# Many98/Crop2Seg

Measured on AMD Instinct MI355X. Metric: train patches/sec (Tx10x128x128) U-TAE, higher is better.
Workload: dtype f32

## Files before the change

crop2seg_amd/_lib.py:

```python
from __future__ import annotations

import ctypes as C
import os
from typing import Optional

HERE = os.path.dirname(os.path.abspath(__file__))
LIB_PATH = os.environ.get("C2S_LIB", os.path.join(HERE, "libc2s_hip.so"))

c_float_p = C.c_void_p
c_int_p = C.c_void_p

PAD_ZEROS, PAD_REFLECT = 0, 1
SRC_F32, SRC_I16, SRC_U16 = 0, 1, 2
NORM_GROUP, NORM_BATCH = 0, 1


class ConvDesc(C.Structure):
    _fields_ = [(n, C.c_int) for n in (
        "N", "C0", "C1", "Hin", "Win", "Cout", "CoutP", "Hout", "Wout", "OutH", "OutW", "KH", "KW", "S",
        "pad_y", "pad_x", "pad_mode", "osy", "osx", "ooy", "oox", "accumulate", "reflect_adjoint")]


class WgradDesc(C.Structure):
    _fields_ = [(n, C.c_int) for n in (
        "N", "C0", "C1", "Hin", "Win", "Cout", "Hout", "Wout", "KH", "KW", "S", "pad_y", "pad_x", "pad_mode",
        "nslices")]


class NormDesc(C.Structure):
    _fields_ = [("N", C.c_int), ("C", C.c_int), ("HW", C.c_int), ("kind", C.c_int), ("groups", C.c_int),
                ("training", C.c_int), ("eps", C.c_float), ("momentum", C.c_float)]


class LtaeDesc(C.Structure):
    _fields_ = [("B", C.c_int), ("T", C.c_int), ("C", C.c_int), ("HW", C.c_int), ("n_head", C.c_int),
                ("d_model", C.c_int), ("eps", C.c_float), ("dropout_p", C.c_float), ("seed", C.c_uint64),
                ("keep", C.c_void_p), ("seed_dev", C.c_void_p), ("keep_bits", C.c_void_p)]


class AggDesc(C.Structure):
    _fields_ = [(n, C.c_int) for n in ("B", "T", "C", "H", "W", "n_head", "h", "w")]


P = C.c_void_p
I = C.c_int
L = C.c_long
F = C.c_float
SZ = C.c_size_t

SIGNATURES = {
    "c2s_abi_version": (I, []),
    "c2s_last_error": (C.c_char_p, []),
    "c2s_init": (I, [I]),
    "c2s_device_cus": (I, []),
    "c2s_pack_weights": (I, [P, P, I, I, I, I, L, L, C.POINTER(I), P]),
    "c2s_pack_job_bytes": (SZ, []),
    "c2s_pack_job_fill": (I, [P, P, P, I, I, I, I, L, L, I, C.POINTER(I), I]),
    "c2s_pack_job_blocks": (I, [I, I, I, I]),
    "c2s_pack_batch": (I, [P, I, I, P]),
    "c2s_conv_igemm": (I, [C.POINTER(ConvDesc), P, P, P, P, P, P, P]),
    "c2s_conv_igemm_split": (I, [C.POINTER(ConvDesc), I]),
    "c2s_conv_xpair": (I, [C.POINTER(ConvDesc), P, P, P, P, P, P]),
    "c2s_conv3x3_smallcin_supported": (I, [C.POINTER(ConvDesc)]),
    "c2s_conv3x3_smallcin": (I, [C.POINTER(ConvDesc), P, P, P, P, P, P]),
    "c2s_winograd_packed_floats": (SZ, [I, I]),
    "c2s_pack_weights_winograd": (I, [P, P, I, I, I, L, L, C.POINTER(I), P]),
    "c2s_conv3x3_winograd": (I, [C.POINTER(ConvDesc), P, P, P, P, P, P, P]),
    "c2s_winograd16_packed_floats": (SZ, [I, I]),
    "c2s_pack_weights_winograd16": (I, [P, P, I, I, I, L, L, C.POINTER(I), P]),
    "c2s_conv3x3_winograd16_supported": (I, [C.POINTER(ConvDesc)]),
    "c2s_conv3x3_winograd16": (I, [C.POINTER(ConvDesc), P, P, P, P, P, P, P]),
    "c2s_s2wino_packed_floats": (SZ, [I, I]),
    "c2s_pack_weights_s2wino": (I, [P, P, I, I, I, L, L, C.POINTER(I), P]),
    "c2s_conv4x4s2_winograd_supported": (I, [C.POINTER(ConvDesc)]),
    "c2s_conv4x4s2_winograd": (I, [C.POINTER(ConvDesc), P, P, P, P, P, P]),
    "c2s_s2dgrad_packed_floats": (SZ, [I, I]),
    "c2s_pack_weights_s2dgrad": (I, [P, P, I, I, I, L, L, C.POINTER(I), P]),
    "c2s_conv4x4s2_dgrad_winograd_supported": (I, [C.POINTER(ConvDesc)]),
    "c2s_conv4x4s2_dgrad_winograd": (I, [C.POINTER(ConvDesc), P, P, P, P, P]),
    "c2s_conv4x4s2_dgrad_winograd_skip_supported": (I, [C.POINTER(ConvDesc), I, I]),
    "c2s_conv4x4s2_dgrad_winograd_skip": (I, [C.POINTER(ConvDesc), P, P, P, P, P, P, I, I, P]),
    "c2s_bf16x3_packed_elems": (SZ, [I, I]),
    "c2s_pack_weights_bf16x3": (I, [P, P, P, I, I, I, I, L, L, C.POINTER(I), P]),
    "c2s_conv3x3_bf16x3": (I, [C.POINTER(ConvDesc), P, P, P, P, P, P, P, P]),
    "c2s_bf16x3_set_single_product": (None, [I]),
    "c2s_wgrad_workspace_floats": (SZ, [C.POINTER(WgradDesc)]),
    "c2s_conv_wgrad": (I, [C.POINTER(WgradDesc), P, P, P, P, SZ, P, P]),
    "c2s_wgrad_algorithms": (I, [I, I]),
    "c2s_wgrad_path": (I, [C.POINTER(WgradDesc), C.POINTER(I)]),
    "c2s_wgrad_reduce": (I, [C.POINTER(WgradDesc), P, P, L, L, C.POINTER(I), I, P]),
    "c2s_wgrad_reduce_job_bytes": (SZ, []),
    "c2s_wgrad_reduce_job_blocks": (I, [C.POINTER(WgradDesc)]),
    "c2s_wgrad_reduce_job_fill": (I, [P, C.POINTER(WgradDesc), P, P, L, L, C.POINTER(I), I, I]),
    "c2s_wgrad_reduce_batch": (I, [P, I, I, P]),
    "c2s_dwconv_fwd": (I, [P, P, P, P, I, I, I, I, I, I, I, I, P]),
    "c2s_dwconv_dgrad": (I, [P, P, P, P, I, I, I, I, I, I, I, I, I, P]),
    "c2s_dwconv_wgrad": (I, [P, P, P, P, P, I, I, I, I, I, I, I, I, P]),
    "c2s_dwconv_paths": (I, [I, I, I, I, I, I, C.POINTER(I), C.POINTER(I), C.POINTER(I)]),
    "c2s_norm_workspace_floats": (SZ, [C.POINTER(NormDesc)]),
    "c2s_norm_fwd": (I, [C.POINTER(NormDesc), P, P, P, P, P, P, P, P, P, P, I, P, SZ, P, F, P]),
    "c2s_norm_bwd": (I, [C.POINTER(NormDesc), P, P, P, P, P, I, P, P, P, P, P, SZ, P, P]),
    "c2s_norm_bwd_params": (I, [C.POINTER(NormDesc), P, P, P, P, P, P]),
    "c2s_norm_onepass_sync_bytes": (SZ, [C.POINTER(NormDesc), I]),
    "c2s_norm_fwd_onepass": (I, [C.POINTER(NormDesc), P, P, P, P, P, P, P, P, P, P, I, P, F, P, SZ, P]),
    "c2s_norm_bwd_onepass": (I, [C.POINTER(NormDesc), P, P, P, P, P, I, P, P, P, P, P, SZ, P, P, SZ, P]),
    "c2s_se_workspace_floats": (SZ, [I, I, I]),
    "c2s_channel_bias_add": (I, [P, P, P, I, I, I, P]),
    "c2s_se_fwd": (I, [P, P, P, P, P, P, P, P, I, I, I, F, P, SZ, P]),
    "c2s_se_bwd": (I, [P, P, P, P, P, P, P, P, P, P, I, I, P, I, I, I, P, SZ, P]),
    "c2s_frame_flags": (I, [P, P, I, L, F, P]),
    "c2s_ltae_attn_fwd": (I, [C.POINTER(LtaeDesc)] + [P] * 13 + [P]),
    "c2s_positional_table": (I, [P, P, L, C.c_float, P]),
    "c2s_ltae_fold_fwd": (I, [P] * 9 + [I, I, P]),
    "c2s_ltae_fold_bwd": (I, [P] * 16 + [I, I, I, P, SZ, P]),
    "c2s_ltae_fold_bwd_workspace_floats": (SZ, []),
    "c2s_positional_table_ex": (I, [P, P, L, C.c_float, I, P]),
    "c2s_ltae_fold_fwd_ex": (I, [P] * 9 + [I, I, I, I, I, P]),
    "c2s_ltae_fold_bwd_ex": (I, [P] * 16 + [I, I, I, I, I, I, P, SZ, P]),
    "c2s_ltae_fold_bwd_workspace_floats_ex": (SZ, [I, I]),
    "c2s_ltae_pe_table": (I, [I, P, P, F, P, P, P, P, P, I, P]),
    "c2s_ltae_pe_abs_add": (I, [P, P, P, P, P, I, P]),
    "c2s_ltae_pe_abs_bwd": (I, [P, P, P, P, I, P]),
    "c2s_ltae_pe_fwd": (I, [P, P, P, P, P, I, I, I, I, P]),
    "c2s_ltae_pe_gattn": (I, [P, P, P, P, I, I, I, P]),
    "c2s_ltae_pe_bwd": (I, [I] + [P] * 15 + [I, I, I, P]),
    "c2s_ltae_pe_bwd_ex": (I, [I] + [P] * 15 + [I, I, I, I, P]),
    "c2s_ltae_fwd_workspace_floats": (SZ, [C.POINTER(LtaeDesc)]),
    "c2s_ltae_attn_fwd_ws": (I, [C.POINTER(LtaeDesc)] + [P] * 13 + [P, SZ, P]),
    "c2s_ltae_uses_streaming": (I, [C.POINTER(LtaeDesc)]),
    "c2s_ltae_fwd_path": (I, [C.POINTER(LtaeDesc)]),
    "c2s_ltae_attn_optional": (I, [C.POINTER(LtaeDesc)]),
    "c2s_ltae_paths": (I, [C.POINTER(LtaeDesc), I, P, P]),
    "c2s_ltae_bwd_workspace_floats": (SZ, [C.POINTER(LtaeDesc)]),
    "c2s_ltae_attn_bwd": (I, [C.POINTER(LtaeDesc)] + [P] * 22 + [SZ, P]),
    "c2s_dropout_nchw": (I, [P, P, I, I, I, F, C.c_uint64, P, P, P]),
    "c2s_pixel_gn_fwd": (I, [P, P, P, P, P, I, I, I, I, F, P]),
    "c2s_pixel_gn_bwd_workspace_floats": (SZ, [I, I, I]),
    "c2s_pixel_gn_bwd": (I, [P, P, P, P, P, P, P, I, I, I, I, P, SZ, P]),
    "c2s_attn_head_mean": (I, [P, P, I, L, P]),
    "c2s_attn_head_mean_bwd": (I, [P, P, I, L, I, P]),
    "c2s_frame_mean_weights": (I, [P, P, I, I, I, P]),
    "c2s_temporal_aggregate_fwd": (I, [C.POINTER(AggDesc), P, P, P, P, P]),
    "c2s_temporal_aggregate_bwd_workspace_floats": (SZ, [C.POINTER(AggDesc)]),
    "c2s_temporal_aggregate_bwd": (I, [C.POINTER(AggDesc), P, P, P, P, P, I, P, P, SZ, P]),
    "c2s_temporal_aggregate_bwd_skip": (I, [C.POINTER(AggDesc), P, P, P, P, P, I, P, P, P, SZ, P]),
    "c2s_agg_skip_term": (I, [C.POINTER(AggDesc), P, P, P, P, P]),
    "c2s_cross_entropy_workspace_floats": (SZ, [I, I]),
    "c2s_cross_entropy": (I, [P, P, P, P, P, I, I, I, F, C.c_longlong, P, SZ, P]),
    "c2s_metrics_update": (I, [P, P, P, P, P, P, I, I, I, P]),
    "c2s_confusion_add": (I, [P, P, P, L, I, P]),
    "c2s_loss_meter_add": (I, [P, P, P]),
    "c2s_boundary_target": (I, [P, P, I, I, I, P]),
    "c2s_region_relabel": (I, [P, P, I, I, I, I, C.c_longlong, P]),
    "c2s_focal_ce_workspace_floats": (SZ, []),
    "c2s_focal_ce": (I, [P, P, P, P, I, I, I, F, C.c_longlong, I, P, SZ, P]),
    "c2s_focal_ce_ex": (I, [P, P, P, P, P, I, I, I, F, C.c_longlong, I, I, P, SZ, P]),
    "c2s_smooth_ce_workspace_floats": (SZ, []),
    "c2s_smooth_ce": (I, [P, P, P, P, P, P, I, I, I, I, F, C.c_longlong, I, P, SZ, P]),
    "c2s_smooth_ce_ex": (I, [P, P, P, P, P, P, P, I, I, I, I, F, C.c_longlong, I, I, P, SZ, P]),
    "c2s_recall_ce_workspace_floats": (SZ, [I, I]),
    "c2s_recall_ce": (I, [P, P, P, P, P, P, I, I, I, C.c_longlong, I, P, SZ, P]),
    "c2s_parcel_seeds": (I, [P, P, P, P, I, I, I, I, I, I, F, P]),
    "c2s_label_components_workspace_bytes": (SZ, [I, I, I]),
    "c2s_label_components": (I, [P, P, P, I, I, I, I, P, SZ, P, P]),
    "c2s_parcel_vote_workspace_bytes": (SZ, [I, I, I]),
    "c2s_parcel_vote": (I, [P, P, P, P, I, I, I, I, I, F, I, P, SZ, P, P]),
    "c2s_parcel_soft_vote_workspace_bytes": (SZ, [I, I, I]),
    "c2s_parcel_soft_vote": (I, [P, P, P, P, P, P, P, I, I, I, I, I, I, F, I, P, SZ, P, P]),
    "c2s_collate_series": (I, [P, I, P, P, P, P, P, I, I, I, I, I, C.POINTER(I), C.POINTER(F), C.POINTER(F), F, P]),
    "c2s_collate_series_ndvi": (I, [P, I, P, P, P, P, P, I, I, I, I, I, C.POINTER(I), C.POINTER(F), C.POINTER(F), F, I, I, P]),
    "c2s_softmax_stitch": (I, [P, P, P, I, I, I, I, I, I, I, I, P]),
    "c2s_window_count": (I, [I, I, I]),
    "c2s_window_origin": (I, [I, I, I, I]),
    "c2s_cut_windows": (I, [P, P, I, I, I, I, I, I, I, I, I, I, I, C.POINTER(F), P]),
    "c2s_window_frames": (I, [P, I, P, P, P, P, P, I, I, I, I, I, I, I, I, I, I, F, I, P]),
    "c2s_cut_windows_raw": (I, [P, I, P, P, I, I, I, I, I, I, I, I, I, I, I, I, C.POINTER(I), C.POINTER(F), C.POINTER(F),
                                C.POINTER(F), F, I, I, P]),
    "c2s_softmax_blend": (I, [P, P, P, P, P, I, I, I, I, I, I, I, I, I, I, P]),
    "c2s_blend_finish": (I, [P, P, P, I, I, I, P]),
    "c2s_adam_flat": (I, [P, P, P, P, L, F, F, F, F, I, P, F, P]),
    "c2s_grad_sumsq_workspace_doubles": (SZ, []),
    "c2s_grad_sumsq": (I, [P, P, P, I, L, P, SZ, P, P]),
    "c2s_step_decide": (I, [P, F, F, I, P, P, I, P, P]),
    "c2s_adam_slots": (I, [P, P, P, P, P, P, P, I, L, F, F, F, F, P, P]),
    "c2s_restore_if_skipped": (I, [P, P, L, P, P]),
    "c2s_fill": (I, [P, L, F, P]),
    "c2s_add_inplace": (I, [P, P, L, P]),
}

_LIB: Optional[C.CDLL] = None


class C2SError(RuntimeError):
    pass


def lib() -> C.CDLL:
    global _LIB
    if _LIB is None:
        if not os.path.exists(LIB_PATH):
            raise C2SError(
                f"{LIB_PATH} not found: build it with `python -m crop2seg_amd.build` "
                "(or __graft_entry__.build()); crop2seg_amd has no CPU/PyTorch fallback")
        handle = C.CDLL(LIB_PATH)
        for name, (res, args) in SIGNATURES.items():
            fn = getattr(handle, name)
            fn.restype = res
            fn.argtypes = args
        _LIB = handle
    return _LIB


_INITED = set()


def init_device(index: int) -> None:
    if index in _INITED:
        return
    check(lib().c2s_init(index), "c2s_init")
    _INITED.add(index)


def check(rc: int, what: str) -> None:
    if rc != 0:
        msg = lib().c2s_last_error().decode(errors="replace")
        raise C2SError(f"{what} failed (code {rc}): {msg}")
```

crop2seg_amd/backbones/functional.py:

```python
from __future__ import annotations

from dataclasses import dataclass, field
from typing import List, Optional, Sequence, Tuple

import torch

from .. import _lib
from .. import engine as E

Tensor = torch.Tensor


@dataclass
class BackboneSpec:
    model: str = "utae"
    input_dim: int = 10
    encoder_widths: List[int] = field(default_factory=lambda: [64, 64, 64, 128])
    decoder_widths: List[int] = field(default_factory=lambda: [32, 32, 64, 128])
    out_conv: List[int] = field(default_factory=lambda: [32, 20])
    str_conv_k: int = 4
    str_conv_s: int = 2
    str_conv_p: int = 1
    agg_mode: str = "att_group"
    encoder_norm: str = "group"
    n_head: int = 16
    d_model: int = 256
    d_k: int = 4
    pad_value: float = 0.0
    padding_mode: str = "reflect"
    conv_type: str = "2d"
    add_boundary_loss: bool = False
    encoder: bool = False
    return_maps: bool = False
    pe_period: float = 1000.0
    pe_mode: str = "rel"
    num_queries: int = 1
    add_squeeze_excit: bool = False
    use_mbconv: bool = False
    attn_dropout: float = 0.1
    mlp_dropout: float = 0.2


@dataclass
class DropoutState:
    attn_seed: int = 0
    mlp_seed: int = 0
    attn_keep: Optional[Tensor] = None
    mlp_keep: Optional[Tensor] = None
    seed_dev: Optional[Tensor] = None


def _mode(spec: BackboneSpec) -> int:
    return _lib.PAD_REFLECT if spec.padding_mode == "reflect" else _lib.PAD_ZEROS


def _norm_kind(norm: str) -> int:
    if norm not in ("group", "batch", "instance"):
        raise NotImplementedError(f"norm {norm!r}")
    return _lib.NORM_BATCH if norm == "batch" else _lib.NORM_GROUP


def conv_layer(ctx: E.Ctx, srcs: Sequence[Tensor], prefix: str, n_convs: int, norm: str, k: int, s: int, p: int,
               spec: BackboneSpec, valid: Optional[Tensor], residual: Optional[Tensor] = None,
               depthwise_separable: bool = False, need_input_grad: bool = True, add_squeeze: bool = False) -> Tensor:
    mode = _mode(spec)
    x = list(srcs)
    y = None
    for i in range(n_convs):
        cp = f"{prefix}.conv.{3 * i}"
        if depthwise_separable:
            t = E.depthwise_conv2d(ctx, x[0], cp + ".depthwise.weight", k, s, p, mode, valid)
            y = E.conv2d(ctx, [t], cp + ".pointwise.weight", None, 1, 1, 0, _lib.PAD_ZEROS, valid)
            bias = None
        else:
            y = E.conv2d(ctx, x, cp + ".weight", cp + ".bias", k, s, p, mode, valid,
                         need_input_grad=need_input_grad or i > 0)
            bias = cp + ".bias"
        last = i == n_convs - 1
        y = E.norm_act(ctx, y, f"{prefix}.conv.{3 * i + 1}", _norm_kind(norm), y.shape[1] if norm == "instance" else 4, True,
                       residual if last else None, valid, spec.pad_value if valid is not None else 0.0, conv_bias=bias,
                       affine=norm != "instance")
        x = [y]
    if add_squeeze:
        y = E.squeeze_excite(ctx, y, f"{prefix}.conv.{3 * n_convs}", valid, spec.pad_value if valid is not None else 0.0)
    return y


def _norm_groups(norm: str, channels: int) -> int:
    return channels if norm == "instance" else 4


def mbconv(ctx: E.Ctx, srcs: Sequence[Tensor], prefix: str, norm: str, spec: BackboneSpec, valid: Optional[Tensor],
           need_input_grad: bool = True) -> Tensor:
    cin = sum(t.shape[1] for t in srcs)
    res = (prefix + ".0.0.block.0.weight") in ctx.p
    base = prefix + (".0.0.block" if res else ".0.0.0")
    cout = ctx.p[base + ".7.weight"].shape[0]
    assert res == (cin == cout) and (not res or len(srcs) == 1)
    kind = _norm_kind(norm)
    pv = spec.pad_value if valid is not None else 0.0
    aff = norm != "instance"
    o = E.conv2d(ctx, srcs, base + ".0.weight", base + ".0.bias", 1, 1, 0, _lib.PAD_ZEROS, valid, need_input_grad=need_input_grad)
    o = E.norm_act(ctx, o, base + ".1", kind, _norm_groups(norm, o.shape[1]), True, None, valid, pv, conv_bias=base + ".0.bias",
                   affine=aff)
    o = E.depthwise_conv2d(ctx, o, base + ".3.weight", 3, 1, 1, _lib.PAD_REFLECT, valid, bname=base + ".3.bias")
    o = E.norm_act(ctx, o, base + ".4", kind, _norm_groups(norm, o.shape[1]), True, None, valid, pv, conv_bias=base + ".3.bias",
                   affine=aff)
    o = E.squeeze_excite(ctx, o, base + ".6", valid, pv)
    o = E.conv2d(ctx, [o], base + ".7.weight", base + ".7.bias", 1, 1, 0, _lib.PAD_ZEROS, valid)
    return E.norm_act(ctx, o, base + ".8", kind, _norm_groups(norm, o.shape[1]), False, srcs[0] if res else None, valid, pv,
                      conv_bias=base + ".7.bias", affine=aff)


def mbconv_layer(ctx, srcs, prefix, n, norm, spec, valid, need_input_grad=True):
    x = list(srcs)
    for i in range(n):
        x = [mbconv(ctx, x, f"{prefix}.conv.{i}", norm, spec, valid, need_input_grad=need_input_grad or i > 0)]
    return x[0]


def conv_block(ctx, x, prefix, n_convs, norm, spec, valid, need_input_grad=True, depthwise_separable=False, add_squeeze=False):
    if spec.use_mbconv:
        return mbconv_layer(ctx, [x], prefix + ".conv", n_convs, norm, spec, valid, need_input_grad=need_input_grad)
    return conv_layer(ctx, [x], prefix + ".conv", n_convs, norm, 3, 1, 1, spec, valid, need_input_grad=need_input_grad,
                      depthwise_separable=depthwise_separable, add_squeeze=add_squeeze)


def down_conv_block(ctx, x, prefix, norm, spec, valid, depthwise_separable=False, add_squeeze=False):
    o = conv_layer(ctx, [x], prefix + ".down", 1, norm, spec.str_conv_k, spec.str_conv_s, spec.str_conv_p, spec, valid,
                   depthwise_separable=depthwise_separable)
    if spec.use_mbconv:
        o1 = mbconv_layer(ctx, [o], prefix + ".conv1", 1, norm, spec, valid)
        return mbconv_layer(ctx, [o1], prefix + ".conv2", 1, norm, spec, valid)
    o1 = conv_layer(ctx, [o], prefix + ".conv1", 1, norm, 3, 1, 1, spec, valid, depthwise_separable=depthwise_separable)
    o2 = conv_layer(ctx, [o1], prefix + ".conv2", 1, norm, 3, 1, 1, spec, valid, residual=o1,
                    depthwise_separable=depthwise_separable)
    if add_squeeze:
        o2 = E.squeeze_excite(ctx, o2, prefix + ".sae", valid, spec.pad_value if valid is not None else 0.0)
    return o2


def up_conv_block(ctx, x, skip, prefix, spec):
    sk = E.conv2d(ctx, [skip], prefix + ".skip_conv.0.weight", prefix + ".skip_conv.0.bias", 1, 1, 0, _lib.PAD_ZEROS, None)
    sk = E.norm_act(ctx, sk, prefix + ".skip_conv.1", _lib.NORM_BATCH, 1, True, None, None,
                    conv_bias=prefix + ".skip_conv.0.bias")
    assert spec.str_conv_s == 2, "only stride-2 up-convs are built"
    up = E.conv_transpose2d(ctx, x, prefix + ".up.0.weight", prefix + ".up.0.bias", spec.str_conv_k, spec.str_conv_p)
    up = E.norm_act(ctx, up, prefix + ".up.1", _lib.NORM_BATCH, 1, True, None, None, conv_bias=prefix + ".up.0.bias")
    if spec.use_mbconv:
        o1 = mbconv_layer(ctx, [up, sk], prefix + ".conv1", 1, "batch", spec, None)
        return mbconv_layer(ctx, [o1], prefix + ".conv2", 1, "batch", spec, None)
    o1 = conv_layer(ctx, [up, sk], prefix + ".conv1", 1, "batch", 3, 1, 1, spec, None)
    return conv_layer(ctx, [o1], prefix + ".conv2", 1, "batch", 3, 1, 1, spec, None, residual=o1)


def ltae(ctx, x5, dates, valid, prefix, spec: BackboneSpec, drop: DropoutState, with_tail: bool, need_attn: bool = True):
    emb, attn = E.ltae_attention(ctx, x5, dates, valid, prefix, spec.n_head, spec.d_k, spec.d_model, spec.pe_period,
                                 spec.attn_dropout, with_tail, drop.attn_seed, drop.attn_keep, drop.seed_dev,
                                 pe_mode=spec.pe_mode, need_attn=need_attn)
    if not with_tail:
        return None, attn
    o = E.conv2d(ctx, [emb], prefix + ".mlp.0.weight", prefix + ".mlp.0.bias", 1, 1, 0, _lib.PAD_ZEROS, None)
    o = E.norm_act(ctx, o, prefix + ".mlp.2", _lib.NORM_BATCH, 1, True, None, None, conv_bias=prefix + ".mlp.0.bias")
    o = E.dropout_nchw(ctx, o, spec.mlp_dropout, drop.mlp_seed, drop.mlp_keep, drop.seed_dev)
    o = E.pixel_group_norm(ctx, o, prefix + ".out_norm", spec.n_head)
    return o, attn


@dataclass
class BackboneOutput:
    logits: Optional[Tensor]
    att: Tensor
    boundary: Optional[Tensor] = None
    maps: Optional[List[Tensor]] = None
    last: Optional[Tensor] = None


def _decoder_and_head(ctx, out, skips, spec, att):
    n_stages = len(spec.encoder_widths)
    maps = [out]
    for i in range(n_stages - 1):
        out = up_conv_block(ctx, out, skips[i], f"up_blocks.{i}", spec)
        maps.append(out)
    keep_maps = maps if (spec.return_maps or spec.encoder) else None
    if spec.encoder:
        return BackboneOutput(None, att, None, keep_maps, out)
    if spec.use_mbconv:
        logits = mbconv_layer(ctx, [out], "out_conv.conv", len(spec.out_conv), "group", spec, None)
        boundary = mbconv_layer(ctx, [out], "boundary_conv.conv", 2, "group", spec, None) if spec.add_boundary_loss else None
        return BackboneOutput(logits, att, boundary, keep_maps, out)
    logits = conv_layer(ctx, [out], "out_conv.conv", len(spec.out_conv), "batch", 3, 1, 1, spec, None)
    boundary = None
    if spec.add_boundary_loss:
        boundary = conv_layer(ctx, [out], "boundary_conv.conv", 2, "batch", 3, 1, 1, spec, None)
    return BackboneOutput(logits, att, boundary, keep_maps, out)


def _fold(x5: Tensor) -> Tensor:
    B, T = x5.shape[:2]
    return x5.view(B * T, *x5.shape[2:])


def _unfold(x4: Tensor, B: int, T: int) -> Tensor:
    return x4.view(B, T, *x4.shape[1:])


def utae_forward(ctx, spec, x5, dates, drop):
    B, T = x5.shape[:2]
    valid = E.frame_flags(x5, spec.pad_value)
    dws = spec.conv_type == "depthwise_separable"
    se = spec.add_squeeze_excit
    f = conv_block(ctx, _fold(x5), "in_conv", 2, spec.encoder_norm, spec, valid, need_input_grad=False, depthwise_separable=dws,
                   add_squeeze=se)
    fmaps = [f]
    n_stages = len(spec.encoder_widths)
    for i in range(n_stages - 1):
        f = down_conv_block(ctx, f, f"down_blocks.{i}", spec.encoder_norm, spec, valid, depthwise_separable=dws, add_squeeze=se)
        fmaps.append(f)
    if ctx.tape is not None and ctx.early_hook is not None:
        ctx.tape.record(ctx.early_hook)
    out, att = ltae(ctx, _unfold(fmaps[-1], B, T), dates, valid, "temporal_encoder", spec, drop, True)
    skips = [E.temporal_aggregate(ctx, _unfold(fmaps[-(i + 2)], B, T), att, valid, spec.n_head, spec.agg_mode)
             for i in range(n_stages - 1)]
    return _decoder_and_head(ctx, out, skips, spec, att)


def timeunet_forward(ctx, spec, x5, dates, drop):
    B, T = x5.shape[:2]
    valid = E.frame_flags(x5, spec.pad_value)
    dws = spec.conv_type == "depthwise_separable"
    se = spec.add_squeeze_excit
    f0 = conv_block(ctx, _fold(x5), "in_conv", 2, spec.encoder_norm, spec, valid, need_input_grad=False, depthwise_separable=dws,
                    add_squeeze=se)
    if ctx.tape is not None and ctx.early_hook is not None:
        ctx.tape.record(ctx.early_hook)
    out, att = ltae(ctx, _unfold(f0, B, T), dates, valid, "temporal_encoder", spec, drop, True, need_attn=ctx.want_att)
    fmaps = [out]
    n_stages = len(spec.encoder_widths)
    for i in range(n_stages - 1):
        fmaps.append(down_conv_block(ctx, fmaps[-1], f"down_blocks.{i}", spec.encoder_norm, spec, None, depthwise_separable=dws,
                                     add_squeeze=se))
    skips = [fmaps[-(i + 2)] for i in range(n_stages - 1)]
    return _decoder_and_head(ctx, fmaps[-1], skips, spec, att)


def wtae_forward(ctx, spec, x5, dates, drop):
    B, T = x5.shape[:2]
    valid = E.frame_flags(x5, spec.pad_value)
    dws = spec.conv_type == "depthwise_separable"
    se = spec.add_squeeze_excit
    f0 = conv_block(ctx, _fold(x5), "in_conv", 2, spec.encoder_norm, spec, valid, need_input_grad=False, depthwise_separable=dws,
                    add_squeeze=se)
    red = f0
    n_stages = len(spec.encoder_widths)
    for i in range(n_stages - 1):
        red = down_conv_block(ctx, red, f"spatial_reduction.{i}", spec.encoder_norm, spec, valid, depthwise_separable=True,
                              add_squeeze=se)
    if ctx.tape is not None and ctx.early_hook is not None:
        ctx.tape.record(ctx.early_hook)
    _, att = ltae(ctx, _unfold(red, B, T), dates, valid, "temporal_encoder", spec, drop, False)
    fmaps = [E.temporal_aggregate(ctx, _unfold(f0, B, T), att, valid, spec.n_head, spec.agg_mode)]
    for i in range(n_stages - 1):
        fmaps.append(down_conv_block(ctx, fmaps[-1], f"down_blocks.{i}", spec.encoder_norm, spec, None, depthwise_separable=dws,
                                     add_squeeze=se))
    skips = [fmaps[-(i + 2)] for i in range(n_stages - 1)]
    return _decoder_and_head(ctx, fmaps[-1], skips, spec, att)


FORWARDS = {"utae": utae_forward, "timeunet": timeunet_forward, "wtae": wtae_forward}
```

crop2seg_amd/build.py:

```python
from __future__ import annotations

import os
import shutil
import subprocess
import sys
from concurrent.futures import ThreadPoolExecutor

HERE = os.path.dirname(os.path.abspath(__file__))
CSRC = os.path.join(HERE, "csrc")
LIB = os.path.join(HERE, "libc2s_hip.so")
SOURCES = ["pack.hip", "conv_igemm.hip", "conv_bf16x3.hip", "conv_xpair.hip", "conv_first.hip", "conv_winograd.hip", "conv_winograd16.hip", "conv_s2wino.hip", "conv_s2dgrad.hip", "conv_wgrad.hip", "norm.hip", "se.hip", "ltae.hip", "ltae_long.hip", "ltae_pe.hip", "aggregate.hip", "misc.hip", "guard.hip", "metrics.hip", "loss.hip", "parcels.hip", "io.hip"]
FLAGS = ["--offload-arch=gfx950", "-O3", "-fPIC", "-std=c++17", "-Wall", "-Wno-unused-function",
         "-Wno-unused-result", "-Wno-unused-value", "-D__HIP_PLATFORM_AMD__"]


def hipcc() -> str:
    for cand in (os.environ.get("HIPCC"), shutil.which("hipcc"), "/opt/rocm/bin/hipcc"):
        if cand and os.path.exists(cand):
            return cand
    raise RuntimeError("hipcc not found")


def _stale(target: str, deps) -> bool:
    if not os.path.exists(target):
        return True
    t = os.path.getmtime(target)
    return any(os.path.getmtime(d) > t for d in deps)


def build(force: bool = False, verbose: bool = True) -> str:
    cc = hipcc()
    headers = [os.path.join(CSRC, "common.h"), os.path.join(CSRC, "ltae_drop.h"), os.path.join(CSRC, "ltae_long.h"),
               os.path.join(CSRC, "parcels_uf.h"),
               os.path.join(os.path.dirname(HERE), "include", "c2s_hip.h")]
    objs, jobs = [], []
    for s in SOURCES:
        src = os.path.join(CSRC, s)
        obj = os.path.join(CSRC, s.replace(".hip", ".o"))
        objs.append(obj)
        if force or _stale(obj, [src] + headers):
            jobs.append((src, obj))

    def compile_one(job):
        src, obj = job
        cmd = [cc, *FLAGS, "-c", src, "-o", obj]
        r = subprocess.run(cmd, capture_output=True, text=True)
        if r.returncode != 0:
            raise RuntimeError(f"hipcc failed for {src}:\n{r.stdout}\n{r.stderr}")
        if verbose and r.stderr.strip():
            print(r.stderr, file=sys.stderr)
        return obj

    if jobs:
        with ThreadPoolExecutor(max_workers=min(4, len(jobs))) as ex:
            list(ex.map(compile_one, jobs))
    if force or jobs or _stale(LIB, objs):
        r = subprocess.run([cc, "--offload-arch=gfx950", "-shared", "-fPIC", *objs, "-o", LIB],
                           capture_output=True, text=True)
        if r.returncode != 0:
            raise RuntimeError(f"link failed:\n{r.stdout}\n{r.stderr}")
    return LIB


if __name__ == "__main__":
    print(build(force="--force" in sys.argv))
```

crop2seg_amd/csrc/conv_first.hip:

```cpp
#include "common.h"

namespace {

struct FirstParams {
    const float* src;
    const float* wpk;
    const float* bias;
    float* out;
    const int* valid;
    int N, Cin, H, W, Cout, CoutP;
    int tiles_x, tiles_y, ntiles;
};

constexpr int FT_ROWS = 8, FT_COLS = 32;
constexpr int FT_PR = FT_ROWS + 2, FT_PC = FT_COLS + 2;
constexpr int ft_chs() {
    int v = FT_PR * FT_PC;
    while (v % 64 != 32) ++v;
    return v;
}
constexpr int FT_CHS = ft_chs();

template <int NP, bool REFLECT>
__global__ __launch_bounds__(256, 2) void conv_first_kernel(FirstParams p) {
    constexpr int NCH = 2 * NP;
    constexpr int NE = NCH * FT_PR * FT_PC;
    constexpr int EPT = (NE + 255) / 256;
    __shared__ float patch[NCH * FT_CHS];
    const int tid = threadIdx.x, lane = tid & 63, wave = __builtin_amdgcn_readfirstlane(tid >> 6);
    const int px = lane & 31, kk = lane >> 5;
    const int cb = blockIdx.y * 64;

    float wreg[9][NP][2];
#pragma unroll
    for (int t = 0; t < 9; ++t)
#pragma unroll
        for (int s = 0; s < NP; ++s) {
            const int ch = 2 * s + kk;
#pragma unroll
            for (int h = 0; h < 2; ++h) {
                const float v = p.wpk[((size_t)t * p.Cin + (ch < p.Cin ? ch : 0)) * p.CoutP + cb + h * 32 + px];
                wreg[t][s][h] = ch < p.Cin ? v : 0.f;
            }
        }
    __shared__ float bias_s[64];
    if (tid < 64) bias_s[tid] = (p.bias != nullptr && cb + tid < p.Cout) ? p.bias[cb + tid] : 0.f;

    auto load_patch = [&](int tile, float (&v)[EPT]) {
        int tid = threadIdx.x;
        asm volatile("" : "+v"(tid));
        const int n = tile / (p.tiles_x * p.tiles_y);
        const int rem = tile - n * (p.tiles_x * p.tiles_y);
        const int y0 = (rem / p.tiles_x) * FT_ROWS - 1, x0 = (rem % p.tiles_x) * FT_COLS - 1;
        const float* base = p.src + (size_t)n * p.Cin * p.H * p.W;
#pragma unroll
        for (int j = 0; j < EPT; ++j) {
            const int e = tid + 256 * j;
            const int ch = e / (FT_PR * FT_PC), r2 = e - ch * (FT_PR * FT_PC);
            const int row = r2 / FT_PC, col = r2 - row * FT_PC;
            int gy = y0 + row, gx = x0 + col;
            bool ok = e < NE && ch < p.Cin;
            if (REFLECT) {
                gy = reflect_idx(gy, p.H); gx = reflect_idx(gx, p.W);
            } else {
                ok = ok && gy >= 0 && gy < p.H && gx >= 0 && gx < p.W;
                gy = min(max(gy, 0), p.H - 1); gx = min(max(gx, 0), p.W - 1);
            }
            const int chc = min(ch, p.Cin - 1);
            const float t = base[((size_t)chc * p.H + gy) * p.W + gx];
            v[j] = ok ? t : 0.f;
        }
    };
    auto store_patch = [&](const float (&v)[EPT]) {
        int tid = threadIdx.x;
        asm volatile("" : "+v"(tid));
#pragma unroll
        for (int j = 0; j < EPT; ++j) {
            const int e = tid + 256 * j;
            const int ch = e / (FT_PR * FT_PC), r2 = e - ch * (FT_PR * FT_PC);
            if (e < NE) patch[ch * FT_CHS + r2] = v[j];
        }
    };
    auto frame_ok = [&](int tile) {
        return p.valid == nullptr || p.valid[tile / (p.tiles_x * p.tiles_y)] != 0;
    };

    int tile = blockIdx.x;
    float pre[EPT];
    if (tile < p.ntiles && frame_ok(tile)) load_patch(tile, pre);
    for (; tile < p.ntiles; tile += gridDim.x) {
        const bool ok = frame_ok(tile);
        const int nxt = tile + gridDim.x;
        if (ok) {
            __syncthreads();
            store_patch(pre);
            __syncthreads();
        }
        if (nxt < p.ntiles && frame_ok(nxt)) load_patch(nxt, pre);
        if (!ok) continue;
        f32x16 acc[2][2];
#pragma unroll
        for (int r = 0; r < 2; ++r)
#pragma unroll
            for (int h = 0; h < 2; ++h)
#pragma unroll
                for (int i = 0; i < 16; ++i) acc[r][h][i] = 0.f;
        const float* pb = patch + kk * FT_CHS + (2 * wave) * FT_PC + px;
#pragma unroll
        for (int ky = 0; ky < 3; ++ky)
#pragma unroll
            for (int kx = 0; kx < 3; ++kx)
#pragma unroll
                for (int s = 0; s < NP; ++s) {
                    const float b0 = pb[2 * s * FT_CHS + ky * FT_PC + kx];
                    const float b1 = pb[2 * s * FT_CHS + (ky + 1) * FT_PC + kx];
                    acc[0][0] = __builtin_amdgcn_mfma_f32_32x32x2f32(wreg[ky * 3 + kx][s][0], b0, acc[0][0], 0, 0, 0);
                    acc[0][1] = __builtin_amdgcn_mfma_f32_32x32x2f32(wreg[ky * 3 + kx][s][1], b0, acc[0][1], 0, 0, 0);
                    acc[1][0] = __builtin_amdgcn_mfma_f32_32x32x2f32(wreg[ky * 3 + kx][s][0], b1, acc[1][0], 0, 0, 0);
                    acc[1][1] = __builtin_amdgcn_mfma_f32_32x32x2f32(wreg[ky * 3 + kx][s][1], b1, acc[1][1], 0, 0, 0);
                }
        const int n = tile / (p.tiles_x * p.tiles_y);
        const int rem = tile - n * (p.tiles_x * p.tiles_y);
        const int y = (rem / p.tiles_x) * FT_ROWS + 2 * wave, x0 = (rem % p.tiles_x) * FT_COLS;
        const size_t plane = (size_t)p.H * p.W;
        float* ub = p.out + ((size_t)n * p.Cout + cb) * plane + (size_t)y * p.W + x0;
        const unsigned lo = (unsigned)(4 * kk) * (unsigned)plane + (unsigned)px;
#pragma unroll
        for (int h = 0; h < 2; ++h)
#pragma unroll
            for (int i = 0; i < 16; ++i) {
                const int og = h * 32 + (i & 3) + 8 * (i >> 2);
                float* op = ub + (size_t)og * plane;
                const float b = bias_s[og + 4 * kk];
                op[lo] = acc[0][h][i] + b;
                op[lo + p.W] = acc[1][h][i] + b;
            }
    }
}

}

extern "C" int c2s_conv3x3_smallcin_supported(const c2s_conv_desc* d) {
    return d && d->KH == 3 && d->KW == 3 && d->S == 1 && d->pad_y == 1 && d->pad_x == 1 && d->C1 == 0 && d->C0 >= 1 &&
           d->C0 <= 10 && d->Cout % 64 == 0 && d->CoutP == d->Cout && d->Hin % FT_ROWS == 0 && d->Win % FT_COLS == 0 && d->Hout == d->Hin &&
           d->Wout == d->Win && d->OutH == d->Hin && d->OutW == d->Win && d->osy == 1 && d->osx == 1 && d->ooy == 0 &&
           d->oox == 0 && !d->accumulate && !d->reflect_adjoint;
}

extern "C" int c2s_conv3x3_smallcin(const c2s_conv_desc* d, const float* src, const float* wpk, const float* bias,
                                    float* out, const int* valid, void* stream) {
    C2S_REQUIRE(d && src && wpk && out, "conv3x3_smallcin: null pointer");
    C2S_REQUIRE(c2s_conv3x3_smallcin_supported(d),
                "conv3x3_smallcin: needs 3x3/s1/pad1, one source of <= 10 channels, Cout %% 64 == 0, H %% 8 == 0, W %% 32 == 0");
    if (d->pad_mode == C2S_PAD_REFLECT) C2S_REQUIRE(d->Hin >= 2 && d->Win >= 2, "conv3x3_smallcin: reflect needs planes >= 2x2");
    FirstParams p;
    p.src = src; p.wpk = wpk; p.bias = bias; p.out = out; p.valid = valid;
    p.N = d->N; p.Cin = d->C0; p.H = d->Hin; p.W = d->Win; p.Cout = d->Cout; p.CoutP = d->CoutP;
    p.tiles_x = d->Win / FT_COLS; p.tiles_y = d->Hin / FT_ROWS;
    const long nt = (long)d->N * p.tiles_x * p.tiles_y;
    C2S_REQUIRE(nt < (1L << 30), "conv3x3_smallcin: too many tiles");
    p.ntiles = (int)nt;
    const int cus = c2s_cus();
    const int wgs = (int)(nt < 2L * cus ? nt : 2L * cus);
    const dim3 grid(wgs, d->CoutP / 64);
    hipStream_t st = (hipStream_t)stream;
    const bool reflect = d->pad_mode == C2S_PAD_REFLECT;
    if (d->C0 <= 4) {
        if (reflect) hipLaunchKernelGGL((conv_first_kernel<2, true>), grid, dim3(256), 0, st, p);
        else hipLaunchKernelGGL((conv_first_kernel<2, false>), grid, dim3(256), 0, st, p);
    } else {
        if (reflect) hipLaunchKernelGGL((conv_first_kernel<5, true>), grid, dim3(256), 0, st, p);
        else hipLaunchKernelGGL((conv_first_kernel<5, false>), grid, dim3(256), 0, st, p);
    }
    C2S_CHECK_LAUNCH("conv_first");
    return C2S_OK;
}
```

crop2seg_amd/csrc/norm.hip:

```cpp
#include "common.h"

namespace {

constexpr int SEG = 2048;

__host__ __device__ inline int seg_len(int HW) { return HW < SEG ? HW : SEG; }
__host__ __device__ inline int n_segs(int HW) { return (HW + seg_len(HW) - 1) / seg_len(HW); }

struct SegItem { long row; int seg, len; size_t base; };
__device__ __forceinline__ SegItem seg_item(long item, int HW, int segs) {
    SegItem it;
    it.row = item / segs;
    it.seg = (int)(item % segs);
    const int L = seg_len(HW);
    const int beg = it.seg * L;
    it.len = (HW - beg) < L ? (HW - beg) : L;
    it.base = (size_t)it.row * HW + beg;
    return it;
}


__device__ __forceinline__ float fwd_element(float x, float mu, float a, float b, int relu, bool has_res, float r) {
    float t = (x - mu) * a + b;
    if (relu) t = fmaxf(t, 0.f);
    if (has_res) t += r;
    return t;
}
__device__ __forceinline__ float masked_grad(float g, float xc, float a, float b, int relu) {
    return (!relu || xc * a + b > 0.f) ? g : 0.f;
}
__device__ __forceinline__ void grad_sums(float gg, float xc, float rstd, float& s1, float& s2) {
    s1 += gg;
    s2 += gg * (xc * rstd);
}
__device__ __forceinline__ float bwd_element(float gg, float xc, float k1, float k2, float k3, float& sdx) {
    const float o = k1 * gg + k2 * xc + k3;
    sdx += o;
    return o;
}

__device__ __forceinline__ float chunk_sum(const f32x4& v) { return (v.x + v.y) + (v.z + v.w); }
__device__ __forceinline__ float chunk_sum(float v) { return v; }
__device__ __forceinline__ float chunk_sqdev(const f32x4& v, float mean) {
    const float a = v.x - mean, b = v.y - mean, c = v.z - mean, d = v.w - mean;
    return (a * a + b * b) + (c * c + d * d);
}
__device__ __forceinline__ float chunk_sqdev(float v, float mean) {
    const float a = v - mean;
    return a * a;
}
template <typename F>
__device__ __forceinline__ void each(float x, float r, float& o, F fe) { fe(x, r, o); }
template <typename F>
__device__ __forceinline__ void each(const f32x4& x, const f32x4& r, f32x4& o, F fe) {
#pragma unroll
    for (int e = 0; e < 4; ++e) {
        float t = 0.f;
        fe(x[e], r[e], t);
        o[e] = t;
    }
}

template <typename V, int NK>
__device__ __forceinline__ void load_segment(const float* __restrict__ p, int lane, f32x4 (&v)[NK]) {
#pragma unroll
    for (int k = 0; k < NK; ++k) v[k] = *reinterpret_cast<const V*>(p + lane * 4 + 256 * k);
}

template <int NK>
__device__ __forceinline__ void segment_moments(const f32x4 (&v)[NK], float& mean, float& m2) {
    float s = 0.f;
#pragma unroll
    for (int k = 0; k < NK; ++k) s += chunk_sum(v[k]);
    s = wave_sum(s);
    mean = s / (float)(NK * 256);
    m2 = 0.f;
#pragma unroll
    for (int k = 0; k < NK; ++k) m2 += chunk_sqdev(v[k], mean);
}

template <bool STORE, typename F>
__device__ __forceinline__ void walk_tail(const float* __restrict__ x, const float* __restrict__ r, bool has_r,
                                          float* __restrict__ out, size_t base, int len, int lane, F f) {
    if ((len & 3) == 0) {
        for (int i = lane * 4; i < len; i += 256) {
            const f32x4 xv = *reinterpret_cast<const f32x4*>(x + base + i);
            f32x4 rv = {0.f, 0.f, 0.f, 0.f}, o;
            if (has_r) rv = *reinterpret_cast<const f32x4*>(r + base + i);
            f(xv, rv, o);
            if (STORE) *reinterpret_cast<f32x4*>(out + base + i) = o;
        }
    } else {
        for (int i = lane; i < len; i += 64) {
            float o;
            f(x[base + i], has_r ? r[base + i] : 0.f, o);
            if (STORE) out[base + i] = o;
        }
    }
}
template <bool STORE, typename F>
__device__ __forceinline__ void walk_segment(const float* __restrict__ x, const float* __restrict__ r, bool has_r,
                                             float* __restrict__ out, size_t base, int len, int lane, F f) {
    if (len != SEG) return walk_tail<STORE>(x, r, has_r, out, base, len, lane, f);
    f32x4 xv[SEG / 256], rv[SEG / 256];
    load_segment<f32x4u>(x + base, lane, xv);
    if (has_r) load_segment<f32x4u>(r + base, lane, rv);
#pragma unroll
    for (int k = 0; k < SEG / 256; ++k) {
        f32x4 o;
        f(xv[k], has_r ? rv[k] : f32x4{0.f, 0.f, 0.f, 0.f}, o);
        if (STORE) *reinterpret_cast<f32x4u*>(out + base + lane * 4 + 256 * k) = o;
    }
}

template <typename P>
__device__ __forceinline__ void merge_moments(int items, int lane, float eps, P partial, float& mean_f, float& rstd_f,
                                              float& unbiased) {
    double cnt = 0.0, sum = 0.0;
    for (int it = lane; it < items; it += 64) {
        float pm, pm2;
        int len;
        if (!partial(it, pm, pm2, len)) continue;
        cnt += len;
        sum += (double)pm * len;
    }
    for (int o = 32; o > 0; o >>= 1) { cnt += __shfl_xor(cnt, o, 64); sum += __shfl_xor(sum, o, 64); }
    const double mean = cnt > 0 ? sum / cnt : 0.0;
    double m2 = 0.0;
    for (int it = lane; it < items; it += 64) {
        float pm, pm2;
        int len;
        if (!partial(it, pm, pm2, len)) continue;
        const double dm = (double)pm - mean;
        m2 += (double)pm2 + dm * dm * len;
    }
    for (int o = 32; o > 0; o >>= 1) m2 += __shfl_xor(m2, o, 64);
    const double var = cnt > 0 ? m2 / cnt : 0.0;
    mean_f = (float)mean;
    rstd_f = (float)(1.0 / sqrt(var + (double)eps));
    unbiased = (float)(cnt > 1 ? m2 / (cnt - 1.0) : var);
}

template <typename P>
__device__ __forceinline__ void row_sums(int segs, P partial, float& s1, float& s2) {
    double t1 = 0.0, t2 = 0.0;
    for (int s = 0; s < segs; ++s) {
        float p1, p2;
        partial(s, p1, p2);
        t1 += p1;
        t2 += p2;
    }
    s1 = (float)t1;
    s2 = (float)t2;
}
template <typename R>
__device__ __forceinline__ void merge_coeffs(int n_rows, int lane, int HW, float rstd, R row, float& k2, float& k3) {
    double A = 0.0, Bv = 0.0, cnt = 0.0;
    for (int r = lane; r < n_rows; r += 64) {
        float gm, s1, s2;
        if (!row(r, gm, s1, s2)) continue;
        A += (double)gm * (double)s1;
        Bv += (double)gm * (double)s2;
        cnt += HW;
    }
    for (int o = 32; o > 0; o >>= 1) { A += __shfl_xor(A, o, 64); Bv += __shfl_xor(Bv, o, 64); cnt += __shfl_xor(cnt, o, 64); }
    const double m = cnt > 0 ? cnt : 1.0;
    k2 = (float)(-(double)rstd * rstd * Bv / m);
    k3 = (float)(-(double)rstd * A / m);
}

__global__ __launch_bounds__(256) void row_stats_kernel(const float* __restrict__ x, float* __restrict__ part,
                                                        const int* __restrict__ valid, int C, int HW, int segs,
                                                        long nitems) {
    const long item = (long)blockIdx.x * 4 + (threadIdx.x >> 6);
    if (item >= nitems) return;
    const int lane = threadIdx.x & 63;
    const auto [row, seg, len, base] = seg_item(item, HW, segs);
    if (valid != nullptr && valid[row / C] == 0) return;
    float mean, m2 = 0.f;
    if (len == SEG) {
        f32x4 v[SEG / 256];
        load_segment<f32x4u>(x + base, lane, v);
        segment_moments(v, mean, m2);
    } else {
        float s = 0.f;
        walk_tail<false>(x, nullptr, false, nullptr, base, len, lane, [&](auto v, auto, auto&) { s += chunk_sum(v); });
        s = wave_sum(s);
        mean = s / (float)len;
        walk_tail<false>(x, nullptr, false, nullptr, base, len, lane, [&](auto v, auto, auto&) { m2 += chunk_sqdev(v, mean); });
    }
    m2 = wave_sum(m2);
    if (lane == 0) {
        part[item * 2 + 0] = mean;
        part[item * 2 + 1] = m2;
    }
}

__device__ __forceinline__ void group_mean_rstd(const float* __restrict__ part, const int* __restrict__ valid,
                                                const c2s_norm_desc& d, int segs, int grp, int lane, float& mean_f,
                                                float& rstd_f, float& unbiased) {
    const int L = seg_len(d.HW);
    const bool batch = d.kind == C2S_NORM_BATCH;
    const int cpg = batch ? 1 : d.C / d.groups;
    const int n_rows = batch ? d.N : cpg;
    merge_moments(n_rows * segs, lane, d.eps, [&](int it, float& pm, float& pm2, int& len) {
        const int r = it / segs, sg = it % segs;
        const long row = batch ? (long)r * d.C + grp : (long)(grp / d.groups) * d.C + (grp % d.groups) * cpg + r;
        if (batch && valid != nullptr && valid[r] == 0) return false;
        len = (d.HW - sg * L) < L ? (d.HW - sg * L) : L;
        pm = part[(row * segs + sg) * 2];
        pm2 = part[(row * segs + sg) * 2 + 1];
        return true;
    }, mean_f, rstd_f, unbiased);
}

__global__ __launch_bounds__(256) void norm_apply_kernel(const float* __restrict__ x, const float* __restrict__ part,
                                                         const float* __restrict__ gamma, const float* __restrict__ beta,
                                                         float* __restrict__ rmean, float* __restrict__ rvar,
                                                         long long* __restrict__ nbt,
                                                         float* __restrict__ gstats, float* __restrict__ row_ab,
                                                         const float* __restrict__ res, float* __restrict__ y,
                                                         const int* __restrict__ valid, c2s_norm_desc d, int segs,
                                                         long nitems, int relu, float pad_value) {
    const long item = (long)blockIdx.x * 4 + (threadIdx.x >> 6);
    if (item >= nitems) return;
    const int lane = threadIdx.x & 63;
    const int C = d.C, HW = d.HW;
    const auto [row, seg, len, base] = seg_item(item, HW, segs);
    const int n = (int)(row / C), c = (int)(row % C);
    const bool ok = valid == nullptr || valid[n] != 0;
    const bool batch = d.kind == C2S_NORM_BATCH;
    const int cpg = batch ? 1 : C / d.groups;
    const int grp = batch ? c : n * d.groups + c / cpg;
    const bool first_row = seg == 0 && (batch ? n == 0 : c % cpg == 0);
    float mu = 0.f, rstd = 0.f;
    if (batch && !d.training) {
        mu = rmean[grp];
        rstd = rsqrtf(rvar[grp] + d.eps);
    } else if (batch || ok) {
        float unb;
        group_mean_rstd(part, valid, d, segs, grp, lane, mu, rstd, unb);
        if (batch && first_row && lane == 0 && rmean != nullptr) {
            rmean[grp] = (1.f - d.momentum) * rmean[grp] + d.momentum * mu;
            rvar[grp] = (1.f - d.momentum) * rvar[grp] + d.momentum * unb;
        }
        if (batch && item == 0 && lane == 0 && nbt != nullptr) *nbt += 1;
    }
    if (first_row && lane == 0) { gstats[grp * 2] = mu; gstats[grp * 2 + 1] = rstd; }
    if (!ok) {
        if (seg == 0 && lane == 0) { row_ab[row * 3] = 0.f; row_ab[row * 3 + 1] = 0.f; row_ab[row * 3 + 2] = 0.f; }
        for (int i = lane; i < len; i += 64) y[base + i] = pad_value;
        return;
    }
    const float a = gamma[c] * rstd, b = beta[c];
    if (seg == 0 && lane == 0) { row_ab[row * 3] = a; row_ab[row * 3 + 1] = b; row_ab[row * 3 + 2] = mu; }
    const bool has_res = res != nullptr;
    walk_segment<true>(x, res, has_res, y, base, len, lane, [&](auto xv, auto rv, auto& o) {
        each(xv, rv, o, [&](float xe, float re, float& t) { t = fwd_element(xe, mu, a, b, relu, has_res, re); });
    });
}

__global__ __launch_bounds__(256) void norm_bwd_sums_kernel(const float* __restrict__ x, const float* __restrict__ g,
                                                            const float* __restrict__ row_ab,
                                                            const float* __restrict__ gstats, float* __restrict__ part,
                                                            const int* __restrict__ valid, c2s_norm_desc d, int segs,
                                                            long nitems, int relu) {
    const long item = (long)blockIdx.x * 4 + (threadIdx.x >> 6);
    if (item >= nitems) return;
    const int lane = threadIdx.x & 63;
    const auto [row, seg, len, base] = seg_item(item, d.HW, segs);
    const int n = (int)(row / d.C), c = (int)(row % d.C);
    if (valid != nullptr && valid[n] == 0) {
        if (lane == 0) { part[item * 3] = 0.f; part[item * 3 + 1] = 0.f; }
        return;
    }
    const int grp = d.kind == C2S_NORM_BATCH ? c : n * d.groups + c / (d.C / d.groups);
    const float mean = gstats[grp * 2], rstd = gstats[grp * 2 + 1];
    const float a = row_ab[row * 3], b = row_ab[row * 3 + 1];
    float s1 = 0.f, s2 = 0.f;
    walk_segment<false>(x, g, true, nullptr, base, len, lane, [&](auto xv, auto gv, auto& o) {
        each(xv, gv, o, [&](float xe, float ge, float&) {
            const float xc = xe - mean;
            grad_sums(masked_grad(ge, xc, a, b, relu), xc, rstd, s1, s2);
        });
    });
    s1 = wave_sum(s1); s2 = wave_sum(s2);
    if (lane == 0) { part[item * 3] = s1; part[item * 3 + 1] = s2; }
}

__device__ __forceinline__ void part_row_sums(const float* __restrict__ part, long row, int segs, float& s1, float& s2) {
    row_sums(segs, [&](int s, float& p1, float& p2) {
        p1 = part[(row * segs + s) * 3];
        p2 = part[(row * segs + s) * 3 + 1];
    }, s1, s2);
}

__global__ __launch_bounds__(64) void norm_bwd_params_kernel(const float* __restrict__ part, float* __restrict__ dgamma,
                                                             float* __restrict__ dbeta, float* __restrict__ dbias,
                                                             const int* __restrict__ valid, int N, int C, int segs) {
    const int c = blockIdx.x, lane = threadIdx.x;
    double dg = 0, db = 0;
    for (int n = lane; n < N; n += 64) {
        if (valid != nullptr && valid[n] == 0) continue;
        float s1, s2;
        part_row_sums(part, (long)n * C + c, segs, s1, s2);
        dg += (double)s2;
        db += (double)s1;
    }
    for (int o = 32; o > 0; o >>= 1) { dg += __shfl_xor(dg, o, 64); db += __shfl_xor(db, o, 64); }
    if (lane == 0) {
        if (dgamma != nullptr) dgamma[c] = (float)dg;
        if (dbeta != nullptr) dbeta[c] = (float)db;
    }
    if (dbias == nullptr) return;
    double s = 0;
    for (int it = lane; it < N * segs; it += 64) {
        const int n = it / segs, k = it - n * segs;
        if (valid != nullptr && valid[n] == 0) continue;
        s += part[(((long)n * C + c) * segs + k) * 3 + 2];
    }
    for (int o = 32; o > 0; o >>= 1) s += __shfl_xor(s, o, 64);
    if (lane == 0) dbias[c] = (float)s;
}

__global__ __launch_bounds__(256) void norm_bwd_apply_kernel(const float* __restrict__ x, const float* __restrict__ g,
                                                             const float* __restrict__ row_ab,
                                                             const float* __restrict__ gamma,
                                                             const float* __restrict__ gstats, float* __restrict__ gx,
                                                             float* __restrict__ part,
                                                             const int* __restrict__ valid, c2s_norm_desc d, int segs,
                                                             long nitems, int relu) {
    const long item = (long)blockIdx.x * 4 + (threadIdx.x >> 6);
    if (item >= nitems) return;
    const int lane = threadIdx.x & 63;
    const int C = d.C, HW = d.HW;
    const auto [row, seg, len, base] = seg_item(item, HW, segs);
    if (valid != nullptr && valid[row / C] == 0) {
        for (int i = lane; i < len; i += 64) gx[base + i] = 0.f;
        if (lane == 0) part[item * 3 + 2] = 0.f;
        return;
    }
    const bool batch = d.kind == C2S_NORM_BATCH;
    const int cpg = batch ? 1 : C / d.groups;
    const int n_rows = batch ? d.N : cpg;
    const int cc = (int)(row % C), nn = (int)(row / C);
    const int grp = batch ? cc : nn * d.groups + cc / cpg;
    const float rstd = gstats[grp * 2 + 1];
    float k1 = rstd * gamma[cc], k2 = 0.f, k3 = 0.f;
    if (!(batch && !d.training)) {
        merge_coeffs(n_rows, lane, HW, rstd, [&](int r, float& gm, float& s1, float& s2) {
            const long rr = batch ? (long)r * C + grp : (long)nn * C + (grp % d.groups) * cpg + r;
            if (valid != nullptr && valid[rr / C] == 0) return false;
            gm = gamma[rr % C];
            part_row_sums(part, rr, segs, s1, s2);
            return true;
        }, k2, k3);
    }
    const float a = row_ab[row * 3], b = row_ab[row * 3 + 1], mu = row_ab[row * 3 + 2];
    float sdx = 0.f;
    walk_segment<true>(x, g, true, gx, base, len, lane, [&](auto xv, auto gv, auto& o) {
        each(xv, gv, o, [&](float xe, float ge, float& dx) {
            const float xc = xe - mu;
            dx = bwd_element(masked_grad(ge, xc, a, b, relu), xc, k1, k2, k3, sdx);
        });
    });
    sdx = wave_sum(sdx);
    if (lane == 0) part[item * 3 + 2] = sdx;
}

struct SyncView {
    unsigned* hdr;
    unsigned long long* gran;
};
__host__ __device__ inline size_t sync_bytes(long nitems) { return 64 + (size_t)nitems * 16; }
__device__ __forceinline__ SyncView sync_view(void* base) {
    SyncView v;
    v.hdr = reinterpret_cast<unsigned*>(base);
    v.gran = reinterpret_cast<unsigned long long*>(reinterpret_cast<char*>(base) + 64);
    return v;
}
constexpr int OP_MAXG = 8;

__device__ __forceinline__ void onepass_begin(const SyncView& sv, unsigned* s_hdr, unsigned& epoch, bool& poisoned) {
    if (threadIdx.x == 0) {
        s_hdr[0] = __hip_atomic_load(&sv.hdr[2], __ATOMIC_RELAXED, __HIP_MEMORY_SCOPE_AGENT);
        s_hdr[1] = __hip_atomic_load(&sv.hdr[3], __ATOMIC_RELAXED, __HIP_MEMORY_SCOPE_AGENT);
    }
    __syncthreads();
    epoch = s_hdr[0] + 1u;
    poisoned = s_hdr[1] != 0u;
}
__device__ __forceinline__ void onepass_end(const SyncView& sv, unsigned epoch) {
    __syncthreads();
    if (threadIdx.x == 0) {
        const unsigned f = __hip_atomic_fetch_add(&sv.hdr[0], 1u, __ATOMIC_RELAXED, __HIP_MEMORY_SCOPE_AGENT);
        if (f + 1u == gridDim.x) {
            __hip_atomic_store(&sv.hdr[0], 0u, __ATOMIC_RELAXED, __HIP_MEMORY_SCOPE_AGENT);
            __hip_atomic_store(&sv.hdr[2], epoch, __ATOMIC_RELAXED, __HIP_MEMORY_SCOPE_AGENT);
        }
    }
}
__device__ __forceinline__ void onepass_publish(const SyncView& sv, long v, unsigned epoch, float p0, float p1, int lane) {
    if (lane == 0) {
        const unsigned long long e = (unsigned long long)epoch << 32;
        __hip_atomic_store(&sv.gran[v * 2 + 0], e | __float_as_uint(p0), __ATOMIC_RELAXED, __HIP_MEMORY_SCOPE_AGENT);
        __hip_atomic_store(&sv.gran[v * 2 + 1], e | __float_as_uint(p1), __ATOMIC_RELAXED, __HIP_MEMORY_SCOPE_AGENT);
    }
}
__device__ __forceinline__ void onepass_sweep(const SyncView& sv, long g0, int wpg, unsigned epoch, int lane, bool poisoned,
                                              float* __restrict__ pa, float* __restrict__ pb) {
    for (int polls = poisoned ? (1 << 17) : 0;; ++polls) {
        bool hit = true;
#pragma unroll 2
        for (int w = lane; w < wpg; w += 64) {
            const unsigned long long ga = __hip_atomic_load(&sv.gran[(g0 + w) * 2 + 0], __ATOMIC_RELAXED, __HIP_MEMORY_SCOPE_AGENT);
            const unsigned long long gb = __hip_atomic_load(&sv.gran[(g0 + w) * 2 + 1], __ATOMIC_RELAXED, __HIP_MEMORY_SCOPE_AGENT);
            hit = hit && (unsigned)(ga >> 32) == epoch && (unsigned)(gb >> 32) == epoch;
            pa[w] = __uint_as_float((unsigned)ga);
            pb[w] = __uint_as_float((unsigned)gb);
        }
        if (__all(hit)) break;
        if (polls > (1 << 17)) {
            if (lane == 0) __hip_atomic_store(&sv.hdr[3], 1u, __ATOMIC_RELAXED, __HIP_MEMORY_SCOPE_AGENT);
            for (int w = lane; w < wpg; w += 64) { pa[w] = __uint_as_float(0x7fc00000u); pb[w] = __uint_as_float(0x7fc00000u); }
            break;
        }
        __builtin_amdgcn_s_sleep(4);
    }
    asm volatile("s_waitcnt lgkmcnt(0)" ::: "memory");
}

struct OnepassItem { int grp, w, seg; long row; };
__device__ __forceinline__ OnepassItem onepass_item(long v, const c2s_norm_desc& d, int segs) {
    const bool batch = d.kind == C2S_NORM_BATCH;
    const int cpg = batch ? 1 : d.C / d.groups;
    const int n_rows = batch ? d.N : cpg;
    const int ipg = n_rows * segs;
    OnepassItem it;
    it.grp = (int)(v / ipg);
    it.w = (int)(v - (long)it.grp * ipg);
    const int r = it.w / segs;
    it.seg = it.w - r * segs;
    it.row = batch ? (long)r * d.C + it.grp : (long)it.grp * cpg + r;
    return it;
}

template <int NK>
struct OpSlot {
    f32x4 xv[NK];
    long v, row;
    size_t base;
    int grp, w, seg;
    bool live, ok;
};

template <int NK, bool RES>
__global__ __launch_bounds__(256) void norm_onepass_fwd_kernel(const float* __restrict__ x, const float* __restrict__ gamma,
                                                               const float* __restrict__ beta, float* __restrict__ rmean,
                                                               float* __restrict__ rvar, long long* __restrict__ nbt,
                                                               float* __restrict__ gstats, float* __restrict__ row_ab,
                                                               const float* __restrict__ res, float* __restrict__ y,
                                                               const int* __restrict__ valid, c2s_norm_desc d, int segs,
                                                               long nitems, int relu, float pad_value, void* sync) {
    __shared__ unsigned s_hdr[2];
    __shared__ float s_stat[2][2];
    __shared__ float s_part[2][OP_MAXG * 64];
    const SyncView sv = sync_view(sync);
    unsigned epoch;
    bool poisoned;
    onepass_begin(sv, s_hdr, epoch, poisoned);
    const int lane = threadIdx.x & 63, wave = threadIdx.x >> 6;
    const int C = d.C, HW = d.HW;
    const bool batch = d.kind == C2S_NORM_BATCH;
    const int cpg = batch ? 1 : C / d.groups;
    const int wpg = (batch ? d.N : cpg) * segs;
    constexpr int L = NK * 256;
    const long quads = (nitems + 3) >> 2;

    auto fetch = [&](OpSlot<NK>& s, long q) {
        s.v = q * 4 + wave;
        s.live = s.v < nitems;
        const OnepassItem it = onepass_item(s.live ? s.v : nitems - 1, d, segs);
        s.row = it.row; s.grp = it.grp; s.w = it.w; s.seg = it.seg;
        s.base = (size_t)it.row * HW + (size_t)it.seg * L;
        s.ok = valid == nullptr || valid[(int)(it.row / C)] != 0;
        if (s.live && s.ok) {
#pragma unroll
            for (int k = 0; k < NK; ++k) s.xv[k] = *reinterpret_cast<const f32x4*>(x + s.base + lane * 4 + 256 * k);
        }
    };
    auto reduce_publish = [&](OpSlot<NK>& s, float& pmean, float& m2) {
        pmean = 0.f; m2 = 0.f;
        if (!(s.live && s.ok)) return;
        segment_moments(s.xv, pmean, m2);
        m2 = wave_sum(m2);
        if (wpg > 1) onepass_publish(sv, s.v, epoch, pmean, m2, lane);
    };
    auto finish = [&](OpSlot<NK>& s, float pmean, float m2, int par) {
        const int c = (int)(s.row % C);
        if (!s.ok) {
            if (s.live) {
                if (s.seg == 0 && lane == 0) {
                    row_ab[s.row * 3] = 0.f; row_ab[s.row * 3 + 1] = 0.f; row_ab[s.row * 3 + 2] = 0.f;
                    if (c % cpg == 0) { gstats[s.grp * 2] = 0.f; gstats[s.grp * 2 + 1] = 0.f; }
                }
                f32x4 pv = {pad_value, pad_value, pad_value, pad_value};
#pragma unroll
                for (int k = 0; k < NK; ++k) *reinterpret_cast<f32x4*>(y + s.base + lane * 4 + 256 * k) = pv;
            }
            return;
        }
        f32x4 rv[NK];
        if constexpr (RES) {
            if (s.live) {
#pragma unroll
                for (int k = 0; k < NK; ++k) rv[k] = *reinterpret_cast<const f32x4*>(res + s.base + lane * 4 + 256 * k);
            }
        }
        float mu, rstd, unb;
        bool leader;
        if (wpg > 1) {
            if (wave == 0) {
                onepass_sweep(sv, s.v - s.w, wpg, epoch, lane, poisoned, s_part[0], s_part[1]);
                merge_moments(wpg, lane, d.eps, [&](int w, float& pm, float& pm2, int& len) {
                    pm = s_part[0][w];
                    pm2 = s_part[1][w];
                    len = L;
                    return true;
                }, mu, rstd, unb);
                if (lane == 0) { s_stat[par][0] = mu; s_stat[par][1] = rstd; }
            }
            __syncthreads();
            if (wave != 0) { mu = s_stat[par][0]; rstd = s_stat[par][1]; unb = 0.f; }
            leader = s.w == 0;
        } else {
            const double var = (double)m2 / L;
            mu = pmean;
            rstd = (float)(1.0 / sqrt(var + (double)d.eps));
            unb = (float)(L > 1 ? (double)m2 / (L - 1.0) : var);
            leader = s.live;
        }
        if (!s.live) return;
        if (leader && lane == 0) {
            gstats[s.grp * 2] = mu; gstats[s.grp * 2 + 1] = rstd;
            if (batch && rmean != nullptr) {
                rmean[s.grp] = (1.f - d.momentum) * rmean[s.grp] + d.momentum * mu;
                rvar[s.grp] = (1.f - d.momentum) * rvar[s.grp] + d.momentum * unb;
            }
            if (batch && s.grp == 0 && nbt != nullptr) *nbt += 1;
        }
        const float a = gamma[c] * rstd, b = beta[c];
        if (s.seg == 0 && lane == 0) { row_ab[s.row * 3] = a; row_ab[s.row * 3 + 1] = b; row_ab[s.row * 3 + 2] = mu; }
        const bool failed = mu != mu;
#pragma unroll
        for (int k = 0; k < NK; ++k) {
            f32x4 o;
#pragma unroll
            for (int e = 0; e < 4; ++e) {
                const float t = fwd_element(s.xv[k][e], mu, a, b, relu, RES, RES ? rv[k][e] : 0.f);
                o[e] = failed ? mu : t;
            }
            *reinterpret_cast<f32x4*>(y + s.base + lane * 4 + 256 * k) = o;
        }
    };

    OpSlot<NK> A, B;
    long q = blockIdx.x;
    if (q < quads) fetch(A, q);
    while (q < quads) {
        float pm, m2;
        reduce_publish(A, pm, m2);
        long qn = q + gridDim.x;
        if (qn < quads) fetch(B, qn);
        finish(A, pm, m2, 0);
        q = qn;
        if (q >= quads) break;
        reduce_publish(B, pm, m2);
        qn = q + gridDim.x;
        if (qn < quads) fetch(A, qn);
        finish(B, pm, m2, 1);
        q = qn;
    }
    onepass_end(sv, epoch);
}

template <int NK>
struct OpSlotB {
    f32x4 xa[NK], ga[NK];
    long v, row;
    size_t base;
    int grp, w, seg;
    bool live, ok;
};

template <int NK>
__global__ __launch_bounds__(256) void norm_onepass_bwd_kernel(const float* __restrict__ x, const float* __restrict__ g,
                                                               const float* __restrict__ row_ab,
                                                               const float* __restrict__ gamma,
                                                               const float* __restrict__ gstats, float* __restrict__ gx,
                                                               float* __restrict__ part, const int* __restrict__ valid,
                                                               c2s_norm_desc d, int segs, long nitems, int relu,
                                                               void* sync) {
    __shared__ unsigned s_hdr[2];
    __shared__ float s_stat[2][2];
    __shared__ float s_part[2][OP_MAXG * 64];
    const SyncView sv = sync_view(sync);
    unsigned epoch;
    bool poisoned;
    onepass_begin(sv, s_hdr, epoch, poisoned);
    const int lane = threadIdx.x & 63, wave = threadIdx.x >> 6;
    const int C = d.C, HW = d.HW;
    const bool batch = d.kind == C2S_NORM_BATCH;
    const int cpg = batch ? 1 : C / d.groups;
    const int n_rows = batch ? d.N : cpg;
    const int wpg = n_rows * segs;
    constexpr int L = NK * 256;
    const long quads = (nitems + 3) >> 2;

    auto fetch = [&](OpSlotB<NK>& s, long q) {
        s.v = q * 4 + wave;
        s.live = s.v < nitems;
        const OnepassItem it = onepass_item(s.live ? s.v : nitems - 1, d, segs);
        s.row = it.row; s.grp = it.grp; s.w = it.w; s.seg = it.seg;
        s.base = (size_t)it.row * HW + (size_t)it.seg * L;
        s.ok = valid == nullptr || valid[(int)(it.row / C)] != 0;
        if (s.live && s.ok) {
#pragma unroll
            for (int k = 0; k < NK; ++k) {
                s.xa[k] = *reinterpret_cast<const f32x4*>(x + s.base + lane * 4 + 256 * k);
                s.ga[k] = *reinterpret_cast<const f32x4*>(g + s.base + lane * 4 + 256 * k);
            }
        }
    };
    auto reduce_publish = [&](OpSlotB<NK>& s, float& s1, float& s2) {
        s1 = 0.f; s2 = 0.f;
        if (!(s.live && s.ok)) return;
        const float mean = gstats[s.grp * 2], rstd = gstats[s.grp * 2 + 1];
        const float a = row_ab[s.row * 3], b = row_ab[s.row * 3 + 1];
#pragma unroll
        for (int k = 0; k < NK; ++k)
#pragma unroll
            for (int e = 0; e < 4; ++e) {
                const float xc = s.xa[k][e] - mean;
                const float gg = masked_grad(s.ga[k][e], xc, a, b, relu);
                s.ga[k][e] = gg;
                grad_sums(gg, xc, rstd, s1, s2);
            }
        s1 = wave_sum(s1); s2 = wave_sum(s2);
        if (wpg > 1) onepass_publish(sv, s.v, epoch, s1, s2, lane);
        const long item = s.row * segs + s.seg;
        if (lane == 0) { part[item * 3] = s1; part[item * 3 + 1] = s2; }
    };
    auto finish = [&](OpSlotB<NK>& s, float s1, float s2, int par) {
        const int cc = (int)(s.row % C);
        const long item = s.row * segs + s.seg;
        if (!s.ok) {
            if (s.live) {
                f32x4 z = {0.f, 0.f, 0.f, 0.f};
#pragma unroll
                for (int k = 0; k < NK; ++k) *reinterpret_cast<f32x4*>(gx + s.base + lane * 4 + 256 * k) = z;
                if (lane == 0) { part[item * 3] = 0.f; part[item * 3 + 1] = 0.f; part[item * 3 + 2] = 0.f; }
            }
            return;
        }
        const float rstd = gstats[s.grp * 2 + 1];
        float k2, k3;
        if (wpg > 1) {
            if (wave == 0) {
                onepass_sweep(sv, s.v - s.w, wpg, epoch, lane, poisoned, s_part[0], s_part[1]);
                merge_coeffs(n_rows, lane, HW, rstd, [&](int r, float& gm, float& t1, float& t2) {
                    const long rr = batch ? (long)r * C + s.grp : (long)s.grp * cpg + r;
                    gm = gamma[rr % C];
                    row_sums(segs, [&](int sg, float& p1, float& p2) {
                        p1 = s_part[0][r * segs + sg];
                        p2 = s_part[1][r * segs + sg];
                    }, t1, t2);
                    return true;
                }, k2, k3);
                if (lane == 0) { s_stat[par][0] = k2; s_stat[par][1] = k3; }
            }
            __syncthreads();
            if (wave != 0) { k2 = s_stat[par][0]; k3 = s_stat[par][1]; }
        } else {
            const double gm = (double)gamma[cc];
            k2 = (float)(-(double)rstd * rstd * (gm * (double)s2) / (double)HW);
            k3 = (float)(-(double)rstd * (gm * (double)s1) / (double)HW);
        }
        if (!s.live) return;
        const float mu = row_ab[s.row * 3 + 2];
        const float k1 = rstd * gamma[cc];
        float sdx = 0.f;
#pragma unroll
        for (int k = 0; k < NK; ++k) {
            f32x4 o;
#pragma unroll
            for (int e = 0; e < 4; ++e) o[e] = bwd_element(s.ga[k][e], s.xa[k][e] - mu, k1, k2, k3, sdx);
            *reinterpret_cast<f32x4*>(gx + s.base + lane * 4 + 256 * k) = o;
        }
        sdx = wave_sum(sdx);
        if (lane == 0) part[item * 3 + 2] = sdx;
    };

    OpSlotB<NK> A, B;
    long q = blockIdx.x;
    if (q < quads) fetch(A, q);
    while (q < quads) {
        float s1, s2;
        reduce_publish(A, s1, s2);
        long qn = q + gridDim.x;
        if (qn < quads) fetch(B, qn);
        finish(A, s1, s2, 0);
        q = qn;
        if (q >= quads) break;
        reduce_publish(B, s1, s2);
        qn = q + gridDim.x;
        if (qn < quads) fetch(A, qn);
        finish(B, s1, s2, 1);
        q = qn;
    }
    onepass_end(sv, epoch);
}

__host__ inline int onepass_nk(const c2s_norm_desc* d, const int* valid) {
    const int L = seg_len(d->HW);
    if (d->HW % L != 0 || L % 256 != 0) return 0;
    const int nk = L / 256;
    if (nk != 1 && nk != 2 && nk != 4 && nk != 8) return 0;
    const bool batch = d->kind == C2S_NORM_BATCH;
    if (batch && (!d->training || valid != nullptr)) return 0;
    const long wpg = (long)(batch ? d->N : d->C / d->groups) * n_segs(d->HW);
    if (wpg > 64 * OP_MAXG || (wpg != 1 && wpg % 4 != 0)) return 0;
    return nk;
}
// ... 159 lines not shown
```

crop2seg_amd/engine.py:

```python
from __future__ import annotations

import ctypes as C
from typing import Callable, Dict, List, NamedTuple, Optional, Sequence, Tuple

import torch

from . import _lib
from ._lib import AggDesc, ConvDesc, LtaeDesc, NormDesc, WgradDesc, check, lib

Tensor = torch.Tensor


def _ptr(t: Optional[Tensor]) -> Optional[int]:
    return None if t is None else t.data_ptr()


def _stream() -> int:
    return torch.cuda.current_stream().cuda_stream


import os as _os

_SIDE = None
SIDE_WGRAD = _os.environ.get("C2S_WGRAD_STREAM", "1") != "0"
SIDE_BATCH = int(_os.environ.get("C2S_WGRAD_BATCH", "8"))
SIDE_FLUSH_POSITIONS = int(_os.environ.get("C2S_WGRAD_FLUSH_POSITIONS", str(1 << 22)))
GRAPH_SIDE = _os.environ.get("C2S_GRAPH_SIDE", "0") != "0"
AGG_SKIP_TERM = _os.environ.get("C2S_AGG_SKIP_TERM", "1") != "0"


BACKWARD_LOG: Optional[list] = None


def _log(op: str, name: str, kind: str) -> None:
    if BACKWARD_LOG is not None:
        BACKWARD_LOG.append((op, name, kind))


def _side_ok() -> bool:
    return SIDE_WGRAD and (GRAPH_SIDE or not torch.cuda.is_current_stream_capturing())


def _side_stream():
    global _SIDE
    if _SIDE is None:
        _SIDE = torch.cuda.Stream()
    return _SIDE


class PackRecord(NamedTuple):
    src_ptr: int
    cin: int
    cout: int
    coutP: int
    ntaps: int
    so: int
    sc: int
    kind: int
    taps: Tuple[int, ...]
    nfloats: int


PACK_KINDS = {0: (32, None, "c2s_pack_weights"),
              1: (64, "c2s_winograd_packed_floats", "c2s_pack_weights_winograd"),
              2: (64, "c2s_winograd16_packed_floats", "c2s_pack_weights_winograd16"),
              3: (64, "c2s_s2wino_packed_floats", "c2s_pack_weights_s2wino"),
              4: (64, "c2s_s2dgrad_packed_floats", "c2s_pack_weights_s2dgrad")}


def _tap_array(offs: Sequence[int]):
    return (C.c_int * len(offs))(*offs)


class Workspace:

    def __init__(self, device):
        self.device = device
        if getattr(device, "type", None) == "cuda":
            idx = device.index if device.index is not None else torch.cuda.current_device()
            with torch.cuda.device(idx):
                _lib.init_device(idx)
        self.bufs: Dict[str, Tensor] = {}
        self.pack_record: Dict[Tuple, PackRecord] = {}
        self.pack_plan: Optional[dict] = None
        self.reduce_jobs: List[Tuple] = []
        self.reduce_post: List[Tuple] = []
        self.reduce_plan: Optional[dict] = None

    def finalize_pack_plan(self) -> None:
        if self.pack_plan is not None or not self.pack_record:
            return
        L_ = lib()
        rec_bytes = L_.c2s_pack_job_bytes()
        jobs = list(self.pack_record.items())
        table = torch.zeros(len(jobs) * rec_bytes, dtype=torch.uint8).pin_memory() if torch.cuda.is_available() else \
            torch.zeros(len(jobs) * rec_bytes, dtype=torch.uint8)
        outs, block = {}, 0
        for i, (key, r) in enumerate(jobs):
            out = torch.empty(r.nfloats, device=self.device, dtype=torch.float32)
            check(L_.c2s_pack_job_fill(table.data_ptr() + i * rec_bytes, r.src_ptr, out.data_ptr(), r.cin, r.cout, r.coutP,
                                       r.ntaps, r.so, r.sc, r.kind, _tap_array(r.taps), block), "pack_job_fill")
            block += L_.c2s_pack_job_blocks(r.cin, r.coutP, r.ntaps, r.kind)
            outs[key] = (out, r.src_ptr)
        self.pack_plan = {"table": table.to(self.device), "njobs": len(jobs), "blocks": block, "outs": outs}
        self.pack_record = {}

    def run_reduce_batch(self) -> None:
        jobs, self.reduce_jobs = self.reduce_jobs, []
        post, self.reduce_post = self.reduce_post, []
        if jobs:
            self._reduce_batch(jobs, {j[0].data_ptr() for j in post})
        for (slabs, dst_ptr, so, sc, taps, d) in post:
            check(lib().c2s_wgrad_reduce(C.byref(d), slabs.data_ptr(), dst_ptr, so, sc, _tap_array(taps), 1, _stream()),
                  "wgrad_reduce")

    def _reduce_batch(self, jobs: List[Tuple], post_slabs: set) -> None:
        L_ = lib()
        key = tuple(j[:-1] for j in jobs)
        plan = self.reduce_plan
        if plan is None or plan["key"] != key:
            if torch.cuda.is_current_stream_capturing():
                import warnings
                warnings.warn("crop2seg_amd: the batched weight-gradient slice sum has no job table for this capture (the warm-up "
                              "pass ran other layers or buffers): falling back to one launch per layer inside the graph")
                for (dbytes, slabs_ptr, dst_ptr, so, sc, taps, acc, d) in jobs:
                    check(L_.c2s_wgrad_reduce(C.byref(d), slabs_ptr, dst_ptr, so, sc, _tap_array(taps), acc, _stream()), "wgrad_reduce")
                return
            rec = L_.c2s_wgrad_reduce_job_bytes()
            table = torch.zeros(len(jobs) * rec, dtype=torch.uint8).pin_memory()
            block = 0
            for i, (dbytes, slabs_ptr, dst_ptr, so, sc, taps, acc, d) in enumerate(jobs):
                check(L_.c2s_wgrad_reduce_job_fill(table.data_ptr() + i * rec, C.byref(d), slabs_ptr, dst_ptr, so, sc,
                                                   _tap_array(taps), acc, block), "wgrad_reduce_job_fill")
                block += L_.c2s_wgrad_reduce_job_blocks(C.byref(d))
            plan = self.reduce_plan = {"key": key, "table": table.to(self.device), "njobs": len(jobs), "blocks": block}
            live = {j[1] for j in jobs} | post_slabs
            for name in [k for k, b in self.bufs.items() if k.startswith("wgrad_slabs:") and b.data_ptr() not in live]:
                del self.bufs[name]
        check(L_.c2s_wgrad_reduce_batch(plan["table"].data_ptr(), plan["njobs"], plan["blocks"], _stream()), "wgrad_reduce_batch")

    def sync_area(self, nbytes: int) -> Tensor:
        b = self.bufs.get("sync")
        if b is None or b.numel() < nbytes:
            nb = torch.zeros(max(int(nbytes), 4096), device=self.device, dtype=torch.uint8)
            if b is not None:
                nb[12:16].copy_(b[12:16])
            b = self.bufs["sync"] = nb
        return b

    def sync_error(self) -> int:
        b = self.bufs.get("sync")
        return 0 if b is None else int(b[:16].view(torch.int32)[3])

    def check_sync(self) -> None:
        if self.sync_error() == 0:
            return
        global ONEPASS_NORM
        ONEPASS_NORM = False
        torch.cuda.synchronize(self.device)
        self.bufs["sync"].zero_()
        raise RuntimeError(
            "crop2seg_amd: a one-pass normalisation wait gave up (the workgroups of a group were not co-resident: "
            "shared or masked GPU, profiler serialisation?).  The affected outputs are NaN.  The sync area has been "
            "reset and this process now uses the two-pass normalisation kernels.  Repeat the step if it was a forward pass or "
            "a TrainStep(skip_nonfinite=True) step (the device skipped the update); otherwise the NaN has reached the "
            "parameters, the Adam moments and the BatchNorm running statistics: restore the last checkpoint.")

    def get(self, name: str, nfloats: int) -> Tensor:
        b = self.bufs.get(name)
        if b is None or b.numel() < nfloats:
            b = torch.empty(max(int(nfloats), 1), device=self.device, dtype=torch.float32)
            self.bufs[name] = b
        return b


class Tape:

    def __init__(self):
        self.ops: List[Callable[[], None]] = []
        self.grads: Dict[int, Tensor] = {}
        self.keep: List[Tensor] = []
        self.side_keep: List[Tensor] = []
        self.side_used = False
        self.side_pending: List[Callable[[], None]] = []
        self.finalizers: Dict[int, Callable[[], None]] = {}
        self.s2d_sources: Dict[int, Tuple[object, Optional[int]]] = {}
        self.skip_terms: Dict[int, "SkipTerm"] = {}

    def fork(self) -> "torch.cuda.Stream":
        side = _side_stream()
        ev = torch.cuda.Event()
        ev.record()
        side.wait_event(ev)
        self.side_used = True
        return side

    def record(self, fn: Callable[[], None]) -> None:
        self.ops.append(fn)

    def track(self, t: Tensor) -> Tensor:
        self.keep.append(t)
        return t

    def settle(self, key: int) -> None:
        term = self.skip_terms.pop(key, None)
        if term is not None:
            check(lib().c2s_agg_skip_term(C.byref(term.desc), term.a_up.data_ptr(), term.gskip.data_ptr(), _ptr(term.valid),
                                          self.grads[key].data_ptr(), _stream()), "agg_skip_term")

    def take_skip_term(self, t: Tensor) -> Optional["SkipTerm"]:
        return self.skip_terms.pop(t.data_ptr(), None)

    def grad_of(self, t: Tensor) -> Optional[Tensor]:
        self.settle(t.data_ptr())
        return self.grads.get(t.data_ptr())

    def pop_grad(self, t: Tensor) -> Optional[Tensor]:
        self.settle(t.data_ptr())
        return self.grads.pop(t.data_ptr(), None)

    def add_grad(self, t: Tensor, g: Tensor, own: bool = True) -> None:
        self.settle(t.data_ptr())
        cur = self.grads.get(t.data_ptr())
        if cur is None:
            self.grads[t.data_ptr()] = g if own else g.clone()
        else:
            check(lib().c2s_add_inplace(cur.data_ptr(), g.data_ptr(), g.numel(), _stream()), "add_inplace")

    def grad_buffer(self, t: Tensor) -> Tuple[Tensor, int]:
        self.settle(t.data_ptr())
        g = self.grads.get(t.data_ptr())
        if g is not None:
            return g, 1
        g = self.grads[t.data_ptr()] = torch.empty_like(t)
        return g, 0

    def defer(self, fn: Callable[[], None], keep: Sequence[Tensor]) -> None:
        self.side_pending.append(fn)
        self.side_keep.extend(keep)
        if len(self.side_pending) >= SIDE_BATCH:
            self.flush_side()

    def flush_side(self) -> None:
        if not self.side_pending:
            return
        with torch.cuda.stream(self.fork()):
            for fn in self.side_pending:
                fn()
        self.side_pending.clear()

    def backward(self) -> None:
        for fn in reversed(self.ops):
            fn()
        for key in list(self.skip_terms):
            self.settle(key)
        assert not self.skip_terms
        self.s2d_sources.clear()
        self.flush_side()
        if self.finalizers:
            fins, self.finalizers = list(self.finalizers.values()), {}
            if self.side_used:
                with torch.cuda.stream(_side_stream()):
                    for fn in fins:
                        fn()
            else:
                for fn in fins:
                    fn()
        if self.side_used:
            ev = torch.cuda.Event()
            ev.record(_side_stream())
            torch.cuda.current_stream().wait_event(ev)
            self.side_used = False
        self.side_keep.clear()
        self.ops.clear()
        self.keep.clear()


class SkipTerm(NamedTuple):
    a_up: Tensor
    gskip: Tensor
    desc: object
    valid: Optional[Tensor]
    n_head: int
    T: int
    name: str


class Ctx:

    def __init__(self, params: Dict[str, Tensor], buffers: Dict[str, Tensor], grads: Optional[Dict[str, Tensor]],
                 ws: Workspace, training: bool, tape: Optional[Tape], eps: float = 1e-5, momentum: float = 0.1,
                 trainable: Optional[Sequence[str]] = None):
        self.p = params
        self.b = buffers
        self.g = grads
        self.trainable = None if trainable is None else frozenset(trainable)
        self._needs: set = set()
        self.ws = ws
        self.training = training
        self.tape = tape
        self.eps = eps
        self.momentum = momentum
        self.device = ws.device
        self._packed: Dict[Tuple, Tensor] = {}
        self._plan_ran = False
        self._gwritten: set = set()
        self.early_hook = None
        self.want_att = True
        cus = lib().c2s_device_cus()
        self.cus = cus if cus > 0 else 256

    def trains(self, name: Optional[str]) -> bool:
        return name is not None and (self.trainable is None or name in self.trainable)

    def needs(self, t: Optional[Tensor]) -> bool:
        return self.trainable is None or (t is not None and t.data_ptr() in self._needs)

    def mark(self, outs: Sequence[Optional[Tensor]], inputs: Sequence[Optional[Tensor]] = (),
             params: Sequence[Optional[str]] = ()) -> bool:
        if self.tape is None:
            return False
        if self.trainable is None:
            return True
        if not (any(self.needs(t) for t in inputs if t is not None) or any(self.trains(n) for n in params)):
            return False
        self._needs.update(o.data_ptr() for o in outs if o is not None)
        return True

    def grad_sink(self, name: str) -> Tuple[Tensor, int]:
        assert self.trains(name), f"grad_sink: {name} is frozen"
        acc = 1 if name in self._gwritten else 0
        self._gwritten.add(name)
        return self.g[name], acc

    def add_param_grad(self, name: str, g: Tensor) -> None:
        dst, acc = self.grad_sink(name)
        if acc:
            check(lib().c2s_add_inplace(dst.data_ptr(), g.data_ptr(), g.numel(), _stream()), "add_inplace")
        else:
            dst.copy_(g.view_as(dst))

    def _planned(self, key: Tuple, src_ptr: int) -> Optional[Tensor]:
        plan = self.ws.pack_plan
        if plan is None:
            return None
        hit = plan["outs"].get(key)
        if hit is None or hit[1] != src_ptr:
            self.ws.pack_plan = None
            self.ws.pack_record = {}
            return None
        if not self._plan_ran:
            check(lib().c2s_pack_batch(plan["table"].data_ptr(), plan["njobs"], plan["blocks"], _stream()), "pack_batch")
            self._plan_ran = True
        return hit[0]

    def pack(self, key: Tuple, src: Tensor, src_off: int, cin: int, cout: int, so: int, sc: int, taps: Sequence[int],
             kind: int = 0) -> Tuple[Tensor, int]:
        step, floats_fn, pack_fn = PACK_KINDS[kind]
        coutP = (cout + step - 1) // step * step
        hit = self._packed.get(key)
        if hit is not None:
            return hit, coutP
        src_ptr = src.data_ptr() + 4 * src_off
        out = self._planned(key, src_ptr)
        if out is None:
            L_ = lib()
            ntaps = len(taps)
            nfl = ntaps * cin * coutP if kind == 0 else getattr(L_, floats_fn)(cin, coutP)
            out = torch.empty(nfl, device=self.device, dtype=torch.float32)
            lead = (src_ptr, out.data_ptr(), cin, cout, coutP) + ((ntaps,) if kind == 0 else ())
            check(getattr(L_, pack_fn)(*lead, so, sc, _tap_array(taps), _stream()), pack_fn)
            self.ws.pack_record[key] = PackRecord(src_ptr, cin, cout, coutP, ntaps, so, sc, kind, tuple(taps), nfl)
        self._packed[key] = out
        return out, coutP


def _pack_bf16x3(ctx: "Ctx", key: Tuple, src: Tensor, src_off: int, cin: int, cout: int, so: int, sc: int,
                 taps: Sequence[int]) -> Tuple[Tensor, Tensor, int]:
    hit = ctx._packed.get(key)
    coutP = (cout + 31) // 32 * 32
    if hit is not None:
        return hit[0], hit[1], coutP
    n = lib().c2s_bf16x3_packed_elems(cin, coutP)
    whi = torch.empty(n, device=ctx.device, dtype=torch.bfloat16)
    wlo = torch.empty(n, device=ctx.device, dtype=torch.bfloat16)
    check(lib().c2s_pack_weights_bf16x3(src.data_ptr() + 4 * src_off, whi.data_ptr(), wlo.data_ptr(), cin, cout, coutP,
                                        len(taps), so, sc, _tap_array(taps), _stream()), "pack_weights_bf16x3")
    ctx._packed[key] = (whi, wlo)
    return whi, wlo, coutP


def frame_flags(x5: Tensor, pad_value: float) -> Tensor:
    B, T = x5.shape[:2]
    valid = torch.empty(B * T, device=x5.device, dtype=torch.int32)
    check(lib().c2s_frame_flags(x5.data_ptr(), valid.data_ptr(), B * T, x5[0, 0].numel(), float(pad_value), _stream()),
          "frame_flags")
    return valid


REDUCE_BATCH = _os.environ.get("C2S_REDUCE_BATCH", "0") != "0"

CONV_MODE = _os.environ.get("C2S_CONV_MODE", "f32")
assert CONV_MODE in ("f32", "bf16x3"), CONV_MODE
WINOGRAD = _os.environ.get("C2S_WINOGRAD", "1") != "0"
WINO16 = _os.environ.get("C2S_WINO16", "1") != "0"
S2WINO = _os.environ.get("C2S_S2WINO", "1") != "0"


def _use_winograd(K: int, S: int, pad: int, chans: Sequence[int], cout: int, H: int, W: int) -> bool:
    return (WINOGRAD and CONV_MODE == "f32" and K == 3 and S == 1 and pad == 1 and sum(chans) >= 32 and cout >= 64
            and H % 2 == 0 and W % 4 == 0 and W >= 8 and (len(chans) == 1 or chans[0] % 8 == 0))


def _wide_winograd(H: int, W: int, chans: Sequence[int]) -> bool:
    return WINO16 and W >= 32 and H >= 8 and sum(chans) > 24 and all(c % 8 == 0 for c in chans)


def _use_bf16x3(K: int, S: int, pad: int, chans: Sequence[int]) -> bool:
    return CONV_MODE == "bf16x3" and K == 3 and S == 1 and pad == 1 and all(c % 8 == 0 for c in chans)


def _xpair_taps(py: int) -> List[int]:
    return [((3 - py) - 2 * ty) * 4 + ((3 - px) - 2 * tx) for px in range(2) for ty in range(2) for tx in range(2)]


PARITY_GEOMETRIES = ((2, 0), (6, 2))


def _parity_taps(K: int, pad: int, py: int, px: int) -> List[int]:
    kp = K // 2
    return [(py + 2 * pad - 2 * ty) * K + (px + 2 * pad - 2 * tx) for ty in range(kp) for tx in range(kp)]


def _conv_desc(*, N: int, C0: int, C1: int = 0, Hin: int, Win: int, Cout: int, CoutP: int, Hout: int, Wout: int, K: int,
               S: int = 1, pad: int, pad_x: Optional[int] = None, pad_mode: int = _lib.PAD_ZEROS, OutH: Optional[int] = None,
               OutW: Optional[int] = None, osy: int = 1, osx: int = 1, ooy: int = 0, oox: int = 0, accumulate: int = 0,
               reflect_adjoint: int = 0) -> ConvDesc:
    return ConvDesc(N, C0, C1, Hin, Win, Cout, CoutP, Hout, Wout, Hout if OutH is None else OutH,
                    Wout if OutW is None else OutW, K, K, S, pad, pad if pad_x is None else pad_x, pad_mode, osy, osx, ooy, oox,
                    accumulate, reflect_adjoint)


class ConvLaunch(NamedTuple):
    desc: ConvDesc
    key: Tuple
    kind: int
    off: int
    cin: int
    cout: int
    so: int
    sc: int
    taps: Tuple[int, ...]


class ConvPlan(NamedTuple):
    family: str
    launches: Tuple[ConvLaunch, ...]


CONV_FAMILIES = {
    "wino16": ("c2s_conv3x3_winograd16", True, True, True),
    "wino4": ("c2s_conv3x3_winograd", True, True, True),
    "bf16x3": ("c2s_conv3x3_bf16x3", True, True, False),
    "s2wino": ("c2s_conv4x4s2_winograd", False, True, False),
    "s2dgrad": ("c2s_conv4x4s2_dgrad_winograd", False, False, False),
    "smallcin": ("c2s_conv3x3_smallcin", False, True, False),
    "igemm": ("c2s_conv_igemm", True, True, True),
    "xpair": ("c2s_conv_xpair", False, True, False),
    "parity": ("c2s_conv_igemm", True, True, True),
}


def _launch(kind: int, key: Tuple, off: int, cin: int, cout: int, so: int, sc: int, taps: Sequence[int], **desc) -> ConvLaunch:
    step = PACK_KINDS[kind][0]
    return ConvLaunch(_conv_desc(**{"C0": cin, **desc}, Cout=cout, CoutP=(cout + step - 1) // step * step),
                      key, kind, off, cin, cout, so, sc, tuple(taps))


def _transposed_launches(family: str, key: Tuple, off: int, cin: int, cout: int, so: int, sc: int, K: int, pad: int, N: int,
                         H: int, W: int, accumulate: int, radj: int) -> ConvPlan:
    plane = dict(N=N, Hin=H, Win=W, Hout=H, Wout=W, OutH=2 * H, OutW=2 * W, osy=2, osx=2, accumulate=accumulate)
    if family == "xpair":
        return ConvPlan(family, tuple(
            _launch(0, key + (py,), off, cin, cout, so, sc, _xpair_taps(py), K=2, pad=1 - py, pad_x=0, ooy=py,
                    reflect_adjoint=radj, **plane) for py in range(2)))
    return ConvPlan(family, tuple(
        _launch(0, key + ("par", py, px), off, cin, cout, so, sc, _parity_taps(K, pad, py, px), K=K // 2, pad=pad // 2, ooy=py,
                oox=px, reflect_adjoint=2 if radj else 0, **plane) for py in range(2) for px in range(2)))


def _family_3x3(N: int, chans: Sequence[int], cout: int, H: int, W: int, K: int, S: int, pad: int):
    if _use_winograd(K, S, pad, chans, cout, H, W):
        wide = _wide_winograd(H, W, chans) and N <= 65536
        return ("wino16", 2, "wino") if wide else ("wino4", 1, "wino")
    return ("bf16x3", 0, "bx") if _use_bf16x3(K, S, pad, chans) and H != 3 and W != 3 else None


def conv_plan(op: str, N: int, chans: Sequence[int], Cout: int, Hin: int, Win: int, K: int, S: int, pad: int, pad_mode: int,
              si: int = 0, accumulate: int = 0) -> ConvPlan:
    KK, Cin = K * K, sum(chans)
    if op == "tfwd":
        return _transposed_launches("xpair" if K == 4 else "parity", ("fwd",), 0, Cin, Cout, KK, Cout * KK, K, pad, N, Hin, Win,
                                    0, 0)
    if op == "tdgrad":
        return ConvPlan("igemm", (_launch(0, ("dgrad",), 0, Cout, Cin, Cout * KK, KK, range(KK), N=N, Hin=2 * Hin, Win=2 * Win,
                                          Hout=Hin, Wout=Win, K=K, S=2, pad=pad, accumulate=accumulate),))
    Ho, Wo = (Hin + 2 * pad - K) // S + 1, (Win + 2 * pad - K) // S + 1
    if op == "fwd":
        def fwd(family, kind, *key):
            return ConvPlan(family, (_launch(kind, ("fwd",) + key, 0, Cin, Cout, Cin * KK, KK, range(KK), N=N,
                                             C0=chans[0], C1=Cin - chans[0], Hin=Hin, Win=Win, Hout=Ho, Wout=Wo, K=K, S=S, pad=pad,
                                             pad_mode=pad_mode),))
        pick = _family_3x3(N, chans, Cout, Hin, Win, K, S, pad)
        if pick:
            return fwd(*pick)
        if S2WINO and CONV_MODE == "f32" and K == 4 and S == 2 and Cin == chans[0]:
            plan = fwd("s2wino", 3, "s2w")
            if lib().c2s_conv4x4s2_winograd_supported(C.byref(plan.launches[0].desc)):
                return plan
        plan = fwd("igemm", 0)
        first = lib().c2s_conv3x3_smallcin_supported(C.byref(plan.launches[0].desc))
        return plan._replace(family="smallcin") if first else plan
    assert op == "dgrad", op
    Cs, c_lo = chans[si], sum(chans[:si])
    radj = 1 if (pad_mode == _lib.PAD_REFLECT and pad > 0) else 0
    w = (c_lo * KK, Cout, Cs, KK, Cin * KK)

    def dgrad(family, kind, key, taps, **desc):
        return ConvPlan(family, (_launch(kind, ("dgrad",) + key, *w, taps, N=N, Hin=Ho, Win=Wo, Hout=Hin, Wout=Win,
                                         accumulate=accumulate, reflect_adjoint=radj, **desc),))
    if S == 1:
        taps = [(K - 1 - ky) * K + (K - 1 - kx) for ky in range(K) for kx in range(K)]
        pick = _family_3x3(N, [Cout], Cs, Hin, Win, K, S, pad)
        if pick:
            return dgrad(pick[0], pick[1], (pick[2], si), taps, K=K, pad=1)
        return dgrad("igemm", 0, (si,), taps, K=K, pad=K - 1 - pad)
    assert S == 2 and Hin == 2 * Ho and Win == 2 * Wo, (K, S, pad, Hin, Win)
    if (K, pad) in PARITY_GEOMETRIES:
        return _transposed_launches("parity", ("dgrad", si), *w, K, pad, N, Ho, Wo, accumulate, radj)
    assert K == 4 and pad == 1, (K, pad)
    plan = dgrad("s2dgrad", 4, ("s2d", si), range(KK), K=4, S=2, pad=1)
    if S2WINO and CONV_MODE == "f32" and lib().c2s_conv4x4s2_dgrad_winograd_supported(C.byref(plan.launches[0].desc)):
        return plan
    return _transposed_launches("xpair", ("dgrad", si), *w, K, pad, N, Ho, Wo, accumulate, radj)


PROFILE: Optional[dict] = None


def _run_conv(ctx: Ctx, plan: ConvPlan, wname: str, weight: Tensor, src0: Tensor, src1: Optional[Tensor],
              bias: Optional[Tensor], out: Tensor, valid: Optional[Tensor]) -> None:
    entry, two_sources, has_bias, profiled = CONV_FAMILIES[plan.family]
    for desc, key, kind, *where in plan.launches:
        request = ((wname,) + key, weight, *where)
        packed = _pack_bf16x3(ctx, *request)[:2] if plan.family == "bf16x3" else ctx.pack(*request, kind=kind)[:1]
        args = [src0.data_ptr()] + ([_ptr(src1)] if two_sources else []) + [t.data_ptr() for t in packed] + \
            ([_ptr(bias)] if has_bias else []) + [out.data_ptr(), _ptr(valid), _stream()]
        prof = PROFILE
        timed = profiled and prof is not None and all(getattr(desc, k) == v for k, v in prof["match"].items())
        if timed:
            e0, e1 = torch.cuda.Event(enable_timing=True), torch.cuda.Event(enable_timing=True)
            e0.record()
        check(getattr(lib(), entry)(C.byref(desc), *args), entry[4:])
        if timed:
            e1.record()
            prof["events"].append((e0, e1))


def _wgrad_slices(ctx: Ctx, N: int, Hout: int, Wout: int, S: int, cin: int, cout: int) -> int:
    TP = 64 if S == 2 else 128
    l2 = 5
    while l2 > 2 and (1 << l2) > Wout:
        l2 -= 1
    PC = 1 << l2
    ntiles = N * ((Wout + PC - 1) // PC) * ((Hout + TP // PC - 1) // (TP // PC))
    blocks = ((cin + 31) // 32) * ((cout + 63) // 64)
    return max(1, min(ntiles, (2 * ctx.cus) // blocks))


def _wgrad(ctx: Ctx, srcs: Sequence[Tensor], gout: Tensor, Cout: int, Hout: int, Wout: int, K: int, S: int, pad: int,
           pad_mode: int, dst: Tensor, so: int, sc: int, taps: Sequence[int], accumulate: int,
           valid: Optional[Tensor]) -> None:
    if ctx.tape is not None and _side_ok():
        ctx.tape.defer(lambda: _wgrad_launch(ctx, srcs, gout, Cout, Hout, Wout, K, S, pad, pad_mode, dst, so, sc, taps,
                                             accumulate, valid), [gout, *srcs])
        if srcs[0].shape[0] * Hout * Wout >= SIDE_FLUSH_POSITIONS:
            ctx.tape.flush_side()
    else:
        _wgrad_launch(ctx, srcs, gout, Cout, Hout, Wout, K, S, pad, pad_mode, dst, so, sc, taps, accumulate, valid)


def _wgrad_desc(ctx: Ctx, srcs: Sequence[Tensor], Cout: int, Hout: int, Wout: int, K: int, S: int, pad: int,
                pad_mode: int) -> WgradDesc:
    N, C0, Hin, Win = srcs[0].shape
    C1 = srcs[1].shape[1] if len(srcs) > 1 else 0
    return WgradDesc(N, C0, C1, Hin, Win, Cout, Hout, Wout, K, K, S, pad, pad, pad_mode,
                     _wgrad_slices(ctx, N, Hout, Wout, S, C0 + C1, Cout))


def _wgrad_launch(ctx: Ctx, srcs: Sequence[Tensor], gout: Tensor, Cout: int, Hout: int, Wout: int, K: int, S: int, pad: int,
                  pad_mode: int, dst: Tensor, so: int, sc: int, taps: Sequence[int], accumulate: int,
                  valid: Optional[Tensor]) -> None:
    s0 = srcs[0]
    s1 = srcs[1] if len(srcs) > 1 else None
    d = _wgrad_desc(ctx, srcs, Cout, Hout, Wout, K, S, pad, pad_mode)
    nfl = lib().c2s_wgrad_workspace_floats(C.byref(d))
    batched = REDUCE_BATCH and ctx.tape is not None
    tag = f":acc{len(ctx.ws.reduce_post)}" if accumulate else ""
    slabs = ctx.ws.get(f"wgrad_slabs:{dst.data_ptr()}:{so}:{taps[0]}{tag}" if batched else "wgrad_slabs", nfl)
    check(lib().c2s_conv_wgrad(C.byref(d), s0.data_ptr(), _ptr(s1), gout.data_ptr(), slabs.data_ptr(), slabs.numel(),
                               _ptr(valid), _stream()), "conv_wgrad")
    if batched:
        if accumulate:
            ctx.ws.reduce_post.append((slabs, dst.data_ptr(), so, sc, tuple(taps), d))
        else:
            ctx.ws.reduce_jobs.append((bytes(d), slabs.data_ptr(), dst.data_ptr(), so, sc, tuple(taps), accumulate, d))
        ctx.tape.finalizers[id(ctx.ws)] = ctx.ws.run_reduce_batch
    else:
        check(lib().c2s_wgrad_reduce(C.byref(d), slabs.data_ptr(), dst.data_ptr(), so, sc, _tap_array(taps), accumulate,
                                     _stream()), "wgrad_reduce")


def conv2d(ctx: Ctx, srcs: Sequence[Tensor], wname: str, bname: Optional[str], K: int, S: int, pad: int,
           pad_mode: int, valid: Optional[Tensor], need_input_grad: bool = True) -> Tensor:
    W = ctx.p[wname]
    Cout, Cin = W.shape[0], W.shape[1]
    s0 = srcs[0]
    s1 = srcs[1] if len(srcs) > 1 else None
    N, C0, Hin, Win = s0.shape
    C1 = s1.shape[1] if s1 is not None else 0
    assert C0 + C1 == Cin, (wname, C0, C1, Cin)
    chans = [C0, C1] if C1 else [C0]
    Ho = (Hin + 2 * pad - K) // S + 1
    Wo = (Win + 2 * pad - K) // S + 1
    KK = K * K
    out = torch.empty(N, Cout, Ho, Wo, device=s0.device, dtype=torch.float32)
    _run_conv(ctx, conv_plan("fwd", N, chans, Cout, Hin, Win, K, S, pad, pad_mode), wname, W, s0, s1,
              ctx.p[bname] if bname else None, out, valid)
    if not ctx.mark([out], srcs, [wname, bname]):
        return out
    tape = ctx.tape
    tape.track(out)
    train_w = ctx.trains(wname)
    need_src = [need_input_grad and ctx.needs(src) for src in srcs]
    if AGG_SKIP_TERM and (K, S, pad) == (4, 2, 1):
        for si, src in enumerate(srcs):
            plan = conv_plan("dgrad", N, chans, Cout, Hin, Win, K, S, pad, pad_mode, si, 0) if need_src[si] else None
            if plan is not None and plan.family == "s2dgrad":
                tape.s2d_sources[src.data_ptr()] = (plan.launches[0].desc, _ptr(valid))

    def bwd():
        g = tape.pop_grad(out)
        if g is None:
            return
        if train_w:
            gw, acc = ctx.grad_sink(wname)
            _log("conv2d", wname, "wgrad")
            _wgrad(ctx, srcs, g, Cout, Ho, Wo, K, S, pad, pad_mode, gw, Cin * KK, KK, list(range(KK)), acc, valid)
        for si, src in enumerate(srcs):
            if not need_src[si]:
                continue
            _log("conv2d", wname, "dgrad")
            if src.data_ptr() in tape.skip_terms:
                plan = conv_plan("dgrad", N, chans, Cout, Hin, Win, K, S, pad, pad_mode, si, 0)
                if plan.family == "s2dgrad" and tape.s2d_sources.get(src.data_ptr(), (None, 0))[1] == _ptr(valid):
                    term = tape.take_skip_term(src)
                    desc, key, kind, *where = plan.launches[0]
                    packed = ctx.pack((wname,) + key, W, *where, kind=kind)[0]
                    check(lib().c2s_conv4x4s2_dgrad_winograd_skip(
                        C.byref(desc), g.data_ptr(), packed.data_ptr(), tape.grads[src.data_ptr()].data_ptr(), _ptr(valid),
                        term.a_up.data_ptr(), term.gskip.data_ptr(), term.n_head, term.T, _stream()),
                        "conv4x4s2_dgrad_winograd_skip")
                    continue
            gin, accf = tape.grad_buffer(src)
            _run_conv(ctx, conv_plan("dgrad", N, chans, Cout, Hin, Win, K, S, pad, pad_mode, si, accf), wname, W, g, None, None,
                      gin, valid)

    tape.record(bwd)
    return out


def conv_transpose2d(ctx: Ctx, x: Tensor, wname: str, bname: str, K: int = 4, pad: int = 1) -> Tensor:
    Wt = ctx.p[wname]
    Cin, Cout = Wt.shape[0], Wt.shape[1]
    N, _, H, Wd = x.shape
    assert (K, pad) == (4, 1) or (K, pad) in PARITY_GEOMETRIES, (K, pad)
    KK = K * K
    out = torch.empty(N, Cout, 2 * H, 2 * Wd, device=x.device, dtype=torch.float32)
    _run_conv(ctx, conv_plan("tfwd", N, [Cin], Cout, H, Wd, K, 2, pad, _lib.PAD_ZEROS), wname, Wt, x, None, ctx.p[bname], out,
              None)
    if not ctx.mark([out], [x], [wname, bname]):
        return out
    tape = ctx.tape
    tape.track(out)
    train_w, need_x = ctx.trains(wname), ctx.needs(x)

    def bwd():
        g = tape.pop_grad(out)
        if g is None:
            return
        if train_w:
            gw, acc = ctx.grad_sink(wname)
            _log("conv_transpose2d", wname, "wgrad")
            _wgrad(ctx, [g], x, Cin, H, Wd, K, 2, pad, _lib.PAD_ZEROS, gw, Cout * KK, KK, list(range(KK)), acc, None)
        if not need_x:
            return
        _log("conv_transpose2d", wname, "dgrad")
        gin, accf = tape.grad_buffer(x)
        _run_conv(ctx, conv_plan("tdgrad", N, [Cin], Cout, H, Wd, K, 2, pad, _lib.PAD_ZEROS, 0, accf), wname, Wt, g, None, None,
                  gin, None)

    tape.record(bwd)
    return out


def depthwise_conv2d(ctx: Ctx, x: Tensor, wname: str, K: int, S: int, pad: int, pad_mode: int,
                     valid: Optional[Tensor], bname: Optional[str] = None) -> Tensor:
    W = ctx.p[wname]
    N, Cc, Hin, Win = x.shape
    Ho = (Hin + 2 * pad - K) // S + 1
    Wo = (Win + 2 * pad - K) // S + 1
    out = torch.empty(N, Cc, Ho, Wo, device=x.device, dtype=torch.float32)
    check(lib().c2s_dwconv_fwd(x.data_ptr(), W.data_ptr(), out.data_ptr(), _ptr(valid), N, Cc, Hin, Win, K, S, pad,
                               pad_mode, _stream()), "dwconv_fwd")
    if bname is not None:
        check(lib().c2s_channel_bias_add(out.data_ptr(), ctx.p[bname].data_ptr(), _ptr(valid), N, Cc, Ho * Wo, _stream()),
              "channel_bias_add")
    if not ctx.mark([out], [x], [wname, bname]):
        return out
    tape = ctx.tape
    tape.track(out)
    train_w, need_x = ctx.trains(wname), ctx.needs(x)

    def bwd():
        g = tape.pop_grad(out)
        if g is None:
            return
        if train_w:
            gw, acc = ctx.grad_sink(wname)
            part = ctx.ws.get("dw_partial", N * Cc * K * K)
            tgt = gw if not acc else torch.empty_like(gw)
            _log("depthwise_conv2d", wname, "wgrad")

            def wgrad():
                check(lib().c2s_dwconv_wgrad(x.data_ptr(), g.data_ptr(), part.data_ptr(), tgt.data_ptr(), _ptr(valid), N, Cc,
                                             Hin, Win, K, S, pad, pad_mode, _stream()), "dwconv_wgrad")
                if acc:
                    check(lib().c2s_add_inplace(gw.data_ptr(), tgt.data_ptr(), tgt.numel(), _stream()), "add_inplace")

            if _side_ok():
                tape.defer(wgrad, [x, g, tgt, part])
            else:
                wgrad()
        if not need_x:
            return
        _log("depthwise_conv2d", wname, "dgrad")
        gin, accf = tape.grad_buffer(x)
        check(lib().c2s_dwconv_dgrad(g.data_ptr(), W.data_ptr(), gin.data_ptr(), _ptr(valid), N, Cc, Hin, Win, K, S, pad,
                                     pad_mode, accf, _stream()), "dwconv_dgrad")

    tape.record(bwd)
    return out


ONEPASS_NORM = _os.environ.get("C2S_NORM_ONEPASS", "1") != "0"
ONEPASS_MIN_HW = int(_os.environ.get("C2S_NORM_ONEPASS_MIN_HW", "1024"))


def norm_act(ctx: Ctx, x: Tensor, prefix: str, kind: int, groups: int, relu: bool, residual: Optional[Tensor],
             valid: Optional[Tensor], pad_value: float = 0.0, conv_bias: Optional[str] = None, affine: bool = True) -> Tensor:
    N, Cc = x.shape[0], x.shape[1]
    HW = x[0, 0].numel()
    batch = kind == _lib.NORM_BATCH
    training = 1 if (ctx.training or not batch) else 0
    d = NormDesc(N, Cc, HW, kind, groups if not batch else 1, training if batch else 1, ctx.eps, ctx.momentum)
    if affine:
        gamma, beta = ctx.p[prefix + ".weight"], ctx.p[prefix + ".bias"]
    else:
        gamma = ctx.ws.get(f"ones{Cc}", Cc)
        beta = ctx.ws.get(f"zeros{Cc}", Cc)
        check(lib().c2s_fill(gamma.data_ptr(), Cc, 1.0, _stream()), "fill")
        check(lib().c2s_fill(beta.data_ptr(), Cc, 0.0, _stream()), "fill")
    rm = ctx.b.get(prefix + ".running_mean") if batch else None
    rv = ctx.b.get(prefix + ".running_var") if batch else None
    ngroups = Cc if batch else N * groups
    gstats = torch.empty(ngroups * 2, device=x.device, dtype=torch.float32)
    row_ab = torch.empty(N * Cc * 3, device=x.device, dtype=torch.float32)
    nws = lib().c2s_norm_workspace_floats(C.byref(d))
    ws = ctx.ws.get("norm", nws)
    y = torch.empty_like(x)
    nbt = ctx.b.get(prefix + ".num_batches_tracked") if (batch and ctx.training) else None
    sync_bytes = (lib().c2s_norm_onepass_sync_bytes(C.byref(d), 1 if valid is not None else 0)
                  if ONEPASS_NORM and HW >= ONEPASS_MIN_HW else 0)
    if sync_bytes:
        sync = ctx.ws.sync_area(sync_bytes)
        check(lib().c2s_norm_fwd_onepass(C.byref(d), x.data_ptr(), gamma.data_ptr(), beta.data_ptr(), _ptr(rm), _ptr(rv),
                                         _ptr(nbt), gstats.data_ptr(), row_ab.data_ptr(), _ptr(residual), y.data_ptr(),
                                         int(relu), _ptr(valid), float(pad_value), sync.data_ptr(), sync.numel(), _stream()),
              "norm_fwd_onepass")
    else:
        check(lib().c2s_norm_fwd(C.byref(d), x.data_ptr(), gamma.data_ptr(), beta.data_ptr(), _ptr(rm), _ptr(rv), _ptr(nbt),
                                 gstats.data_ptr(), row_ab.data_ptr(), _ptr(residual), y.data_ptr(), int(relu),
                                 ws.data_ptr(), ws.numel(), _ptr(valid), float(pad_value), _stream()), "norm_fwd")
    pnames = [prefix + ".weight", prefix + ".bias"] if affine else []
    if not ctx.mark([y], [x, residual], pnames + [conv_bias]):
        return y
    tape = ctx.tape
    tape.track(y)
    need_x = ctx.needs(x)
    need_res = residual is not None and ctx.needs(residual)
    train_gamma, train_beta = [affine and ctx.trains(n) for n in pnames] or [False, False]

    def bwd():
        g = tape.pop_grad(y)
        if g is None:
            return
        if need_res:
            tape.add_grad(residual, g, own=True)
            gx = torch.empty_like(g) if need_x else None
        else:
            gx = g if need_x else None
        if not need_x:
            if train_gamma or train_beta:
                _log("norm", prefix, "params")
                wsn = ctx.ws.get("norm", nws)
                check(lib().c2s_norm_bwd(C.byref(d), x.data_ptr(), g.data_ptr(), gamma.data_ptr(), gstats.data_ptr(),
                                         row_ab.data_ptr(), int(relu), None,
                                         ctx.grad_sink(pnames[0])[0].data_ptr() if train_gamma else None,
                                         ctx.grad_sink(pnames[1])[0].data_ptr() if train_beta else None, None,
                                         wsn.data_ptr(), wsn.numel(), _ptr(valid), _stream()), "norm_bwd")
            return
        _log("norm", prefix, "dgrad")
        if affine and ctx.trainable is not None:
            dgamma = ctx.grad_sink(pnames[0])[0] if train_gamma else None
            dbeta = ctx.grad_sink(pnames[1])[0] if train_beta else None
        elif affine:
            dgamma, _ = ctx.grad_sink(prefix + ".weight")
            dbeta, _ = ctx.grad_sink(prefix + ".bias")
        elif ctx.trainable is None:
            dgamma = torch.empty(Cc, device=x.device, dtype=torch.float32)
            dbeta = torch.empty(Cc, device=x.device, dtype=torch.float32)
        else:
            dgamma = dbeta = None
        dbias = ctx.grad_sink(conv_bias)[0] if ctx.trains(conv_bias) else None
        want_params = dgamma is not None or dbeta is not None or dbias is not None
        if want_params:
            _log("norm", prefix, "params")

        def norm_bwd(ws_, dg_, db_, dbi_):
            if sync_bytes:
                sync = ctx.ws.sync_area(sync_bytes)
                check(lib().c2s_norm_bwd_onepass(C.byref(d), x.data_ptr(), g.data_ptr(), gamma.data_ptr(), gstats.data_ptr(),
                                                 row_ab.data_ptr(), int(relu), gx.data_ptr(), _ptr(dg_), _ptr(db_), _ptr(dbi_),
                                                 ws_.data_ptr(), ws_.numel(), _ptr(valid), sync.data_ptr(), sync.numel(),
                                                 _stream()), "norm_bwd_onepass")
            else:
                check(lib().c2s_norm_bwd(C.byref(d), x.data_ptr(), g.data_ptr(), gamma.data_ptr(), gstats.data_ptr(),
                                         row_ab.data_ptr(), int(relu), gx.data_ptr(), _ptr(dg_), _ptr(db_), _ptr(dbi_),
                                         ws_.data_ptr(), ws_.numel(), _ptr(valid), _stream()), "norm_bwd")

        if _side_ok() and want_params:
            ws2 = torch.empty(nws, device=x.device, dtype=torch.float32)
            norm_bwd(ws2, None, None, None)
            tape.defer(lambda: check(lib().c2s_norm_bwd_params(C.byref(d), ws2.data_ptr(), _ptr(dgamma), _ptr(dbeta),
                                                               _ptr(dbias), _ptr(valid), _stream()), "norm_bwd_params"),
                       [ws2] if affine else [ws2, dgamma, dbeta])
        else:
            norm_bwd(ctx.ws.get("norm", nws), dgamma, dbeta, dbias)
        tape.add_grad(x, gx)

    bwd.saved = {"group_stats": gstats, "row_ab": row_ab}
    tape.record(bwd)
    return y


def squeeze_excite(ctx: Ctx, x: Tensor, prefix: str, valid: Optional[Tensor], pad_value: float = 0.0) -> Tensor:
    W1, W2 = ctx.p[prefix + ".sae.1.weight"], ctx.p[prefix + ".sae.3.weight"]
    N, Cc = x.shape[:2]
    HW = x[0, 0].numel()
    R = Cc // 16
    assert tuple(W1.shape) == (R, Cc) and tuple(W2.shape) == (Cc, R), (prefix, W1.shape, W2.shape)
    dev = x.device
    pooled = torch.empty(N, Cc, device=dev, dtype=torch.float32)
    hidden = torch.empty(N, R, device=dev, dtype=torch.float32)
    scale = torch.empty(N, Cc, device=dev, dtype=torch.float32)
    y = torch.empty_like(x)
    nws = lib().c2s_se_workspace_floats(N, Cc, HW)
    ws = ctx.ws.get("se", nws)
    check(lib().c2s_se_fwd(x.data_ptr(), W1.data_ptr(), W2.data_ptr(), pooled.data_ptr(), hidden.data_ptr(), scale.data_ptr(),
                           y.data_ptr(), _ptr(valid), N, Cc, HW, float(pad_value), ws.data_ptr(), ws.numel(), _stream()), "se_fwd")
    wn = [prefix + ".sae.1.weight", prefix + ".sae.3.weight"]
    if not ctx.mark([y], [x], wn):
        return y
    tape = ctx.tape
    tape.track(y)
    need_x = ctx.needs(x)

    def bwd():
        g = tape.pop_grad(y)
        if g is None:
            return
        (g1, a1), (g2, a2) = [ctx.grad_sink(n) if ctx.trains(n) else (torch.empty_like(ctx.p[n]), 0) for n in wn]
        if ctx.trains(wn[0]) or ctx.trains(wn[1]):
            _log("squeeze_excite", prefix, "params")
        if need_x:
            _log("squeeze_excite", prefix, "dgrad")
        ws_ = ctx.ws.get("se", nws)
        check(lib().c2s_se_bwd(x.data_ptr(), g.data_ptr(), W1.data_ptr(), W2.data_ptr(), pooled.data_ptr(), hidden.data_ptr(),
                               scale.data_ptr(), g.data_ptr(), g1.data_ptr(), g2.data_ptr(), a1, a2, _ptr(valid), N, Cc, HW,
                               ws_.data_ptr(), ws_.numel(), _stream()), "se_bwd")
        if need_x:
            tape.add_grad(x, g)

    tape.record(bwd)
    return y


def temporal_aggregate(ctx: Ctx, x5: Tensor, attn: Tensor, valid: Optional[Tensor], n_head: int,
                       mode: str = "att_group") -> Tensor:
    B, T, Cc, H, W = x5.shape
    src_attn = attn
    if mode == "att_mean":
        attn = torch.empty_like(src_attn)
        check(lib().c2s_attn_head_mean(src_attn.data_ptr(), attn.data_ptr(), n_head, src_attn[0].numel(), _stream()), "attn_head_mean")
    elif mode == "mean":
        attn = torch.empty(n_head, B, T, 1, 1, device=x5.device, dtype=torch.float32)
        check(lib().c2s_frame_mean_weights(_ptr(valid), attn.data_ptr(), n_head, B, T, _stream()), "frame_mean_weights")
    elif mode != "att_group":
        raise ValueError(f"agg_mode {mode!r}")
    h, w = attn.shape[-2:]
    d = AggDesc(B, T, Cc, H, W, n_head, h, w)
    out = torch.empty(B, Cc, H, W, device=x5.device, dtype=torch.float32)
    check(lib().c2s_temporal_aggregate_fwd(C.byref(d), x5.data_ptr(), attn.data_ptr(), _ptr(valid), out.data_ptr(),
                                           _stream()), "temporal_aggregate_fwd")
    if not ctx.mark([out], [x5, src_attn if mode != "mean" else None]):
        return out
    tape = ctx.tape
    tape.track(out)
    need_x = ctx.needs(x5)
    need_a = ctx.needs(src_attn) if mode != "mean" else ctx.trainable is None

    def bwd():
        g = tape.pop_grad(out)
        if g is None:
            return
        key = x5.data_ptr()
        reg = tape.s2d_sources.get(key)
        skip = (AGG_SKIP_TERM and reg is not None and mode in ("att_group", "att_mean") and need_x and need_a
                and key not in tape.grads and key not in tape.skip_terms and reg[1] == _ptr(valid)
                and (reg[0].N, reg[0].Cout, reg[0].Hout, reg[0].Wout) == (B * T, Cc, H, W)
                and lib().c2s_conv4x4s2_dgrad_winograd_skip_supported(C.byref(reg[0]), n_head, T) == 1)
        gx, accx = tape.grad_buffer(x5) if need_x else (None, 0)
        if need_x:
            _log("temporal_aggregate", mode, "dgrad")
        if not need_a:
            gattn = None
        elif mode == "att_group":
            gattn = tape.grad_of(attn)
            if gattn is None:
                gattn = torch.zeros_like(attn)
                tape.grads[attn.data_ptr()] = gattn
        else:
            gattn = torch.zeros_like(attn)
        nws = lib().c2s_temporal_aggregate_bwd_workspace_floats(C.byref(d))
        ws = ctx.ws.get("agg", nws)
        if skip:
            used = {t.name for t in tape.skip_terms.values()}
            name = next(n for n in (f"agg_a_up:{H}x{W}:{k}" for k in range(len(used) + 1)) if n not in used)
            a_up = ctx.ws.get(name, nws)
            check(lib().c2s_temporal_aggregate_bwd_skip(C.byref(d), x5.data_ptr(), attn.data_ptr(), _ptr(valid), g.data_ptr(),
                                                        gx.data_ptr(), accx, gattn.data_ptr(), a_up.data_ptr(),
                                                        ws.data_ptr(), ws.numel(), _stream()), "temporal_aggregate_bwd_skip")
            tape.skip_terms[key] = SkipTerm(a_up, g, d, valid, n_head, T, name)
        else:
            check(lib().c2s_temporal_aggregate_bwd(C.byref(d), x5.data_ptr(), attn.data_ptr(), _ptr(valid), g.data_ptr(),
                                                   _ptr(gx), accx, _ptr(gattn),
                                                   ws.data_ptr(), ws.numel(), _stream()), "temporal_aggregate_bwd")
        if mode == "att_mean" and need_a:
            tgt, acca = tape.grad_buffer(src_attn)
            check(lib().c2s_attn_head_mean_bwd(gattn.data_ptr(), tgt.data_ptr(), n_head, src_attn[0].numel(), acca, _stream()),
                  "attn_head_mean_bwd")

    tape.record(bwd)
    return out


def positional_table(dates: Tensor, d: int, period: float) -> Tensor:
    dl = dates.to(torch.int64).contiguous()
    pe = torch.empty(*dl.shape, d, device=dl.device, dtype=torch.float32)
    check(lib().c2s_positional_table_ex(dl.data_ptr(), pe.data_ptr(), dl.numel(), float(period), d, _stream()), "positional_table")
    return pe


PE_MODES = {"rel": 0, "doy": 1, "abs_rel": 2, "linear": 3, "abs_rel_doy": 4, "abs_rel_linear": 5}


def ltae_attention(ctx: Ctx, x5: Tensor, dates: Tensor, valid: Optional[Tensor], prefix: str, n_head: int, d_k: int,
                   d_model: int, period: float, dropout_p: float, with_embedding: bool, seed: int,
                   keep: Optional[Tensor], seed_dev: Optional[Tensor] = None, pe_mode: str = "rel",
                   need_attn: bool = True) -> Tuple[Optional[Tensor], Optional[Tensor]]:
    B, T, Cc, h, w = x5.shape
    HW = h * w
    rest = (prefix, n_head, d_k, d_model, period, dropout_p, with_embedding, seed, keep, seed_dev, pe_mode, need_attn)
    if HW % 4 == 0:
        return _ltae_attention_quads(ctx, x5, dates, valid, *rest)
    if keep is not None and ctx.training and dropout_p > 0:
        raise NotImplementedError("crop2seg_amd: an explicit attention keep mask needs an L-TAE map of h * w % 4 == 0 pixels; "
                                  f"got {h} x {w}")
    HWp = (HW + 3) // 4 * 4
    tape = ctx.tape
    xp = torch.zeros(B, T, Cc, 1, HWp, device=x5.device, dtype=torch.float32)
    xp[..., :HW].copy_(x5.reshape(B, T, Cc, 1, HW))
    if tape is not None and ctx.needs(x5):
        tape.track(xp)
        if ctx.trainable is not None:
            ctx._needs.add(xp.data_ptr())

        def bwd_in():
            g = tape.pop_grad(xp)
            if g is not None:
                tape.add_grad(x5, g[..., :HW].reshape(x5.shape).contiguous())

        tape.record(bwd_in)
    nops = len(tape.ops) if tape is not None else 0
    outs_p = _ltae_attention_quads(ctx, xp, dates, valid, *rest)
    outs = tuple(None if o is None else o[..., :HW].reshape(*o.shape[:-2], h, w).contiguous() for o in outs_p)
    if tape is not None and len(tape.ops) > nops:
        pairs = [(o, op) for o, op in zip(outs, outs_p) if o is not None]
        for o, _ in pairs:
            tape.track(o)
        if ctx.trainable is not None:
            ctx._needs.update(o.data_ptr() for o, _ in pairs)

        def bwd_out():
            for o, op in pairs:
                g = tape.pop_grad(o)
                if g is not None:
                    gp = torch.zeros_like(op)
                    gp[..., :HW].copy_(g.reshape(*op.shape[:-2], 1, HW))
                    tape.add_grad(op, gp)

        tape.record(bwd_out)
    return outs


def _ltae_attention_quads(ctx: Ctx, x5: Tensor, dates: Tensor, valid: Optional[Tensor], prefix: str, n_head: int, d_k: int,
                          d_model: int, period: float, dropout_p: float, with_embedding: bool, seed: int,
                          keep: Optional[Tensor], seed_dev: Optional[Tensor] = None, pe_mode: str = "rel",
                          need_attn: bool = True) -> Tuple[Optional[Tensor], Optional[Tensor]]:
    B, T, Cc, h, w = x5.shape
    HW = h * w
    Q = ctx.p[prefix + ".attention_head.Q"]
    Wk = ctx.p[prefix + ".attention_head.fc1_k.weight"]
    bk = ctx.p[prefix + ".attention_head.fc1_k.bias"]
    Wc3 = ctx.p[prefix + ".inconv.weight"]
    bc = ctx.p[prefix + ".inconv.bias"]
    gamma, beta = ctx.p[prefix + ".in_norm.weight"], ctx.p[prefix + ".in_norm.bias"]
    mode = PE_MODES[pe_mode]
    if mode != 0 and (n_head, d_model) != (16, 256):
        raise NotImplementedError("crop2seg_amd: the learnable positional encoders (csrc/ltae_pe.hip) are built for n_head=16, "
                                  f"d_model=256; got n_head={n_head}, d_model={d_model}")
    dev = x5.device
    pe256 = sin256 = d0 = d1 = None
    if mode == 0:
        pe = positional_table(dates, d_model // n_head, period)
    else:
        pe = ctx.ws.get("ltae_pe_zero", B * T * (d_model // n_head))
        check(lib().c2s_fill(pe.data_ptr(), B * T * (d_model // n_head), 0.0, _stream()), "fill")
        dl = dates.to(torch.int64)
        two = mode in (2, 4, 5)
        kmode = {4: 1, 5: 3}.get(mode, mode)
        d0 = (dl[..., 0] if two else dl).contiguous()
        d1 = dl[..., 1].contiguous() if two else None
        enc = prefix + (".positional_encoder_abs.fc" if mode == 2 else ".positional_encoder.fc")
        enc2 = prefix + ".positional_encoder_abs.fc" if mode in (4, 5) else None
        peW, peb = ctx.p[enc + ".weight"], ctx.p[enc + ".bias"]
        pe256 = torch.empty(B, T, d_model, device=dev, dtype=torch.float32)
        sin256 = torch.empty(B, T, d_model, device=dev, dtype=torch.float32) if kmode == 3 else None
        bad = ctx.ws.bufs.get("ltae_pe_bad")
        if bad is None:
            bad = ctx.ws.bufs["ltae_pe_bad"] = torch.zeros(1, device=dev, dtype=torch.int32)
        check(lib().c2s_ltae_pe_table(kmode, d0.data_ptr(), _ptr(d1), float(period), peW.data_ptr(), peb.data_ptr(),
                                      pe256.data_ptr(), _ptr(sin256), bad.data_ptr(), B * T, _stream()), "ltae_pe_table")
        if enc2 is not None:
            check(lib().c2s_ltae_pe_abs_add(d1.data_ptr(), ctx.p[enc2 + ".weight"].data_ptr(), ctx.p[enc2 + ".bias"].data_ptr(),
                                            pe256.data_ptr(), bad.data_ptr(), B * T, _stream()), "ltae_pe_abs_add")
    U = torch.empty(n_head, Cc, device=dev, dtype=torch.float32)
    s0 = torch.empty(B, T, n_head, device=dev, dtype=torch.float32)
    qwk = torch.empty(n_head, d_model, device=dev, dtype=torch.float32)
    check(lib().c2s_ltae_fold_fwd_ex(Q.data_ptr(), Wk.data_ptr(), bk.data_ptr(), Wc3.data_ptr(), bc.data_ptr(), pe.data_ptr(),
                                     U.data_ptr(), s0.data_ptr(), qwk.data_ptr(), B * T, Cc, n_head, d_k, d_model, _stream()),
          "ltae_fold_fwd")
    if mode != 0:
        check(lib().c2s_ltae_pe_fwd(qwk.data_ptr(), pe256.data_ptr(), None, s0.data_ptr(), None, B, T, HW, 0, _stream()),
              "ltae_pe_fwd")
    Wc = Wc3.view(d_model, Cc)
    p_eff = dropout_p if ctx.training else 0.0
    d = LtaeDesc(B, T, Cc, HW, n_head, d_model, ctx.eps, p_eff, seed, _ptr(keep) if p_eff > 0 else None, _ptr(seed_dev))
    skip_attn = not need_attn and mode == 0 and with_embedding and (
        bool(lib().c2s_ltae_attn_optional(C.byref(d))) if ctx.tape is not None else lib().c2s_ltae_fwd_path(C.byref(d)) == 2)
    attn = None if skip_attn else torch.empty(n_head, B, T, h, w, device=x5.device, dtype=torch.float32)
    if skip_attn and ctx.tape is not None:
        keep_bits = torch.empty(B * HW * n_head, device=x5.device, dtype=torch.int64)
        d.keep_bits = keep_bits.data_ptr()
        ctx.tape.track(keep_bits)
    need_pre = ctx.tape is not None or lib().c2s_ltae_fwd_path(C.byref(d)) in (1, 4)
    attn_pre = torch.empty(n_head, B, T, h, w, device=x5.device, dtype=torch.float32) if need_pre else None
    emb = torch.empty(B, d_model, h, w, device=x5.device, dtype=torch.float32) if with_embedding else None
    stats = torch.empty(B * HW * n_head * 2, device=x5.device, dtype=torch.float32)
    Ud, s0d = U, s0
    fws = ctx.ws.get("ltae_fwd", lib().c2s_ltae_fwd_workspace_floats(C.byref(d)))
    prof = PROFILE
    timed = prof is not None and "ltae_events" in prof
    if timed:
        e0, e1 = torch.cuda.Event(enable_timing=True), torch.cuda.Event(enable_timing=True)
        e0.record()
    check(lib().c2s_ltae_attn_fwd_ws(C.byref(d), x5.data_ptr(), gamma.data_ptr(), beta.data_ptr(), Ud.data_ptr(),
                                     s0d.data_ptr(), Wc.data_ptr(), bc.data_ptr(), pe.data_ptr(), _ptr(valid),
                                     _ptr(attn), _ptr(attn_pre), _ptr(emb), stats.data_ptr(), fws.data_ptr(),
                                     fws.numel(), _stream()), "ltae_fwd")
    if timed:
        e1.record()
        prof["ltae_events"].append((e0, e1))
    if mode != 0 and emb is not None:
        check(lib().c2s_ltae_pe_fwd(None, pe256.data_ptr(), attn.data_ptr(), None, emb.data_ptr(), B, T, HW, 1, _stream()),
              "ltae_pe_fwd")
    fold_names = [prefix + ".attention_head.Q", prefix + ".attention_head.fc1_k.weight",
                  prefix + ".attention_head.fc1_k.bias", prefix + ".inconv.weight", prefix + ".inconv.bias"]
    norm_names = [prefix + ".in_norm.weight", prefix + ".in_norm.bias"]
    pe_names = [] if mode == 0 else [enc + ".weight", enc + ".bias"] + ([] if enc2 is None else [enc2 + ".weight", enc2 + ".bias"])
    if not ctx.mark([emb, attn], [x5], fold_names + norm_names + pe_names):
        return emb, attn
    tape = ctx.tape
    need_x = ctx.needs(x5)
    train_norm = any(ctx.trains(n) for n in norm_names)
    train_fold = any(ctx.trains(n) for n in fold_names + pe_names)
    if d.keep is not None:
        tape.track(keep)
    if attn is not None:
        tape.track(attn)
    if emb is not None:
        tape.track(emb)

    def bwd():
        g_attn = tape.pop_grad(attn) if attn is not None else None
        g_emb = tape.pop_grad(emb) if emb is not None else None
        if g_attn is None and g_emb is None:
            return
        gx = torch.empty_like(x5) if need_x else None
        dev = x5.device
        gU = torch.empty(n_head, Cc, device=dev)
        gs0 = torch.empty(B, T, n_head, device=dev)
        gWc = torch.empty(d_model, Cc, device=dev)
        gbc = torch.empty(d_model, device=dev)
        pending = []

        def sink(name):
            if not ctx.trains(name):
                return torch.empty_like(ctx.p[name])
            dst, acc = ctx.grad_sink(name)
            if not acc:
                return dst
            tmp = torch.empty_like(dst)
            pending.append((dst, tmp))
            return tmp

        ggam = sink(norm_names[0]) if train_norm else None
        gbet = sink(norm_names[1]) if train_norm else None
        if need_x:
            _log("ltae", prefix, "dgrad")
        if train_norm or train_fold:
            _log("ltae", prefix, "params")
        nws = lib().c2s_ltae_bwd_workspace_floats(C.byref(d))
        ws = ctx.ws.get("ltae", nws)
        if mode != 0 and g_emb is not None:
            g_tot = torch.empty_like(attn)
# ... 167 lines not shown
```

include/c2s_hip.h:

```cpp
#ifndef C2S_HIP_H
#define C2S_HIP_H

#include <stddef.h>
#include <stdint.h>

#ifdef __cplusplus
extern "C" {
#endif

#define C2S_OK 0
#define C2S_EINVAL (-1)
#define C2S_ELAUNCH (-2)
#define C2S_ENOSPACE (-3)

#define C2S_PAD_ZEROS 0
#define C2S_PAD_REFLECT 1

#define C2S_NORM_GROUP 0
#define C2S_NORM_BATCH 1

int c2s_abi_version(void);
const char* c2s_last_error(void);
int c2s_init(int device);
int c2s_device_cus(void);

int c2s_pack_weights(const float* src, float* wpk, int cin, int cout, int coutP, int ntaps,
                     long stride_o, long stride_c, const int* host_tap_off, void* stream);
size_t c2s_pack_job_bytes(void);
int c2s_pack_job_fill(void* host_record, const float* src, float* dst, int cin, int cout, int coutP, int ntaps,
                      long stride_o, long stride_c, int winograd, const int* host_tap_off, int block_start);
int c2s_pack_job_blocks(int cin, int coutP, int ntaps, int winograd);
int c2s_pack_batch(const void* device_table, int njobs, int total_blocks, void* stream);


typedef struct c2s_conv_desc {
    int N, C0, C1;
    int Hin, Win;
    int Cout, CoutP;
    int Hout, Wout;
    int OutH, OutW;
    int KH, KW, S;
    int pad_y, pad_x;
    int pad_mode;
    int osy, osx, ooy, oox;
    int accumulate;
    int reflect_adjoint;
} c2s_conv_desc;

int c2s_conv_igemm(const c2s_conv_desc* d, const float* src0, const float* src1, const float* wpk,
                   const float* bias, float* out, const int* valid, void* stream);
int c2s_conv_igemm_split(const c2s_conv_desc* d, int cus);

int c2s_conv3x3_smallcin_supported(const c2s_conv_desc* d);
int c2s_conv3x3_smallcin(const c2s_conv_desc* d, const float* src, const float* wpk, const float* bias, float* out,
                         const int* valid, void* stream);

int c2s_conv_xpair(const c2s_conv_desc* d, const float* src, const float* wpk, const float* bias, float* out,
                   const int* valid, void* stream);

size_t c2s_winograd_packed_floats(int cin, int coutP);
int c2s_pack_weights_winograd(const float* src, float* upk, int cin, int cout, int coutP, long stride_o, long stride_c,
                              const int* host_tap_off, void* stream);
int c2s_conv3x3_winograd(const c2s_conv_desc* d, const float* src0, const float* src1, const float* upk,
                         const float* bias, float* out, const int* valid, void* stream);

size_t c2s_winograd16_packed_floats(int cin, int coutP);
int c2s_pack_weights_winograd16(const float* src, float* upk, int cin, int cout, int coutP, long stride_o, long stride_c,
                                const int* host_tap_off, void* stream);
int c2s_conv3x3_winograd16_supported(const c2s_conv_desc* d);
int c2s_conv3x3_winograd16(const c2s_conv_desc* d, const float* src0, const float* src1, const float* upk,
                           const float* bias, float* out, const int* valid, void* stream);

size_t c2s_s2wino_packed_floats(int cin, int coutP);
int c2s_pack_weights_s2wino(const float* src, float* upk, int cin, int cout, int coutP, long stride_o, long stride_c,
                            const int* host_tap_off, void* stream);
int c2s_conv4x4s2_winograd_supported(const c2s_conv_desc* d);
int c2s_conv4x4s2_winograd(const c2s_conv_desc* d, const float* src, const float* upk, const float* bias, float* out,
                           const int* valid, void* stream);

size_t c2s_s2dgrad_packed_floats(int kc, int csP);
int c2s_pack_weights_s2dgrad(const float* src, float* upk, int kc, int cs, int csP, long stride_c, long stride_k,
                             const int* host_tap_off, void* stream);
int c2s_conv4x4s2_dgrad_winograd_supported(const c2s_conv_desc* d);
int c2s_conv4x4s2_dgrad_winograd(const c2s_conv_desc* d, const float* gy, const float* upk, float* gx, const int* valid,
                                 void* stream);
int c2s_conv4x4s2_dgrad_winograd_skip_supported(const c2s_conv_desc* d, int n_head, int T);
int c2s_conv4x4s2_dgrad_winograd_skip(const c2s_conv_desc* d, const float* gy, const float* upk, float* gx, const int* valid,
                                      const float* a_up, const float* gskip, int n_head, int T, void* stream);

size_t c2s_bf16x3_packed_elems(int cin, int coutP);
int c2s_pack_weights_bf16x3(const float* src, void* whi, void* wlo, int cin, int cout, int coutP, int ntaps,
                            long stride_o, long stride_c, const int* host_tap_off, void* stream);
int c2s_conv3x3_bf16x3(const c2s_conv_desc* d, const float* src0, const float* src1, const void* whi,
                       const void* wlo, const float* bias, float* out, const int* valid, void* stream);
void c2s_bf16x3_set_single_product(int on);

typedef struct c2s_wgrad_desc {
    int N, C0, C1, Hin, Win;
    int Cout;
    int Hout, Wout;
    int KH, KW, S, pad_y, pad_x, pad_mode;
    int nslices;
} c2s_wgrad_desc;

size_t c2s_wgrad_workspace_floats(const c2s_wgrad_desc* d);
int c2s_conv_wgrad(const c2s_wgrad_desc* d, const float* src0, const float* src1, const float* gout,
                   float* slabs, size_t slab_floats, const int* valid, void* stream);
int c2s_wgrad_algorithms(int winograd_3x3, int winograd_4x4s2);
int c2s_wgrad_path(const c2s_wgrad_desc* d, int* family);
int c2s_wgrad_reduce(const c2s_wgrad_desc* d, const float* slabs, float* dst, long stride_o, long stride_c,
                     const int* host_tap_off, int accumulate, void* stream);
size_t c2s_wgrad_reduce_job_bytes(void);
int c2s_wgrad_reduce_job_blocks(const c2s_wgrad_desc* d);
int c2s_wgrad_reduce_job_fill(void* host_record, const c2s_wgrad_desc* d, const float* slabs, float* dst, long stride_o,
                              long stride_c, const int* host_tap_off, int accumulate, int block_start);
int c2s_wgrad_reduce_batch(const void* device_table, int njobs, int total_blocks, void* stream);

int c2s_dwconv_fwd(const float* in, const float* w, float* out, const int* valid, int N, int C, int Hin, int Win,
                   int K, int S, int pad, int pad_mode, void* stream);
int c2s_dwconv_dgrad(const float* gout, const float* w, float* gin, const int* valid, int N, int C, int Hin, int Win,
                     int K, int S, int pad, int pad_mode, int accumulate, void* stream);
int c2s_dwconv_wgrad(const float* in, const float* gout, float* partial, float* gw, const int* valid, int N, int C,
                     int Hin, int Win, int K, int S, int pad, int pad_mode, void* stream);
int c2s_dwconv_paths(int Hin, int Win, int K, int S, int pad, int pad_mode, int* fwd, int* dgrad, int* wgrad);

typedef struct c2s_norm_desc {
    int N, C, HW;
    int kind;
    int groups;
    int training;
    float eps, momentum;
} c2s_norm_desc;

size_t c2s_norm_workspace_floats(const c2s_norm_desc* d);
int c2s_norm_fwd(const c2s_norm_desc* d, const float* x, const float* gamma, const float* beta,
                 float* running_mean, float* running_var, long long* num_batches_tracked, float* group_stats, float* row_ab,
                 const float* residual, float* y, int relu, float* workspace, size_t ws_floats, const int* valid,
                 float pad_value, void* stream);
int c2s_norm_bwd(const c2s_norm_desc* d, const float* x, const float* g, const float* gamma,
                 const float* group_stats, const float* row_ab, int relu, float* gx, float* dgamma,
                 float* dbeta, float* dbias, float* workspace, size_t ws_floats, const int* valid, void* stream);
int c2s_norm_bwd_params(const c2s_norm_desc* d, const float* workspace, float* dgamma, float* dbeta, float* dbias,
                        const int* valid, void* stream);

size_t c2s_norm_onepass_sync_bytes(const c2s_norm_desc* d, int has_valid);
int c2s_norm_fwd_onepass(const c2s_norm_desc* d, const float* x, const float* gamma, const float* beta,
                         float* running_mean, float* running_var, long long* num_batches_tracked, float* group_stats,
                         float* row_ab, const float* residual, float* y, int relu, const int* valid, float pad_value,
                         void* sync, size_t sync_bytes, void* stream);
int c2s_norm_bwd_onepass(const c2s_norm_desc* d, const float* x, const float* g, const float* gamma,
                         const float* group_stats, const float* row_ab, int relu, float* gx, float* dgamma, float* dbeta,
                         float* dbias, float* workspace, size_t ws_floats, const int* valid, void* sync,
                         size_t sync_bytes, void* stream);

size_t c2s_se_workspace_floats(int N, int C, int HW);
int c2s_channel_bias_add(float* x, const float* bias, const int* valid, int N, int C, int HW, void* stream);
int c2s_se_fwd(const float* x, const float* W1, const float* W2, float* pooled, float* hidden, float* scale, float* y,
               const int* valid, int N, int C, int HW, float pad_value, float* workspace, size_t ws_floats, void* stream);
int c2s_se_bwd(const float* x, const float* g, const float* W1, const float* W2, const float* pooled, const float* hidden,
               const float* scale, float* gx, float* gW1, float* gW2, int acc_w1, int acc_w2, const int* valid, int N, int C,
               int HW, float* workspace, size_t ws_floats, void* stream);

int c2s_frame_flags(const float* x, int* valid, int N, long frame_elems, float pad_value, void* stream);

typedef struct c2s_ltae_desc {
    int B, T, C, HW;
    int n_head, d_model;
    float eps;
    float dropout_p;
    uint64_t seed;
    const float* keep;
    const uint64_t* seed_dev;
    uint64_t* keep_bits;
} c2s_ltae_desc;

int c2s_ltae_attn_fwd(const c2s_ltae_desc* d, const float* x, const float* gamma, const float* beta,
                      const float* U, const float* s0, const float* Wc, const float* bc, const float* pe,
                      const int* valid, float* attn, float* attn_pre, float* emb, float* stats, void* stream);
size_t c2s_ltae_fwd_workspace_floats(const c2s_ltae_desc* d);
int c2s_ltae_attn_fwd_ws(const c2s_ltae_desc* d, const float* x, const float* gamma, const float* beta,
                         const float* U, const float* s0, const float* Wc, const float* bc, const float* pe,
                         const int* valid, float* attn, float* attn_pre, float* emb, float* stats,
                         float* workspace, size_t ws_floats, void* stream);
int c2s_ltae_uses_streaming(const c2s_ltae_desc* d);
int c2s_ltae_fwd_path(const c2s_ltae_desc* d);
int c2s_ltae_attn_optional(const c2s_ltae_desc* d);
int c2s_ltae_paths(const c2s_ltae_desc* d, int with_emb, int* fwd, int* bwd);
size_t c2s_ltae_bwd_workspace_floats(const c2s_ltae_desc* d);
int c2s_ltae_attn_bwd(const c2s_ltae_desc* d, const float* x, const float* gamma, const float* beta,
                      const float* U, const float* s0, const float* Wc, const float* bc, const float* pe,
                      const int* valid, const float* attn, const float* attn_pre, const float* stats,
                      const float* g_emb, const float* g_attn, float* gx, float* gU, float* gs0, float* gWc,
                      float* gbc, float* ggamma, float* gbeta, float* workspace, size_t ws_floats, void* stream);

int c2s_positional_table(const long long* dates, float* pe, long n, float period, void* stream);
int c2s_ltae_fold_fwd(const float* Q, const float* Wk, const float* bk, const float* Wc, const float* bc, const float* pe,
                      float* U, float* s0, float* qwk, int BT, int C, void* stream);
int c2s_ltae_fold_bwd(const float* Q, const float* Wk, const float* bk, const float* Wc, const float* bc, const float* pe,
                      const float* qwk, const float* gU, const float* gs0, const float* gWc_attn, const float* gbc_attn,
                      float* gQ, float* gWk, float* gbk, float* gWc, float* gbc, int BT, int C, int acc_mask,
                      float* workspace, size_t ws_floats, void* stream);
size_t c2s_ltae_fold_bwd_workspace_floats(void);
int c2s_positional_table_ex(const long long* dates, float* pe, long n, float period, int d_v, void* stream);
int c2s_ltae_fold_fwd_ex(const float* Q, const float* Wk, const float* bk, const float* Wc, const float* bc, const float* pe,
                         float* U, float* s0, float* qwk, int BT, int C, int n_head, int d_k, int d_model, void* stream);
int c2s_ltae_fold_bwd_ex(const float* Q, const float* Wk, const float* bk, const float* Wc, const float* bc, const float* pe,
                         const float* qwk, const float* gU, const float* gs0, const float* gWc_attn, const float* gbc_attn,
                         float* gQ, float* gWk, float* gbk, float* gWc, float* gbc, int BT, int C, int n_head, int d_k,
                         int d_model, int acc_mask, float* workspace, size_t ws_floats, void* stream);
size_t c2s_ltae_fold_bwd_workspace_floats_ex(int n_head, int d_model);

int c2s_ltae_pe_table(int mode, const long long* dates0, const long long* dates1, float period, const float* W, const float* b,
                      float* pe256, float* sin256, int* bad_days, int BT, void* stream);
int c2s_ltae_pe_abs_add(const long long* dates1, const float* W2, const float* b2, float* pe256, int* bad_days, int BT,
                        void* stream);
int c2s_ltae_pe_abs_bwd(const long long* dates1, const float* g_pe, float* gW2, float* gb2, int BT, void* stream);
int c2s_ltae_pe_fwd(const float* qwk, const float* pe256, const float* attn, float* s0, float* emb, int B, int T, int HW,
                    int phase, void* stream);
int c2s_ltae_pe_gattn(const float* g_emb, const float* pe256, const float* g_attn_in, float* g_attn_out, int B, int T, int HW,
                      void* stream);
int c2s_ltae_pe_bwd(int mode, const long long* dates0, const long long* dates1, const float* Q, const float* Wk,
                    const float* qwk, const float* pe256, const float* sin256, const float* attn, const float* g_emb,
                    const float* gs0, float* g_pe, float* gWk, float* gQ, float* gW, float* gb, int B, int T, int HW,
                    void* stream);
int c2s_ltae_pe_bwd_ex(int mode, const long long* dates0, const long long* dates1, const float* Q, const float* Wk,
                       const float* qwk, const float* pe256, const float* sin256, const float* attn, const float* g_emb,
                       const float* gs0, float* g_pe, float* gWk, float* gQ, float* gW, float* gb, int B, int T, int HW,
                       int d_k, void* stream);

int c2s_dropout_nchw(const float* x, float* y, int B, int C, int HW, float p, uint64_t seed, const uint64_t* seed_dev,
                     const float* keep, void* stream);
int c2s_pixel_gn_fwd(const float* x, const float* gamma, const float* beta, float* y, float* stats, int B, int C,
                     int HW, int groups, float eps, void* stream);
size_t c2s_pixel_gn_bwd_workspace_floats(int B, int C, int HW);
int c2s_pixel_gn_bwd(const float* x, const float* gy, const float* gamma, const float* stats, float* gx,
                     float* dgamma, float* dbeta, int B, int C, int HW, int groups, float* workspace,
                     size_t ws_floats, void* stream);

typedef struct c2s_agg_desc {
    int B, T, C, H, W;
    int n_head, h, w;
} c2s_agg_desc;

int c2s_attn_head_mean(const float* attn, float* v, int n_head, long n, void* stream);
int c2s_attn_head_mean_bwd(const float* gv, float* gattn, int n_head, long n, int accumulate, void* stream);
int c2s_frame_mean_weights(const int* valid, float* v, int n_head, int B, int T, void* stream);
int c2s_temporal_aggregate_fwd(const c2s_agg_desc* d, const float* x, const float* attn, const int* valid,
                               float* out, void* stream);
size_t c2s_temporal_aggregate_bwd_workspace_floats(const c2s_agg_desc* d);
int c2s_temporal_aggregate_bwd(const c2s_agg_desc* d, const float* x, const float* attn, const int* valid,
                               const float* gout, float* gx, int gx_accumulate, float* gattn,
                               float* workspace, size_t ws_floats, void* stream);
int c2s_temporal_aggregate_bwd_skip(const c2s_agg_desc* d, const float* x, const float* attn, const int* valid,
                                    const float* gout, float* gx, int gx_accumulate, float* gattn, float* a_up,
                                    float* workspace, size_t ws_floats, void* stream);
int c2s_agg_skip_term(const c2s_agg_desc* d, const float* a_up, const float* gout, const int* valid, float* gx, void* stream);

size_t c2s_cross_entropy_workspace_floats(int B, int HW);
int c2s_cross_entropy(const float* logits, const int64_t* target, const float* class_w, float* loss,
                      float* glogits, int B, int K, int HW, float label_smoothing, long long ignore_index,
                      float* workspace, size_t ws_floats, void* stream);
int c2s_adam_flat(float* p, const float* g, float* m, float* v, long n, float lr, float b1, float b2, float eps,
                  int step, const int* step_dev, float grad_scale, void* stream);

#define C2S_GUARD_STATUS_BYTES 32
size_t c2s_grad_sumsq_workspace_doubles(void);
int c2s_grad_sumsq(const float* g, const long* slots, const int* mask, int nslots, long total, double* workspace,
                   size_t ws_doubles, void* status, void* stream);
int c2s_step_decide(void* status, float max_grad_norm, float grad_scale, int skip_nonfinite, const int* mask,
                    int* slot_steps, int nslots, int* skip_count, void* stream);
int c2s_adam_slots(float* p, const float* g, float* m, float* v, const long* slots, const int* mask,
                   const int* slot_steps, int nslots, long total, float lr, float b1, float b2, float eps,
                   const void* status, void* stream);
int c2s_restore_if_skipped(float* dst, const float* saved, long n, const void* status, void* stream);

int c2s_metrics_update(const float* logits, const long long* target, long long* conf, long long* conf_top2,
                       long long* pred, long long* pred_top2, int B, int K, int HW, void* stream);
int c2s_confusion_add(const long long* pred, const long long* target, long long* conf, long n, int K, void* stream);
int c2s_loss_meter_add(const float* loss, double* acc, void* stream);
int c2s_boundary_target(const long long* y, long long* y_b, int B, int H, int W, void* stream);
int c2s_region_relabel(const long long* y, long long* y_out, int B, int H, int W, int keep_boundary, long long ignore_label,
                       void* stream);
size_t c2s_focal_ce_workspace_floats(void);
int c2s_focal_ce(const float* logits, const long long* target, float* loss, float* glogits, int B, int K, int HW,
                 float gamma, long long ignore_index, int accumulate_loss, float* workspace, size_t ws_floats,
                 void* stream);
int c2s_focal_ce_ex(const float* logits, const long long* target, const float* class_w, float* loss, float* glogits, int B,
                    int K, int HW, float gamma, long long ignore_index, int size_average, int accumulate_loss,
                    float* workspace, size_t ws_floats, void* stream);
size_t c2s_smooth_ce_workspace_floats(void);
int c2s_smooth_ce(const float* logits, const long long* target, const float* class_w, const float* bg_distrib, float* loss,
                  float* glogits, int B, int K, int H, int W, float label_smoothing, long long bg_index, int accumulate_loss,
                  float* workspace, size_t ws_floats, void* stream);
int c2s_smooth_ce_ex(const float* logits, const long long* target, const float* class_w, const float* bg_distrib, float* loss,
                     float* glogits, float* pixel_loss, int B, int K, int H, int W, float label_smoothing, long long bg_index,
                     int reduction, int accumulate_loss, float* workspace, size_t ws_floats, void* stream);
size_t c2s_recall_ce_workspace_floats(int B, int HW);
int c2s_recall_ce(const float* logits, const long long* target, float* loss, float* glogits, float* weights_out,
                  long long* counts_out, int B, int K, int HW, long long ignore_index, int accumulate_loss,
                  float* workspace, size_t ws_floats, void* stream);

int c2s_parcel_seeds(const float* scores, const float* boundary_scores, unsigned char* mask, long long* t1, int B, int K,
                     int H, int W, int from_logits, int boundary_code, float second_threshold, void* stream);
size_t c2s_label_components_workspace_bytes(int B, int H, int W);
int c2s_label_components(const unsigned char* mask, int* labels, int* count, int B, int H, int W, int min_size,
                         void* workspace, size_t ws_bytes, int* error, void* stream);
size_t c2s_parcel_vote_workspace_bytes(int B, int cap, int K);
int c2s_parcel_vote(const long long* pred, const int* labels, long long* out, int* parcel_class, int B, int H, int W, int K,
                    int cap, float bg_share, int outside, void* workspace, size_t ws_bytes, int* error, void* stream);
size_t c2s_parcel_soft_vote_workspace_bytes(int B, int cap, int K);
int c2s_parcel_soft_vote(const float* scores, const int* labels, long long* out, int* parcel_label, int* parcel_top2,
                         float* parcel_mean, int* parcel_pixels, int B, int K, int H, int W, int cap, int from_logits,
                         float bg_mean, int outside, void* workspace, size_t ws_bytes, int* error, void* stream);

#define C2S_SRC_F32 0
#define C2S_SRC_I16 1
#define C2S_SRC_U16 2
int c2s_collate_series(const void* src, int src_dtype, const long long* offsets, const long long* src_dates, float* x,
                       long long* dates, int* valid, int B, int T, int C, int Cs, int HW,
                       const int* host_channel_order, const float* host_mean, const float* host_std, float pad_value,
                       void* stream);
int c2s_collate_series_ndvi(const void* src, int src_dtype, const long long* offsets, const long long* src_dates, float* x,
                            long long* dates, int* valid, int B, int T, int C, int Cs, int HW, const int* host_channel_order,
                            const float* host_mean, const float* host_std, float pad_value, int ndvi_a, int ndvi_b,
                            void* stream);
int c2s_softmax_stitch(const float* logits, float* proba, long long* top1, int first_patch, int npatch, int K, int ph,
                       int pw, int grid_w, int out_h, int out_w, void* stream);

int c2s_window_count(int size, int patch, int stride);
int c2s_window_origin(int i, int size, int patch, int stride);
int c2s_cut_windows(const float* series, float* x, int T, int C, int H, int W, int ph, int pw, int stride_y, int stride_x,
                    int first_window, int nwin, int flip, const float* host_fill, void* stream);
int c2s_window_frames(const void* src, int src_dtype, const long long* dates, int* nodata_px, int* slots, int* counts,
                      long long* win_dates, int T, int Cs, int H, int W, int ph, int pw, int stride_y, int stride_x,
                      int first_window, int nwin, float nodata, int max_nodata_permille, void* stream);
int c2s_cut_windows_raw(const void* src, int src_dtype, float* x, const int* slots, int T, int C, int Cs, int H, int W, int ph,
                        int pw, int stride_y, int stride_x, int first_window, int nwin, int flip,
                        const int* host_channel_order, const float* host_mean, const float* host_std,
                        const float* host_fill, float pad_value, int ndvi_a, int ndvi_b, void* stream);
int c2s_softmax_blend(const float* logits, float* acc, float* wsum, const float* wy, const float* wx, int first_window,
                      int nwin, int K, int ph, int pw, int H, int W, int stride_y, int stride_x, int flip, void* stream);
int c2s_blend_finish(float* acc_proba, const float* wsum, long long* top1, int K, int H, int W, void* stream);

int c2s_fill(float* p, long n, float v, void* stream);
int c2s_add_inplace(float* dst, const float* src, long n, void* stream);

#ifdef __cplusplus
}
#endif
#endif
```

Baseline: 383.6.

## Fuse small-Cin first 3x3 conv with one-pass group norm and ReLU

Adds a fused kernel for the small-input-channel first 3x3 convolution that computes bias-added conv outputs, per-tile moments, publishes them through a grid-wide one-pass sync area, merges group statistics, and applies norm+ReLU in-kernel. It removes the separate norm pass that re-read the conv output and a kernel launch; the raw conv output is still stored when a tape exists for backward. This relies on cross-workgroup spin synchronisation with a poison fallback, which risks deadlock or stalls if not all workgroups are co-resident, and it adds register/LDS pressure.

```diff
diff --git a/crop2seg_amd/_lib.py b/crop2seg_amd/_lib.py
--- a/crop2seg_amd/_lib.py
+++ b/crop2seg_amd/_lib.py
@@ -104,6 +104,9 @@
     "c2s_norm_onepass_sync_bytes": (SZ, [C.POINTER(NormDesc), I]),
     "c2s_norm_fwd_onepass": (I, [C.POINTER(NormDesc), P, P, P, P, P, P, P, P, P, P, I, P, F, P, SZ, P]),
     "c2s_norm_bwd_onepass": (I, [C.POINTER(NormDesc), P, P, P, P, P, I, P, P, P, P, P, SZ, P, P, SZ, P]),
+    "c2s_conv3x3_smallcin_norm_supported": (I, [C.POINTER(ConvDesc), C.POINTER(NormDesc), I, I]),
+    "c2s_conv3x3_smallcin_norm_sync_bytes": (SZ, [C.POINTER(ConvDesc), C.POINTER(NormDesc)]),
+    "c2s_conv3x3_smallcin_norm": (I, [C.POINTER(ConvDesc), C.POINTER(NormDesc), P, P, P, P, P, P, P, P, P, P, F, P, SZ, P]),
     "c2s_se_workspace_floats": (SZ, [I, I, I]),
     "c2s_channel_bias_add": (I, [P, P, P, I, I, I, P]),
     "c2s_se_fwd": (I, [P, P, P, P, P, P, P, P, I, I, I, F, P, SZ, P]),
diff --git a/crop2seg_amd/backbones/functional.py b/crop2seg_amd/backbones/functional.py
--- a/crop2seg_amd/backbones/functional.py
+++ b/crop2seg_amd/backbones/functional.py
@@ -70,16 +70,22 @@
         cp = f"{prefix}.conv.{3 * i}"
         if depthwise_separable:
             t = E.depthwise_conv2d(ctx, x[0], cp + ".depthwise.weight", k, s, p, mode, valid)
-            y = E.conv2d(ctx, [t], cp + ".pointwise.weight", None, 1, 1, 0, _lib.PAD_ZEROS, valid)
+            t = E.conv2d(ctx, [t], cp + ".pointwise.weight", None, 1, 1, 0, _lib.PAD_ZEROS, valid)
             bias = None
         else:
-            y = E.conv2d(ctx, x, cp + ".weight", cp + ".bias", k, s, p, mode, valid,
-                         need_input_grad=need_input_grad or i > 0)
             bias = cp + ".bias"
         last = i == n_convs - 1
-        y = E.norm_act(ctx, y, f"{prefix}.conv.{3 * i + 1}", _norm_kind(norm), y.shape[1] if norm == "instance" else 4, True,
-                       residual if last else None, valid, spec.pad_value if valid is not None else 0.0, conv_bias=bias,
-                       affine=norm != "instance")
+        pad_value = spec.pad_value if valid is not None else 0.0
+        y = None
+        if not depthwise_separable:
+            y = E.conv_norm_fused(ctx, x, cp + ".weight", bias, f"{prefix}.conv.{3 * i + 1}", k, s, p, mode, _norm_kind(norm),
+                                  4, True, residual if last else None, valid, pad_value,
+                                  need_input_grad=need_input_grad or i > 0, affine=norm != "instance")
+            if y is None:
+                t = E.conv2d(ctx, x, cp + ".weight", bias, k, s, p, mode, valid, need_input_grad=need_input_grad or i > 0)
+        if y is None:
+            y = E.norm_act(ctx, t, f"{prefix}.conv.{3 * i + 1}", _norm_kind(norm), t.shape[1] if norm == "instance" else 4, True,
+                           residual if last else None, valid, pad_value, conv_bias=bias, affine=norm != "instance")
         x = [y]
     if add_squeeze:
         y = E.squeeze_excite(ctx, y, f"{prefix}.conv.{3 * n_convs}", valid, spec.pad_value if valid is not None else 0.0)
diff --git a/crop2seg_amd/build.py b/crop2seg_amd/build.py
--- a/crop2seg_amd/build.py
+++ b/crop2seg_amd/build.py
@@ -31,7 +31,7 @@
 def build(force: bool = False, verbose: bool = True) -> str:
     cc = hipcc()
     headers = [os.path.join(CSRC, "common.h"), os.path.join(CSRC, "ltae_drop.h"), os.path.join(CSRC, "ltae_long.h"),
-               os.path.join(CSRC, "parcels_uf.h"),
+               os.path.join(CSRC, "parcels_uf.h"), os.path.join(CSRC, "norm_shared.h"),
                os.path.join(os.path.dirname(HERE), "include", "c2s_hip.h")]
     objs, jobs = [], []
     for s in SOURCES:
diff --git a/crop2seg_amd/csrc/conv_first.hip b/crop2seg_amd/csrc/conv_first.hip
--- a/crop2seg_amd/csrc/conv_first.hip
+++ b/crop2seg_amd/csrc/conv_first.hip
@@ -1,4 +1,5 @@
 #include "common.h"
+#include "norm_shared.h"
 
 namespace {
 
@@ -10,6 +11,15 @@
     const int* valid;
     int N, Cin, H, W, Cout, CoutP;
     int tiles_x, tiles_y, ntiles;
+    const float* gamma;
+    const float* beta;
+    float* y;
+    float* gstats;
+    float* row_ab;
+    void* sync;
+    int wgs_x;
+    int groups, qpg;
+    float eps, pad_value;
 };
 
 constexpr int FT_ROWS = 8, FT_COLS = 32;
@@ -22,31 +32,25 @@
 constexpr int FT_CHS = ft_chs();
 
 template <int NP, bool REFLECT>
-__global__ __launch_bounds__(256, 2) void conv_first_kernel(FirstParams p) {
-    constexpr int NCH = 2 * NP;
-    constexpr int NE = NCH * FT_PR * FT_PC;
-    constexpr int EPT = (NE + 255) / 256;
-    __shared__ float patch[NCH * FT_CHS];
-    const int tid = threadIdx.x, lane = tid & 63, wave = __builtin_amdgcn_readfirstlane(tid >> 6);
-    const int px = lane & 31, kk = lane >> 5;
-    const int cb = blockIdx.y * 64;
-
-    float wreg[9][NP][2];
-#pragma unroll
-    for (int t = 0; t < 9; ++t)
-#pragma unroll
-        for (int s = 0; s < NP; ++s) {
-            const int ch = 2 * s + kk;
-#pragma unroll
-            for (int h = 0; h < 2; ++h) {
-                const float v = p.wpk[((size_t)t * p.Cin + (ch < p.Cin ? ch : 0)) * p.CoutP + cb + h * 32 + px];
-                wreg[t][s][h] = ch < p.Cin ? v : 0.f;
-            }
-        }
-    __shared__ float bias_s[64];
-    if (tid < 64) bias_s[tid] = (p.bias != nullptr && cb + tid < p.Cout) ? p.bias[cb + tid] : 0.f;
-
-    auto load_patch = [&](int tile, float (&v)[EPT]) {
+struct FirstTile {
+    static constexpr int NCH = 2 * NP;
+    static constexpr int NE = NCH * FT_PR * FT_PC;
+    static constexpr int EPT = (NE + 255) / 256;
+
+    static __device__ __forceinline__ void load_weights(const FirstParams& p, int cb, int px, int kk, float (&wreg)[9][NP][2]) {
+#pragma unroll
+        for (int t = 0; t < 9; ++t)
+#pragma unroll
+            for (int s = 0; s < NP; ++s) {
+                const int ch = 2 * s + kk;
+#pragma unroll
+                for (int h = 0; h < 2; ++h) {
+                    const float v = p.wpk[((size_t)t * p.Cin + (ch < p.Cin ? ch : 0)) * p.CoutP + cb + h * 32 + px];
+                    wreg[t][s][h] = ch < p.Cin ? v : 0.f;
+                }
+            }
+    }
+    static __device__ __forceinline__ void load_patch(const FirstParams& p, int tile, float (&v)[EPT]) {
         int tid = threadIdx.x;
         asm volatile("" : "+v"(tid));
         const int n = tile / (p.tiles_x * p.tiles_y);
@@ -70,8 +74,8 @@
             const float t = base[((size_t)chc * p.H + gy) * p.W + gx];
             v[j] = ok ? t : 0.f;
         }
-    };
-    auto store_patch = [&](const float (&v)[EPT]) {
+    }
+    static __device__ __forceinline__ void store_patch(float* patch, const float (&v)[EPT]) {
         int tid = threadIdx.x;
         asm volatile("" : "+v"(tid));
 #pragma unroll
@@ -80,25 +84,12 @@
             const int ch = e / (FT_PR * FT_PC), r2 = e - ch * (FT_PR * FT_PC);
             if (e < NE) patch[ch * FT_CHS + r2] = v[j];
         }
-    };
-    auto frame_ok = [&](int tile) {
+    }
+    static __device__ __forceinline__ bool frame_ok(const FirstParams& p, int tile) {
         return p.valid == nullptr || p.valid[tile / (p.tiles_x * p.tiles_y)] != 0;
-    };
-
-    int tile = blockIdx.x;
-    float pre[EPT];
-    if (tile < p.ntiles && frame_ok(tile)) load_patch(tile, pre);
-    for (; tile < p.ntiles; tile += gridDim.x) {
-        const bool ok = frame_ok(tile);
-        const int nxt = tile + gridDim.x;
-        if (ok) {
-            __syncthreads();
-            store_patch(pre);
-            __syncthreads();
-        }
-        if (nxt < p.ntiles && frame_ok(nxt)) load_patch(nxt, pre);
-        if (!ok) continue;
-        f32x16 acc[2][2];
+    }
+    static __device__ __forceinline__ void mfma(const float* patch, const float (&wreg)[9][NP][2], int wave, int px, int kk,
+                                                f32x16 (&acc)[2][2]) {
 #pragma unroll
         for (int r = 0; r < 2; ++r)
 #pragma unroll
@@ -119,23 +110,253 @@
                     acc[1][0] = __builtin_amdgcn_mfma_f32_32x32x2f32(wreg[ky * 3 + kx][s][0], b1, acc[1][0], 0, 0, 0);
                     acc[1][1] = __builtin_amdgcn_mfma_f32_32x32x2f32(wreg[ky * 3 + kx][s][1], b1, acc[1][1], 0, 0, 0);
                 }
-        const int n = tile / (p.tiles_x * p.tiles_y);
-        const int rem = tile - n * (p.tiles_x * p.tiles_y);
-        const int y = (rem / p.tiles_x) * FT_ROWS + 2 * wave, x0 = (rem % p.tiles_x) * FT_COLS;
-        const size_t plane = (size_t)p.H * p.W;
-        float* ub = p.out + ((size_t)n * p.Cout + cb) * plane + (size_t)y * p.W + x0;
-        const unsigned lo = (unsigned)(4 * kk) * (unsigned)plane + (unsigned)px;
+    }
+};
+
+__host__ __device__ constexpr int first_channel(int h, int i) { return h * 32 + (i & 3) + 8 * (i >> 2); }
+struct FirstOut {
+    size_t plane, off;
+    unsigned lo;
+    int n, rem;
+};
+__device__ __forceinline__ FirstOut first_out(const FirstParams& p, int tile, int cb, int wave, int px, int kk) {
+    FirstOut o;
+    o.n = tile / (p.tiles_x * p.tiles_y);
+    o.rem = tile - o.n * (p.tiles_x * p.tiles_y);
+    const int y = (o.rem / p.tiles_x) * FT_ROWS + 2 * wave, x0 = (o.rem % p.tiles_x) * FT_COLS;
+    o.plane = (size_t)p.H * p.W;
+    o.off = ((size_t)o.n * p.Cout + cb) * o.plane + (size_t)y * p.W + x0;
+    o.lo = (unsigned)(4 * kk) * (unsigned)o.plane + (unsigned)px;
+    return o;
+}
+
+template <int NP, bool REFLECT>
+__global__ __launch_bounds__(256, 2) void conv_first_kernel(FirstParams p) {
+    using T = FirstTile<NP, REFLECT>;
+    __shared__ float patch[T::NCH * FT_CHS];
+    const int tid = threadIdx.x, lane = tid & 63, wave = __builtin_amdgcn_readfirstlane(tid >> 6);
+    const int px = lane & 31, kk = lane >> 5;
+    const int cb = blockIdx.y * 64;
+
+    float wreg[9][NP][2];
+    T::load_weights(p, cb, px, kk, wreg);
+    __shared__ float bias_s[64];
+    if (tid < 64) bias_s[tid] = (p.bias != nullptr && cb + tid < p.Cout) ? p.bias[cb + tid] : 0.f;
+
+    int tile = blockIdx.x;
+    float pre[T::EPT];
+    if (tile < p.ntiles && T::frame_ok(p, tile)) T::load_patch(p, tile, pre);
+    for (; tile < p.ntiles; tile += gridDim.x) {
+        const bool ok = T::frame_ok(p, tile);
+        const int nxt = tile + gridDim.x;
+        if (ok) {
+            __syncthreads();
+            T::store_patch(patch, pre);
+            __syncthreads();
+        }
+        if (nxt < p.ntiles && T::frame_ok(p, nxt)) T::load_patch(p, nxt, pre);
+        if (!ok) continue;
+        f32x16 acc[2][2];
+        T::mfma(patch, wreg, wave, px, kk, acc);
+        const FirstOut o = first_out(p, tile, cb, wave, px, kk);
+        float* ub = p.out + o.off;
 #pragma unroll
         for (int h = 0; h < 2; ++h)
 #pragma unroll
             for (int i = 0; i < 16; ++i) {
-                const int og = h * 32 + (i & 3) + 8 * (i >> 2);
-                float* op = ub + (size_t)og * plane;
+                const int og = first_channel(h, i);
+                float* op = ub + (size_t)og * o.plane;
                 const float b = bias_s[og + 4 * kk];
-                op[lo] = acc[0][h][i] + b;
-                op[lo + p.W] = acc[1][h][i] + b;
-            }
-    }
+                op[o.lo] = acc[0][h][i] + b;
+                op[o.lo + p.W] = acc[1][h][i] + b;
+            }
+    }
+}
+
+constexpr int FN_MAXI = 64 * OP_MAXG;
+constexpr int FN_QLEN = 16 * FT_ROWS * FT_COLS;
+
+template <int NP, bool REFLECT, bool STORE_RAW>
+__global__ __launch_bounds__(256, 2) void conv_first_norm_kernel(FirstParams p) {
+    using T = FirstTile<NP, REFLECT>;
+    __shared__ float patch[T::NCH * FT_CHS];
+    __shared__ float bias_s[64], gamma_s[64], beta_s[64];
+    __shared__ unsigned s_hdr[2];
+    __shared__ float s_wm[4][4][2];
+    __shared__ float s_stat[4][2];
+    __shared__ float s_part[4][2][FN_MAXI];
+    const int tid = threadIdx.x, lane = tid & 63, wave = __builtin_amdgcn_readfirstlane(tid >> 6);
+    const int px = lane & 31, kk = lane >> 5;
+    const int bx = blockIdx.x % p.wgs_x, cb = (blockIdx.x / p.wgs_x) * 64;
+    const int tpf = p.tiles_x * p.tiles_y;
+
+    float wreg[9][NP][2];
+    T::load_weights(p, cb, px, kk, wreg);
+    if (tid < 64) {
+        bias_s[tid] = p.bias != nullptr ? p.bias[cb + tid] : 0.f;
+        gamma_s[tid] = p.gamma[cb + tid];
+        beta_s[tid] = p.beta[cb + tid];
+    }
+    const SyncView sv = sync_view(p.sync);
+    unsigned epoch;
+    bool poisoned;
+    onepass_begin(sv, s_hdr, epoch, poisoned);
+
+    const int quarters = p.Cout / 16, qglob = cb / 16 + wave;
+    const int grp = qglob / p.qpg;
+    const bool grp_first = qglob % p.qpg == 0;
+
+    int tile = bx;
+    float pre[T::EPT];
+    if (tile < p.ntiles && T::frame_ok(p, tile)) T::load_patch(p, tile, pre);
+    for (; tile < p.ntiles; tile += p.wgs_x) {
+        const bool ok = T::frame_ok(p, tile);
+        const int nxt = tile + p.wgs_x;
+        if (ok) {
+            __syncthreads();
+            T::store_patch(patch, pre);
+            __syncthreads();
+        }
+        if (nxt < p.ntiles && T::frame_ok(p, nxt)) T::load_patch(p, nxt, pre);
+        const FirstOut o = first_out(p, tile, cb, wave, px, kk);
+        float* yb = p.y + o.off;
+        const long row0 = (long)o.n * p.Cout + cb + 16 * wave;
+        if (!ok) {
+#pragma unroll
+            for (int h = 0; h < 2; ++h)
+#pragma unroll
+                for (int i = 0; i < 16; ++i) {
+                    float* op = yb + (size_t)first_channel(h, i) * o.plane;
+                    op[o.lo] = p.pad_value;
+                    op[o.lo + p.W] = p.pad_value;
+                }
+            if (o.rem == 0) {
+                if (lane < 16) { p.row_ab[(row0 + lane) * 3] = 0.f; p.row_ab[(row0 + lane) * 3 + 1] = 0.f; p.row_ab[(row0 + lane) * 3 + 2] = 0.f; }
+                if (grp_first && lane == 0) { p.gstats[((long)o.n * p.groups + grp) * 2] = 0.f; p.gstats[((long)o.n * p.groups + grp) * 2 + 1] = 0.f; }
+            }
+            continue;
+        }
+        f32x16 acc[2][2];
+        T::mfma(patch, wreg, wave, px, kk, acc);
+#pragma unroll
+        for (int h = 0; h < 2; ++h)
+#pragma unroll
+            for (int i = 0; i < 16; ++i) {
+                const float b = bias_s[first_channel(h, i) + 4 * kk];
+                acc[0][h][i] = acc[0][h][i] + b;
+                acc[1][h][i] = acc[1][h][i] + b;
+            }
+        auto store_raw = [&]() {
+            float* ub = p.out + o.off;
+#pragma unroll
+            for (int h = 0; h < 2; ++h)
+#pragma unroll
+                for (int i = 0; i < 16; ++i) {
+                    float* op = ub + (size_t)first_channel(h, i) * o.plane;
+                    __builtin_nontemporal_store(acc[0][h][i], op + o.lo);
+                    __builtin_nontemporal_store(acc[1][h][i], op + o.lo + p.W);
+                }
+        };
+#pragma unroll
+        for (int q = 0; q < 4; ++q) {
+            const int h = q >> 1, i0 = (q & 1) * 8;
+            float s = 0.f;
+#pragma unroll
+            for (int j = 0; j < 8; ++j) s += acc[0][h][i0 + j] + acc[1][h][i0 + j];
+            s = wave_sum(s);
+            const float mean = s / (float)(FN_QLEN / 4);
+            float m2 = 0.f;
+#pragma unroll
+            for (int j = 0; j < 8; ++j) {
+                const float a = acc[0][h][i0 + j] - mean, b = acc[1][h][i0 + j] - mean;
+                m2 += a * a + b * b;
+            }
+            m2 = wave_sum(m2);
+            if (lane == 0) { s_wm[q][wave][0] = mean; s_wm[q][wave][1] = m2; }
+        }
+        __syncthreads();
+        {
+            double cnt = 0.0, mean = 0.0, m2 = 0.0;
+#pragma unroll
+            for (int w = 0; w < 4; ++w) {
+                const double nb = FN_QLEN / 4, tot = cnt + nb;
+                const double dm = (double)s_wm[wave][w][0] - mean;
+                mean += dm * (nb / tot);
+                m2 += (double)s_wm[wave][w][1] + dm * dm * (cnt * nb / tot);
+                cnt = tot;
+            }
+            onepass_publish(sv, ((long)o.n * quarters + qglob) * tpf + o.rem, epoch, (float)mean, (float)m2, lane);
+            if (STORE_RAW) store_raw();
+            const long g0 = ((long)o.n * quarters + (long)grp * p.qpg) * tpf;
+            onepass_sweep(sv, g0, p.qpg * tpf, epoch, lane, poisoned, s_part[wave][0], s_part[wave][1]);
+            float mu, rstd, unb;
+            merge_moments(p.qpg * tpf, lane, p.eps, [&](int it, float& pm, float& pm2, int& len) {
+                pm = s_part[wave][0][it];
+                pm2 = s_part[wave][1][it];
+                len = FN_QLEN;
+                return true;
+            }, mu, rstd, unb);
+            if (lane == 0) { s_stat[wave][0] = mu; s_stat[wave][1] = rstd; }
+            if (o.rem == 0) {
+                if (lane < 16) {
+                    p.row_ab[(row0 + lane) * 3] = gamma_s[16 * wave + lane] * rstd;
+                    p.row_ab[(row0 + lane) * 3 + 1] = beta_s[16 * wave + lane];
+                    p.row_ab[(row0 + lane) * 3 + 2] = mu;
+                }
+                if (grp_first && lane == 0) { p.gstats[((long)o.n * p.groups + grp) * 2] = mu; p.gstats[((long)o.n * p.groups + grp) * 2 + 1] = rstd; }
+            }
+        }
+        __syncthreads();
+#pragma unroll
+        for (int h = 0; h < 2; ++h)
+#pragma unroll
+            for (int i = 0; i < 16; ++i) {
+                const int og = first_channel(h, i), q = 2 * h + (i >> 3);
+                const float mu = s_stat[q][0], rstd = s_stat[q][1];
+                const float a = gamma_s[og + 4 * kk] * rstd, b = beta_s[og + 4 * kk];
+                const bool failed = mu != mu;
+                const float t0 = fwd_element(acc[0][h][i], mu, a, b, 1, false, 0.f);
+                const float t1 = fwd_element(acc[1][h][i], mu, a, b, 1, false, 0.f);
+                float* op = yb + (size_t)og * o.plane;
+                __builtin_nontemporal_store(failed ? mu : t0, op + o.lo);
+                __builtin_nontemporal_store(failed ? mu : t1, op + o.lo + p.W);
+            }
+    }
+    onepass_end(sv, epoch);
+}
+
+int fill_params(const c2s_conv_desc* d, FirstParams& p) {
+    p = FirstParams{};
+    p.N = d->N; p.Cin = d->C0; p.H = d->Hin; p.W = d->Win; p.Cout = d->Cout; p.CoutP = d->CoutP;
+    p.tiles_x = d->Win / FT_COLS; p.tiles_y = d->Hin / FT_ROWS;
+    const long nt = (long)d->N * p.tiles_x * p.tiles_y;
+    C2S_REQUIRE(nt < (1L << 30), "conv3x3_smallcin: too many tiles");
+    p.ntiles = (int)nt;
+    return C2S_OK;
+}
+
+template <int NP, bool REFLECT, bool STORE_RAW>
+int norm_cap_of() {
+    static thread_local int cap = 0;
+    if (cap == 0) {
+        int per_cu = 0;
+        if (hipOccupancyMaxActiveBlocksPerMultiprocessor(&per_cu, conv_first_norm_kernel<NP, REFLECT, STORE_RAW>, 256, 0) != hipSuccess || per_cu < 1) per_cu = 1;
+        if (per_cu > 8) per_cu = 8;
+        cap = c2s_cus() * per_cu;
+    }
+    return cap;
+}
+template <bool STORE_RAW>
+int norm_cap_raw(const c2s_conv_desc* d) {
+    const bool reflect = d->pad_mode == C2S_PAD_REFLECT;
+    if (d->C0 <= 4) return reflect ? norm_cap_of<2, true, STORE_RAW>() : norm_cap_of<2, false, STORE_RAW>();
+    return reflect ? norm_cap_of<5, true, STORE_RAW>() : norm_cap_of<5, false, STORE_RAW>();
+}
+int norm_cap(const c2s_conv_desc* d, int store_raw) {
+    if (store_raw > 0) return norm_cap_raw<true>(d);
+    if (store_raw == 0) return norm_cap_raw<false>(d);
+    const int a = norm_cap_raw<true>(d), b = norm_cap_raw<false>(d);
+    return a < b ? a : b;
 }
 
 }
@@ -154,12 +375,9 @@
                 "conv3x3_smallcin: needs 3x3/s1/pad1, one source of <= 10 channels, Cout %% 64 == 0, H %% 8 == 0, W %% 32 == 0");
     if (d->pad_mode == C2S_PAD_REFLECT) C2S_REQUIRE(d->Hin >= 2 && d->Win >= 2, "conv3x3_smallcin: reflect needs planes >= 2x2");
     FirstParams p;
+    if (int rc = fill_params(d, p)) return rc;
     p.src = src; p.wpk = wpk; p.bias = bias; p.out = out; p.valid = valid;
-    p.N = d->N; p.Cin = d->C0; p.H = d->Hin; p.W = d->Win; p.Cout = d->Cout; p.CoutP = d->CoutP;
-    p.tiles_x = d->Win / FT_COLS; p.tiles_y = d->Hin / FT_ROWS;
-    const long nt = (long)d->N * p.tiles_x * p.tiles_y;
-    C2S_REQUIRE(nt < (1L << 30), "conv3x3_smallcin: too many tiles");
-    p.ntiles = (int)nt;
+    const long nt = p.ntiles;
     const int cus = c2s_cus();
     const int wgs = (int)(nt < 2L * cus ? nt : 2L * cus);
     const dim3 grid(wgs, d->CoutP / 64);
@@ -175,3 +393,61 @@
     C2S_CHECK_LAUNCH("conv_first");
     return C2S_OK;
 }
+
+static int first_norm_wgs(const c2s_conv_desc* d, const c2s_norm_desc* nd, int relu, int has_residual, int store_raw) {
+    if (!c2s_conv3x3_smallcin_supported(d) || !nd) return 0;
+    if (d->pad_mode == C2S_PAD_REFLECT && (d->Hin < 2 || d->Win < 2)) return 0;
+    if (nd->kind != C2S_NORM_GROUP || !relu || has_residual) return 0;
+    if (nd->N != d->N || nd->C != d->Cout || (long)nd->HW != (long)d->Hin * d->Win) return 0;
+    if (nd->groups < 1 || nd->C % nd->groups != 0) return 0;
+    const int cpg = nd->C / nd->groups;
+    if (cpg != 16 && cpg != 32 && cpg != 64) return 0;
+    const long tpf = (long)(d->Hin / FT_ROWS) * (d->Win / FT_COLS);
+    if ((long)d->N * tpf >= (1L << 30)) return 0;
+    if ((cpg / 16) * tpf > FN_MAXI) return 0;
+    const int wgs_x = norm_cap(d, store_raw) / (d->CoutP / 64);
+    if (tpf > wgs_x) return 0;
+    return wgs_x;
+}
+
+extern "C" int c2s_conv3x3_smallcin_norm_supported(const c2s_conv_desc* d, const c2s_norm_desc* nd, int relu,
+                                                   int has_residual) {
+    return first_norm_wgs(d, nd, relu, has_residual, -1) > 0;
+}
+
+extern "C" size_t c2s_conv3x3_smallcin_norm_sync_bytes(const c2s_conv_desc* d, const c2s_norm_desc* nd) {
+    if (first_norm_wgs(d, nd, 1, 0, -1) <= 0) return 0;
+    return sync_bytes((long)d->N * (d->Cout / 16) * (d->Hin / FT_ROWS) * (d->Win / FT_COLS));
+}
+
+extern "C" int c2s_conv3x3_smallcin_norm(const c2s_conv_desc* d, const c2s_norm_desc* nd, const float* src, const float* wpk,
+                                         const float* bias, const float* gamma, const float* beta, float* raw, float* y,
+                                         float* group_stats, float* row_ab, const int* valid, float pad_value, void* sync,
+                                         size_t sync_nbytes, void* stream) {
+    C2S_REQUIRE(d && nd && src && wpk && gamma && beta && y && group_stats && row_ab && sync, "conv3x3_smallcin_norm: null pointer");
+    const int wgs_x = first_norm_wgs(d, nd, 1, 0, raw != nullptr);
+    C2S_REQUIRE(wgs_x > 0, "conv3x3_smallcin_norm: not taken by the fused form (c2s_conv3x3_smallcin_norm_supported() == 0): "
+                           "use c2s_conv3x3_smallcin and c2s_norm_fwd");
+    FirstParams p;
+    if (int rc = fill_params(d, p)) return rc;
+    C2S_REQUIRE(sync_nbytes >= sync_bytes((long)d->N * (d->Cout / 16) * p.tiles_x * p.tiles_y),
+                "conv3x3_smallcin_norm: sync area too small");
+    p.src = src; p.wpk = wpk; p.bias = bias; p.out = raw; p.valid = valid;
+    p.gamma = gamma; p.beta = beta; p.y = y; p.gstats = group_stats; p.row_ab = row_ab; p.sync = sync;
+    p.groups = nd->groups; p.qpg = nd->C / nd->groups / 16; p.eps = nd->eps; p.pad_value = pad_value;
+    p.wgs_x = p.ntiles < wgs_x ? p.ntiles : wgs_x;
+    const dim3 grid(p.wgs_x * (d->CoutP / 64));
+    hipStream_t st = (hipStream_t)stream;
+    const bool reflect = d->pad_mode == C2S_PAD_REFLECT;
+#define C2S_FIRST_NORM(NP_, R_)                                                                                         \
+    if (raw != nullptr) hipLaunchKernelGGL((conv_first_norm_kernel<NP_, R_, true>), grid, dim3(256), 0, st, p);         \
+    else hipLaunchKernelGGL((conv_first_norm_kernel<NP_, R_, false>), grid, dim3(256), 0, st, p);
+    if (d->C0 <= 4) {
+        if (reflect) { C2S_FIRST_NORM(2, true) } else { C2S_FIRST_NORM(2, false) }
+    } else {
+        if (reflect) { C2S_FIRST_NORM(5, true) } else { C2S_FIRST_NORM(5, false) }
+    }
+#undef C2S_FIRST_NORM
+    C2S_CHECK_LAUNCH("conv_first_norm");
+    return C2S_OK;
+}
diff --git a/crop2seg_amd/csrc/norm.hip b/crop2seg_amd/csrc/norm.hip
--- a/crop2seg_amd/csrc/norm.hip
+++ b/crop2seg_amd/csrc/norm.hip
@@ -1,4 +1,5 @@
 #include "common.h"
+#include "norm_shared.h"
 
 namespace {
 
@@ -20,12 +21,6 @@
 }
 
 
-__device__ __forceinline__ float fwd_element(float x, float mu, float a, float b, int relu, bool has_res, float r) {
-    float t = (x - mu) * a + b;
-    if (relu) t = fmaxf(t, 0.f);
-    if (has_res) t += r;
-    return t;
-}
 __device__ __forceinline__ float masked_grad(float g, float xc, float a, float b, int relu) {
     return (!relu || xc * a + b > 0.f) ? g : 0.f;
 }
@@ -111,34 +106,6 @@
         f(xv[k], has_r ? rv[k] : f32x4{0.f, 0.f, 0.f, 0.f}, o);
         if (STORE) *reinterpret_cast<f32x4u*>(out + base + lane * 4 + 256 * k) = o;
     }
-}
-
-template <typename P>
-__device__ __forceinline__ void merge_moments(int items, int lane, float eps, P partial, float& mean_f, float& rstd_f,
-                                              float& unbiased) {
-    double cnt = 0.0, sum = 0.0;
-    for (int it = lane; it < items; it += 64) {
-        float pm, pm2;
-        int len;
-        if (!partial(it, pm, pm2, len)) continue;
-        cnt += len;
-        sum += (double)pm * len;
-    }
-    for (int o = 32; o > 0; o >>= 1) { cnt += __shfl_xor(cnt, o, 64); sum += __shfl_xor(sum, o, 64); }
-    const double mean = cnt > 0 ? sum / cnt : 0.0;
-    double m2 = 0.0;
-    for (int it = lane; it < items; it += 64) {
-        float pm, pm2;
-        int len;
-        if (!partial(it, pm, pm2, len)) continue;
-        const double dm = (double)pm - mean;
-        m2 += (double)pm2 + dm * dm * len;
-    }
-    for (int o = 32; o > 0; o >>= 1) m2 += __shfl_xor(m2, o, 64);
-    const double var = cnt > 0 ? m2 / cnt : 0.0;
-    mean_f = (float)mean;
-    rstd_f = (float)(1.0 / sqrt(var + (double)eps));
-    unbiased = (float)(cnt > 1 ? m2 / (cnt - 1.0) : var);
 }
 
 template <typename P>
@@ -368,67 +335,6 @@
     if (lane == 0) part[item * 3 + 2] = sdx;
 }
 
-struct SyncView {
-    unsigned* hdr;
-    unsigned long long* gran;
-};
-__host__ __device__ inline size_t sync_bytes(long nitems) { return 64 + (size_t)nitems * 16; }
-__device__ __forceinline__ SyncView sync_view(void* base) {
-    SyncView v;
-    v.hdr = reinterpret_cast<unsigned*>(base);
-    v.gran = reinterpret_cast<unsigned long long*>(reinterpret_cast<char*>(base) + 64);
-    return v;
-}
-constexpr int OP_MAXG = 8;
-
-__device__ __forceinline__ void onepass_begin(const SyncView& sv, unsigned* s_hdr, unsigned& epoch, bool& poisoned) {
-    if (threadIdx.x == 0) {
-        s_hdr[0] = __hip_atomic_load(&sv.hdr[2], __ATOMIC_RELAXED, __HIP_MEMORY_SCOPE_AGENT);
-        s_hdr[1] = __hip_atomic_load(&sv.hdr[3], __ATOMIC_RELAXED, __HIP_MEMORY_SCOPE_AGENT);
-    }
-    __syncthreads();
-    epoch = s_hdr[0] + 1u;
-    poisoned = s_hdr[1] != 0u;
-}
-__device__ __forceinline__ void onepass_end(const SyncView& sv, unsigned epoch) {
-    __syncthreads();
-    if (threadIdx.x == 0) {
-        const unsigned f = __hip_atomic_fetch_add(&sv.hdr[0], 1u, __ATOMIC_RELAXED, __HIP_MEMORY_SCOPE_AGENT);
-        if (f + 1u == gridDim.x) {
-            __hip_atomic_store(&sv.hdr[0], 0u, __ATOMIC_RELAXED, __HIP_MEMORY_SCOPE_AGENT);
-            __hip_atomic_store(&sv.hdr[2], epoch, __ATOMIC_RELAXED, __HIP_MEMORY_SCOPE_AGENT);
-        }
-    }
-}
-__device__ __forceinline__ void onepass_publish(const SyncView& sv, long v, unsigned epoch, float p0, float p1, int lane) {
-    if (lane == 0) {
-        const unsigned long long e = (unsigned long long)epoch << 32;
-        __hip_atomic_store(&sv.gran[v * 2 + 0], e | __float_as_uint(p0), __ATOMIC_RELAXED, __HIP_MEMORY_SCOPE_AGENT);
-        __hip_atomic_store(&sv.gran[v * 2 + 1], e | __float_as_uint(p1), __ATOMIC_RELAXED, __HIP_MEMORY_SCOPE_AGENT);
-    }
-}
-__device__ __forceinline__ void onepass_sweep(const SyncView& sv, long g0, int wpg, unsigned epoch, int lane, bool poisoned,
-                                              float* __restrict__ pa, float* __restrict__ pb) {
-    for (int polls = poisoned ? (1 << 17) : 0;; ++polls) {
-        bool hit = true;
-#pragma unroll 2
-        for (int w = lane; w < wpg; w += 64) {
-            const unsigned long long ga = __hip_atomic_load(&sv.gran[(g0 + w) * 2 + 0], __ATOMIC_RELAXED, __HIP_MEMORY_SCOPE_AGENT);
-            const unsigned long long gb = __hip_atomic_load(&sv.gran[(g0 + w) * 2 + 1], __ATOMIC_RELAXED, __HIP_MEMORY_SCOPE_AGENT);
-            hit = hit && (unsigned)(ga >> 32) == epoch && (unsigned)(gb >> 32) == epoch;
-            pa[w] = __uint_as_float((unsigned)ga);
-            pb[w] = __uint_as_float((unsigned)gb);
-        }
-        if (__all(hit)) break;
-        if (polls > (1 << 17)) {
-            if (lane == 0) __hip_atomic_store(&sv.hdr[3], 1u, __ATOMIC_RELAXED, __HIP_MEMORY_SCOPE_AGENT);
-            for (int w = lane; w < wpg; w += 64) { pa[w] = __uint_as_float(0x7fc00000u); pb[w] = __uint_as_float(0x7fc00000u); }
-            break;
-        }
-        __builtin_amdgcn_s_sleep(4);
-    }
-    asm volatile("s_waitcnt lgkmcnt(0)" ::: "memory");
-}
 
 struct OnepassItem { int grp, w, seg; long row; };
 __device__ __forceinline__ OnepassItem onepass_item(long v, const c2s_norm_desc& d, int segs) {
diff --git a/crop2seg_amd/csrc/norm_shared.h b/crop2seg_amd/csrc/norm_shared.h
--- /dev/null
+++ b/crop2seg_amd/csrc/norm_shared.h
@@ -0,0 +1,103 @@
+#pragma once
+#include "common.h"
+
+namespace {
+
+__device__ __forceinline__ float fwd_element(float x, float mu, float a, float b, int relu, bool has_res, float r) {
+    float t = (x - mu) * a + b;
+    if (relu) t = fmaxf(t, 0.f);
+    if (has_res) t += r;
+    return t;
+}
+
+template <typename P>
+__device__ __forceinline__ void merge_moments(int items, int lane, float eps, P partial, float& mean_f, float& rstd_f,
+                                              float& unbiased) {
+    double cnt = 0.0, sum = 0.0;
+    for (int it = lane; it < items; it += 64) {
+        float pm, pm2;
+        int len;
+        if (!partial(it, pm, pm2, len)) continue;
+        cnt += len;
+        sum += (double)pm * len;
+    }
+    for (int o = 32; o > 0; o >>= 1) { cnt += __shfl_xor(cnt, o, 64); sum += __shfl_xor(sum, o, 64); }
+    const double mean = cnt > 0 ? sum / cnt : 0.0;
+    double m2 = 0.0;
+    for (int it = lane; it < items; it += 64) {
+        float pm, pm2;
+        int len;
+        if (!partial(it, pm, pm2, len)) continue;
+        const double dm = (double)pm - mean;
+        m2 += (double)pm2 + dm * dm * len;
+    }
+    for (int o = 32; o > 0; o >>= 1) m2 += __shfl_xor(m2, o, 64);
+    const double var = cnt > 0 ? m2 / cnt : 0.0;
+    mean_f = (float)mean;
+    rstd_f = (float)(1.0 / sqrt(var + (double)eps));
+    unbiased = (float)(cnt > 1 ? m2 / (cnt - 1.0) : var);
+}
+
+struct SyncView {
+    unsigned* hdr;
+    unsigned long long* gran;
+};
+__host__ __device__ inline size_t sync_bytes(long nitems) { return 64 + (size_t)nitems * 16; }
+__device__ __forceinline__ SyncView sync_view(void* base) {
+    SyncView v;
+    v.hdr = reinterpret_cast<unsigned*>(base);
+    v.gran = reinterpret_cast<unsigned long long*>(reinterpret_cast<char*>(base) + 64);
+    return v;
+}
+constexpr int OP_MAXG = 8;
+
+__device__ __forceinline__ void onepass_begin(const SyncView& sv, unsigned* s_hdr, unsigned& epoch, bool& poisoned) {
+    if (threadIdx.x == 0) {
+        s_hdr[0] = __hip_atomic_load(&sv.hdr[2], __ATOMIC_RELAXED, __HIP_MEMORY_SCOPE_AGENT);
+        s_hdr[1] = __hip_atomic_load(&sv.hdr[3], __ATOMIC_RELAXED, __HIP_MEMORY_SCOPE_AGENT);
+    }
+    __syncthreads();
+    epoch = s_hdr[0] + 1u;
+    poisoned = s_hdr[1] != 0u;
+}
+__device__ __forceinline__ void onepass_end(const SyncView& sv, unsigned epoch) {
+    __syncthreads();
+    if (threadIdx.x == 0) {
+        const unsigned f = __hip_atomic_fetch_add(&sv.hdr[0], 1u, __ATOMIC_RELAXED, __HIP_MEMORY_SCOPE_AGENT);
+        if (f + 1u == gridDim.x) {
+            __hip_atomic_store(&sv.hdr[0], 0u, __ATOMIC_RELAXED, __HIP_MEMORY_SCOPE_AGENT);
+            __hip_atomic_store(&sv.hdr[2], epoch, __ATOMIC_RELAXED, __HIP_MEMORY_SCOPE_AGENT);
+        }
+    }
+}
+__device__ __forceinline__ void onepass_publish(const SyncView& sv, long v, unsigned epoch, float p0, float p1, int lane) {
+    if (lane == 0) {
+        const unsigned long long e = (unsigned long long)epoch << 32;
+        __hip_atomic_store(&sv.gran[v * 2 + 0], e | __float_as_uint(p0), __ATOMIC_RELAXED, __HIP_MEMORY_SCOPE_AGENT);
+        __hip_atomic_store(&sv.gran[v * 2 + 1], e | __float_as_uint(p1), __ATOMIC_RELAXED, __HIP_MEMORY_SCOPE_AGENT);
+    }
+}
+__device__ __forceinline__ void onepass_sweep(const SyncView& sv, long g0, int wpg, unsigned epoch, int lane, bool poisoned,
+                                              float* __restrict__ pa, float* __restrict__ pb) {
+    for (int polls = poisoned ? (1 << 17) : 0;; ++polls) {
+        bool hit = true;
+#pragma unroll 2
+        for (int w = lane; w < wpg; w += 64) {
+            const unsigned long long ga = __hip_atomic_load(&sv.gran[(g0 + w) * 2 + 0], __ATOMIC_RELAXED, __HIP_MEMORY_SCOPE_AGENT);
+            const unsigned long long gb = __hip_atomic_load(&sv.gran[(g0 + w) * 2 + 1], __ATOMIC_RELAXED, __HIP_MEMORY_SCOPE_AGENT);
+            hit = hit && (unsigned)(ga >> 32) == epoch && (unsigned)(gb >> 32) == epoch;
+            pa[w] = __uint_as_float((unsigned)ga);
+            pb[w] = __uint_as_float((unsigned)gb);
+        }
+        if (__all(hit)) break;
+        if (polls > (1 << 17)) {
+            if (lane == 0) __hip_atomic_store(&sv.hdr[3], 1u, __ATOMIC_RELAXED, __HIP_MEMORY_SCOPE_AGENT);
+            for (int w = lane; w < wpg; w += 64) { pa[w] = __uint_as_float(0x7fc00000u); pb[w] = __uint_as_float(0x7fc00000u); }
+            break;
+        }
+        __builtin_amdgcn_s_sleep(4);
+    }
+    asm volatile("s_waitcnt lgkmcnt(0)" ::: "memory");
+}
+
+}
diff --git a/crop2seg_amd/engine.py b/crop2seg_amd/engine.py
--- a/crop2seg_amd/engine.py
+++ b/crop2seg_amd/engine.py
@@ -155,8 +155,9 @@
     def check_sync(self) -> None:
         if self.sync_error() == 0:
             return
-        global ONEPASS_NORM
+        global ONEPASS_NORM, FIRST_NORM_FUSED
         ONEPASS_NORM = False
+        FIRST_NORM_FUSED = False
         torch.cuda.synchronize(self.device)
         self.bufs["sync"].zero_()
         raise RuntimeError(
@@ -633,10 +634,20 @@
     chans = [C0, C1] if C1 else [C0]
     Ho = (Hin + 2 * pad - K) // S + 1
     Wo = (Win + 2 * pad - K) // S + 1
-    KK = K * K
     out = torch.empty(N, Cout, Ho, Wo, device=s0.device, dtype=torch.float32)
     _run_conv(ctx, conv_plan("fwd", N, chans, Cout, Hin, Win, K, S, pad, pad_mode), wname, W, s0, s1,
               ctx.p[bname] if bname else None, out, valid)
+    return _conv2d_record(ctx, out, srcs, wname, bname, K, S, pad, pad_mode, valid, need_input_grad)
+
+
+def _conv2d_record(ctx: Ctx, out: Tensor, srcs: Sequence[Tensor], wname: str, bname: Optional[str], K: int, S: int, pad: int,
+                   pad_mode: int, valid: Optional[Tensor], need_input_grad: bool) -> Tensor:
+    W = ctx.p[wname]
+    Cout, Cin = W.shape[0], W.shape[1]
+    N, C0, Hin, Win = srcs[0].shape
+    chans = [C0, srcs[1].shape[1]] if len(srcs) > 1 else [C0]
+    Ho, Wo = out.shape[2], out.shape[3]
+    KK = K * K
     if not ctx.mark([out], srcs, [wname, bname]):
         return out
     tape = ctx.tape
@@ -767,8 +778,20 @@
 ONEPASS_MIN_HW = int(_os.environ.get("C2S_NORM_ONEPASS_MIN_HW", "1024"))
 
 
-def norm_act(ctx: Ctx, x: Tensor, prefix: str, kind: int, groups: int, relu: bool, residual: Optional[Tensor],
-             valid: Optional[Tensor], pad_value: float = 0.0, conv_bias: Optional[str] = None, affine: bool = True) -> Tensor:
+class _NormCall(NamedTuple):
+    d: NormDesc
+    gamma: Tensor
+    beta: Tensor
+    rm: Optional[Tensor]
+    rv: Optional[Tensor]
+    nbt: Optional[Tensor]
+    gstats: Tensor
+    row_ab: Tensor
+    nws: int
+    sync_bytes: int
+
+
+def _norm_call(ctx: Ctx, x: Tensor, prefix: str, kind: int, groups: int, valid: Optional[Tensor], affine: bool) -> _NormCall:
     N, Cc = x.shape[0], x.shape[1]
     HW = x[0, 0].numel()
     batch = kind == _lib.NORM_BATCH
@@ -787,11 +810,18 @@
     gstats = torch.empty(ngroups * 2, device=x.device, dtype=torch.float32)
     row_ab = torch.empty(N * Cc * 3, device=x.device, dtype=torch.float32)
     nws = lib().c2s_norm_workspace_floats(C.byref(d))
-    ws = ctx.ws.get("norm", nws)
-    y = torch.empty_like(x)
     nbt = ctx.b.get(prefix + ".num_batches_tracked") if (batch and ctx.training) else None
     sync_bytes = (lib().c2s_norm_onepass_sync_bytes(C.byref(d), 1 if valid is not None else 0)
                   if ONEPASS_NORM and HW >= ONEPASS_MIN_HW else 0)
+    return _NormCall(d, gamma, beta, rm, rv, nbt, gstats, row_ab, nws, sync_bytes)
+
+
+def norm_act(ctx: Ctx, x: Tensor, prefix: str, kind: int, groups: int, relu: bool, residual: Optional[Tensor],
+             valid: Optional[Tensor], pad_value: float = 0.0, conv_bias: Optional[str] = None, affine: bool = True) -> Tensor:
+    nc = _norm_call(ctx, x, prefix, kind, groups, valid, affine)
+    d, gamma, beta, rm, rv, nbt, gstats, row_ab, nws, sync_bytes = nc
+    ws = ctx.ws.get("norm", nws)
+    y = torch.empty_like(x)
     if sync_bytes:
         sync = ctx.ws.sync_area(sync_bytes)
         check(lib().c2s_norm_fwd_onepass(C.byref(d), x.data_ptr(), gamma.data_ptr(), beta.data_ptr(), _ptr(rm), _ptr(rv),
@@ -802,6 +832,13 @@
         check(lib().c2s_norm_fwd(C.byref(d), x.data_ptr(), gamma.data_ptr(), beta.data_ptr(), _ptr(rm), _ptr(rv), _ptr(nbt),
                                  gstats.data_ptr(), row_ab.data_ptr(), _ptr(residual), y.data_ptr(), int(relu),
                                  ws.data_ptr(), ws.numel(), _ptr(valid), float(pad_value), _stream()), "norm_fwd")
+    return _norm_record(ctx, nc, x, y, prefix, relu, residual, valid, conv_bias, affine)
+
+
+def _norm_record(ctx: Ctx, nc: _NormCall, x: Tensor, y: Tensor, prefix: str, relu: bool, residual: Optional[Tensor],
+                 valid: Optional[Tensor], conv_bias: Optional[str], affine: bool) -> Tensor:
+    d, gamma, beta, rm, rv, nbt, gstats, row_ab, nws, sync_bytes = nc
+    Cc = x.shape[1]
     pnames = [prefix + ".weight", prefix + ".bias"] if affine else []
     if not ctx.mark([y], [x, residual], pnames + [conv_bias]):
         return y
@@ -872,6 +909,40 @@
     bwd.saved = {"group_stats": gstats, "row_ab": row_ab}
     tape.record(bwd)
     return y
+
+
+FIRST_NORM_FUSED = _os.environ.get("C2S_FIRST_NORM_FUSED", "1") != "0"
+
+
+def conv_norm_fused(ctx: Ctx, srcs: Sequence[Tensor], wname: str, bname: Optional[str], nprefix: str, K: int, S: int, pad: int,
+                    pad_mode: int, kind: int, groups: int, relu: bool, residual: Optional[Tensor], valid: Optional[Tensor],
+                    pad_value: float = 0.0, need_input_grad: bool = True, affine: bool = True) -> Optional[Tensor]:
+    if not (FIRST_NORM_FUSED and ONEPASS_NORM and affine and len(srcs) == 1):
+        return None
+    W = ctx.p[wname]
+    s0 = srcs[0]
+    N, C0, Hin, Win = s0.shape
+    Cout = W.shape[0]
+    plan = conv_plan("fwd", N, [C0], Cout, Hin, Win, K, S, pad, pad_mode)
+    if plan.family != "smallcin":
+        return None
+    desc, key, pkind, *where = plan.launches[0]
+    nd = NormDesc(N, Cout, Hin * Win, kind, groups if kind != _lib.NORM_BATCH else 1, 1, ctx.eps, ctx.momentum)
+    if not lib().c2s_conv3x3_smallcin_norm_supported(C.byref(desc), C.byref(nd), int(relu), int(residual is not None)):
+        return None
+    y = torch.empty(N, Cout, Hin, Win, device=s0.device, dtype=torch.float32)
+    x1 = torch.empty_like(y) if ctx.tape is not None else None
+    nc = _norm_call(ctx, y, nprefix, kind, groups, valid, affine)
+    packed = ctx.pack((wname,) + key, W, *where, kind=pkind)[0]
+    sync = ctx.ws.sync_area(max(nc.sync_bytes, lib().c2s_conv3x3_smallcin_norm_sync_bytes(C.byref(desc), C.byref(nc.d))))
+    check(lib().c2s_conv3x3_smallcin_norm(C.byref(desc), C.byref(nc.d), s0.data_ptr(), packed.data_ptr(),
+                                          _ptr(ctx.p[bname]) if bname else None, nc.gamma.data_ptr(), nc.beta.data_ptr(),
+                                          _ptr(x1), y.data_ptr(), nc.gstats.data_ptr(), nc.row_ab.data_ptr(), _ptr(valid),
+                                          float(pad_value), sync.data_ptr(), sync.numel(), _stream()), "conv3x3_smallcin_norm")
+    if x1 is None:
+        return y
+    _conv2d_record(ctx, x1, srcs, wname, bname, K, S, pad, pad_mode, valid, need_input_grad)
+    return _norm_record(ctx, nc, x1, y, nprefix, relu, residual, valid, bname, affine)
 
 
 def squeeze_excite(ctx: Ctx, x: Tensor, prefix: str, valid: Optional[Tensor], pad_value: float = 0.0) -> Tensor:
diff --git a/include/c2s_hip.h b/include/c2s_hip.h
--- a/include/c2s_hip.h
+++ b/include/c2s_hip.h
@@ -152,6 +152,13 @@
                          const float* group_stats, const float* row_ab, int relu, float* gx, float* dgamma, float* dbeta,
                          float* dbias, float* workspace, size_t ws_floats, const int* valid, void* sync,
                          size_t sync_bytes, void* stream);
+
+int c2s_conv3x3_smallcin_norm_supported(const c2s_conv_desc* d, const c2s_norm_desc* nd, int relu, int has_residual);
+size_t c2s_conv3x3_smallcin_norm_sync_bytes(const c2s_conv_desc* d, const c2s_norm_desc* nd);
+int c2s_conv3x3_smallcin_norm(const c2s_conv_desc* d, const c2s_norm_desc* nd, const float* src, const float* wpk,
+                              const float* bias, const float* gamma, const float* beta, float* raw, float* y,
+                              float* group_stats, float* row_ab, const int* valid, float pad_value, void* sync,
+                              size_t sync_bytes, void* stream);
 
 size_t c2s_se_workspace_floats(int N, int C, int HW);
 int c2s_channel_bias_add(float* x, const float* bias, const int* valid, int N, int C, int HW, void* stream);
```

Result: no change. 387.1 (median of 6 runs) (+0.9%).
